# hzxie/Stereo-3D-Reconstruction

Hardware: AMD Instinct MI355X
Metric: stereo pairs/s forward (batch 32, 224x224 -> 32^3 voxel) (higher is better)
Workload: dtype f32

## Files before the change

include/s3r.h:

```cpp
#ifndef S3R_H
#define S3R_H

#include <stddef.h>
#include <stdint.h>

#ifdef __cplusplus
extern "C" {
#endif

#define S3R_ABI_VERSION 8

typedef enum s3r_status {
    S3R_OK = 0,
    S3R_ERR_INVALID = -1,
    S3R_ERR_HIP = -2,
    S3R_ERR_WORKSPACE = -3
} s3r_status;

typedef enum s3r_op {
    S3R_OP_CONV = 0,
    S3R_OP_DECONV = 1,
    S3R_OP_LINEAR = 2
} s3r_op;

typedef enum s3r_dtype {
    S3R_F32 = 0,
    S3R_BF16 = 1
} s3r_dtype;

typedef enum s3r_act { S3R_ACT_NONE = 0, S3R_ACT_RELU = 1, S3R_ACT_SIGMOID = 2,
                       S3R_ACT_LEAKY_RELU = 3, S3R_ACT_ELU = 4, S3R_ACT_TANH = 5  } s3r_act;

typedef enum s3r_layout { S3R_LAYOUT_PLAIN = 0, S3R_LAYOUT_WINO_H = 2, S3R_LAYOUT_WINO_DH = 3, S3R_LAYOUT_WINO_HW = 4 } s3r_layout;

typedef enum s3r_algo { S3R_ALGO_AUTO = 0, S3R_ALGO_DIRECT = 1, S3R_ALGO_WINOGRAD = 2 } s3r_algo;

typedef struct s3r_conv_desc {
    int32_t op;
    int32_t ndim;
    int32_t batch;
    int32_t cin, cout;
    int32_t in_size;
    int32_t k, stride, pad;
    int32_t act;
    int32_t tag;
    int32_t tile;
    int32_t in_halo;
    int32_t out_halo;
    int32_t ksplit;
    int32_t dtype;
    int32_t in_layout;
    int32_t out_layout;
    int32_t algo;
    int32_t dilation;
    int32_t out_pad;
    float act_param;
} s3r_conv_desc;

typedef struct s3r_layer {
    s3r_conv_desc desc;
    const void* packed_w;
    const float* scale;
    const float* shift;
} s3r_layer;

int s3r_abi_version(void);
const char* s3r_last_error(void);

int s3r_conv_out_size(const s3r_conv_desc* d);
int s3r_conv_packed_elems(const s3r_conv_desc* d, int64_t* elems);
int s3r_conv_pack_weights(const s3r_conv_desc* d, const float* w, void* packed, void* stream);
int64_t s3r_conv_scratch_elems(const s3r_conv_desc* d);
int s3r_conv_forward(const s3r_conv_desc* d, const void* x, const void* packed_w, const float* scale,
                     const float* shift, void* y, float* scratch, int64_t scratch_elems, void* stream);

int64_t s3r_chain_workspace_elems(const s3r_layer* layers, int n_layers);
int s3r_chain_forward(const s3r_layer* layers, int n_layers, const void* x, void* y, float* ws, int64_t ws_elems,
                      int ws_fresh, void* stream);

int s3r_encoder_forward(const s3r_layer* layers, int n_layers, const float* images_left, const float* images_right,
                        void* features, float* ws, int64_t ws_elems, int ws_fresh, void* stream);
int s3r_decoder_forward(const s3r_layer* layers, int n_layers, const void* volume, float* occupancy, float* ws,
                        int64_t ws_elems, int ws_fresh, void* stream);

int s3r_encoder_forward_u8(const s3r_layer* layers, int n_layers, const uint8_t* images_left, const uint8_t* images_right,
                           void* features, float* ws, int64_t ws_elems, int ws_fresh, void* stream);

int s3r_channels_last_to_f32(const void* x, float* y, int batch, int channels, int64_t positions, void* stream);

int s3r_cost_volume_forward(const float* feat_left, const float* feat_right, float* volume, int batch, int channels,
                            int max_disp, int height, int width, int out_halo, void* stream);

int s3r_cost_volume_forward_wino(const float* feat_left, const float* feat_right, float* planes, int batch, int channels,
                                 int max_disp, int height, int width, void* stream);
int64_t s3r_conv_wino_input_elems(const s3r_conv_desc* d);
int s3r_conv_wino_input_layout(const s3r_conv_desc* d);
int s3r_cost_volume_forward_wino2(const float* feat_left, const float* feat_right, float* planes, int batch, int channels,
                                  int max_disp, int height, int width, void* stream);

int s3r_cost_volume_forward_bf16(const void* feat_left, const void* feat_right, void* volume, int batch, int channels,
                                 int max_disp, int height, int width, int out_halo, void* stream);

int64_t s3r_linear_scratch_elems(int batch, int cin, int cout);
int s3r_linear_forward(const float* x, const float* w, const float* bias, float* y, int batch, int cin, int cout,
                       int act, float* scratch, int64_t scratch_elems, void* stream);

int s3r_chamfer_forward(const float* p, const float* q, float* dist1, float* dist2, int32_t* idx1, int32_t* idx2,
                        int batch, int n, int m, void* stream);

int s3r_chamfer_backward(const float* p, const float* q, const int32_t* idx1, const int32_t* idx2, const float* grad_dist1,
                         const float* grad_dist2, float* grad_p, float* grad_q, int batch, int n, int m, void* stream);

int s3r_voxel_iou(const float* pred, const float* gt, float threshold, float* iou, int batch, int64_t voxels,
                  void* stream);

int s3r_disparity_wta(const float* feat_l, const float* feat_r, float* disp_l, float* disp_r, int batch, int channels,
// ... 33 lines not shown
```

stereo-3d-reconstruction_amd/_lib.py:

```python
from __future__ import annotations

import ctypes as C
import os
import threading

_HERE = os.path.dirname(os.path.abspath(__file__))
LIB_PATH = os.environ.get("S3R_LIB") or os.path.join(_HERE, "csrc", "libs3r_hip.so")

OP_CONV, OP_DECONV, OP_LINEAR = 0, 1, 2
DTYPE = {"fp32": 0, "bf16": 1}
ACT = {"none": 0, "relu": 1, "sigmoid": 2, "leaky_relu": 3, "elu": 4, "tanh": 5}
FAMILY = {0: "conv_mfma", 1: "stem", 2: "head", 3: "cost_volume", 4: "linear", 5: "chamfer", 6: "iou", 7: "pack",
          8: "pad_copy", 9: "disparity", 10: "aux"}
ABI_VERSION = 8
ALGO_AUTO, ALGO_DIRECT, ALGO_WINOGRAD = 0, 1, 2
ALGO = {None: 0, "auto": 0, "direct": 1, "winograd": 2, False: 1, True: 2}
RAN = {0: "direct", 1: "winograd-serial", 2: "winograd-class-parallel", 3: "winograd-dual", 4: "winograd-2axis", 5: "winograd-3axis", 6: "winograd-3axis-class-parallel"}


class ConvDesc(C.Structure):
    _fields_ = [(n, C.c_int32) for n in
                ("op", "ndim", "batch", "cin", "cout", "in_size", "k", "stride", "pad", "act", "tag", "tile",
                 "in_halo", "out_halo", "ksplit", "dtype", "in_layout", "out_layout", "algo", "dilation", "out_pad")] + \
               [("act_param", C.c_float)]
# ... 17 lines not shown
_lock = threading.Lock()

SIGNATURES = {
    "s3r_abi_version": (C.c_int, []),
    "s3r_last_error": (C.c_char_p, []),
    "s3r_conv_out_size": (C.c_int, [C.POINTER(ConvDesc)]),
    "s3r_conv_packed_elems": (C.c_int, [C.POINTER(ConvDesc), C.POINTER(C.c_int64)]),
    "s3r_conv_pack_weights": (C.c_int, [C.POINTER(ConvDesc), C.c_void_p, C.c_void_p, C.c_void_p]),
    "s3r_conv_scratch_elems": (C.c_int64, [C.POINTER(ConvDesc)]),
    "s3r_conv_forward": (C.c_int, [C.POINTER(ConvDesc), C.c_void_p, C.c_void_p, C.c_void_p, C.c_void_p, C.c_void_p,
                                   C.c_void_p, C.c_int64, C.c_void_p]),
    "s3r_chain_workspace_elems": (C.c_int64, [C.POINTER(Layer), C.c_int]),
    "s3r_chain_forward": (C.c_int, [C.POINTER(Layer), C.c_int, C.c_void_p, C.c_void_p, C.c_void_p, C.c_int64,
                                    C.c_int, C.c_void_p]),
    "s3r_encoder_forward": (C.c_int, [C.POINTER(Layer), C.c_int, C.c_void_p, C.c_void_p, C.c_void_p, C.c_void_p,
                                      C.c_int64, C.c_int, C.c_void_p]),
    "s3r_encoder_forward_u8": (C.c_int, [C.POINTER(Layer), C.c_int, C.c_void_p, C.c_void_p, C.c_void_p, C.c_void_p,
                                         C.c_int64, C.c_int, C.c_void_p]),
    "s3r_channels_last_to_f32": (C.c_int, [C.c_void_p, C.c_void_p, C.c_int, C.c_int, C.c_int64, C.c_void_p]),
    "s3r_decoder_forward": (C.c_int, [C.POINTER(Layer), C.c_int, C.c_void_p, C.c_void_p, C.c_void_p, C.c_int64,
                                      C.c_int, C.c_void_p]),
    "s3r_cost_volume_forward": (C.c_int, [C.c_void_p, C.c_void_p, C.c_void_p, C.c_int, C.c_int, C.c_int, C.c_int,
                                          C.c_int, C.c_int, C.c_void_p]),
    "s3r_cost_volume_forward_bf16": (C.c_int, [C.c_void_p, C.c_void_p, C.c_void_p, C.c_int, C.c_int, C.c_int, C.c_int,
                                               C.c_int, C.c_int, C.c_void_p]),
    "s3r_cost_volume_forward_wino": (C.c_int, [C.c_void_p, C.c_void_p, C.c_void_p, C.c_int, C.c_int, C.c_int, C.c_int,
                                               C.c_int, C.c_void_p]),
    "s3r_conv_wino_input_elems": (C.c_int64, [C.POINTER(ConvDesc)]),
    "s3r_conv_wino_input_layout": (C.c_int, [C.POINTER(ConvDesc)]),
    "s3r_cost_volume_forward_wino2": (C.c_int, [C.c_void_p, C.c_void_p, C.c_void_p, C.c_int, C.c_int, C.c_int, C.c_int,
                                                C.c_int, C.c_void_p]),
    "s3r_linear_scratch_elems": (C.c_int64, [C.c_int, C.c_int, C.c_int]),
    "s3r_linear_forward": (C.c_int, [C.c_void_p, C.c_void_p, C.c_void_p, C.c_void_p, C.c_int, C.c_int, C.c_int,
                                     C.c_int, C.c_void_p, C.c_int64, C.c_void_p]),
    "s3r_chamfer_forward": (C.c_int, [C.c_void_p, C.c_void_p, C.c_void_p, C.c_void_p, C.c_void_p, C.c_void_p,
                                      C.c_int, C.c_int, C.c_int, C.c_void_p]),
    "s3r_chamfer_backward": (C.c_int, [C.c_void_p, C.c_void_p, C.c_void_p, C.c_void_p, C.c_void_p, C.c_void_p, C.c_void_p, C.c_void_p,
                                       C.c_int, C.c_int, C.c_int, C.c_void_p]),
    "s3r_voxel_iou": (C.c_int, [C.c_void_p, C.c_void_p, C.c_float, C.c_void_p, C.c_int, C.c_int64, C.c_void_p]),
    "s3r_disparity_wta": (C.c_int, [C.c_void_p, C.c_void_p, C.c_void_p, C.c_void_p, C.c_int, C.c_int, C.c_int, C.c_int,
                                    C.c_int, C.c_void_p]),
    "s3r_disparity_epe": (C.c_int, [C.c_void_p, C.c_void_p, C.c_void_p, C.c_void_p, C.c_int, C.c_int64, C.c_void_p]),
    "s3r_disparity_soft": (C.c_int, [C.c_void_p, C.c_void_p, C.c_int, C.c_void_p, C.c_void_p, C.c_void_p, C.c_void_p, C.c_int,
                                     C.c_int, C.c_int, C.c_int, C.c_int, C.c_float, C.c_int, C.c_int, C.c_float, C.c_void_p]),
    "s3r_disparity_metrics": (C.c_int, [C.c_void_p, C.c_void_p, C.c_void_p, C.c_void_p, C.c_int, C.c_int64, C.c_void_p]),
    "s3r_profile_enable": (C.c_int, [C.c_int]),
    "s3r_profile_reset": (C.c_int, []),
    "s3r_profile_detail": (C.c_int, [C.c_int]),
    "s3r_profile_read": (C.c_int, [C.POINTER(ProfRecord), C.c_int]),
}


def load():
    global _lib
    if _lib is not None:
        return _lib
    with _lock:
        if _lib is not None:
            return _lib
        if not os.path.exists(LIB_PATH):
            raise S3RError(
                f"HIP extension not built: {LIB_PATH} is missing. Run `python -c 'import __graft_entry__ as g; "
                f"g.build()'` (or `make -C stereo-3d-reconstruction_amd/csrc`). There is no CPU fallback.")
        try:
            lib = C.CDLL(LIB_PATH)
        except OSError as e:
            raise S3RError(f"cannot load {LIB_PATH}: {e}") from e
        for name, (res, args) in SIGNATURES.items():
            fn = getattr(lib, name)
            fn.restype, fn.argtypes = res, args
        if lib.s3r_abi_version() != ABI_VERSION:
            raise S3RError("libs3r_hip.so ABI version mismatch")
        _lib = lib
    return _lib


def check(rc, what=""):
    if rc < 0:
        msg = load().s3r_last_error().decode("utf-8", "replace")
        raise S3RError(f"{what}: {msg} (code {rc})")
    return rc


LAYOUT_PLAIN, LAYOUT_WINO_H, LAYOUT_WINO_DH, LAYOUT_WINO_HW = 0, 2, 3, 4


def make_desc(layer, batch, in_size, tag=0, tile=-1, in_halo=0, out_halo=0, ksplit=0, dtype=0, in_layout=0, out_layout=0,
              algo=0):
    from . import arch_spec as _spec
    op = {"conv2d": OP_CONV, "conv3d": OP_CONV, "deconv3d": OP_DECONV, "deconv2d": OP_DECONV, "linear": OP_LINEAR}[layer.op]
    nd = _spec.ndim(layer)
    return ConvDesc(op, nd, batch, layer.cin, layer.cout, in_size, layer.k, layer.s, layer.p, ACT[layer.act], tag,
                    tile, in_halo, out_halo, ksplit, dtype, in_layout, out_layout, algo, getattr(layer, "dil", 1),
                    getattr(layer, "opad", 0), _spec.act_param(layer))


def profile_enable(max_records):
    check(load().s3r_profile_enable(int(max_records)), "profile_enable")


def profile_detail(level):
    check(load().s3r_profile_detail(int(level)), "profile_detail")


def profile_reset():
    check(load().s3r_profile_reset(), "profile_reset")


def profile_read(max_records=4096):
    buf = (ProfRecord * max_records)()
    n = check(load().s3r_profile_read(buf, max_records), "profile_read")
    return [dict(family=FAMILY.get(r.family, str(r.family)), tag=r.tag, ms=r.ms, launches=r.launches, flops=r.flops,
                 bytes=r.bytes, exec_flops=r.exec_flops, ran=RAN.get(r.algo, str(r.algo))) for r in buf[:n]]
```

stereo-3d-reconstruction_amd/csrc/s3r_api.hip:

```cpp
#include "s3r_host.h"

#include <cmath>
#include <cstdlib>
#include <cstring>

using namespace s3rh;

namespace {

inline bool misaligned16(const void* p) { return ((uintptr_t)p & 15) != 0; }
int bf16_align_fail(const char* what, const void* p) {
    return fail(S3R_ERR_INVALID, "%s must be 16-byte aligned (got %p): bf16 tensors are accessed 16 bytes at a time", what, p);
}

int wino2_run(const s3r_conv_desc* d, const Geo& g, s3r::ConvParams p, const float* x, const float* packed_w, float* y, float* scratch,
              int64_t scratch_elems, int form, hipStream_t s, int* launches) {
    const Wino2Geo g2 = wino2_geo(d);
    const WinoNeed need = wino2_need(d, form);
    const bool pre = d->in_layout == S3R_LAYOUT_WINO_DH || d->in_layout == S3R_LAYOUT_WINO_HW;
    const bool to_v = d->out_layout == S3R_LAYOUT_WINO_HW;
    if (g2.bmax <= 0 || ((pre || to_v) && g2.bmax < d->batch))
        return fail(S3R_ERR_INVALID, "two-axis Winograd form: the transformed input of this batch exceeds 2 GiB (at most %d samples per "
                    "call with a producer-written input: s3r_conv_wino_input_elems)", g2.bmax);
    if (!scratch || scratch_elems < need.total)
        return fail(S3R_ERR_WORKSPACE, "the two-axis Winograd form of this layer needs %lld floats of scratch (s3r_conv_scratch_elems), "
                    "got %lld", (long long)need.total, (long long)(scratch ? scratch_elems : 0));
    const int64_t direct_w = ipow(d->k, g.nd) * d->cin * cout_pad(d->cout);
    p.w = packed_w + direct_w + (wino_layer(d) ? wino_w_elems(d) : 0);
    p.x = pre ? x : scratch;
    p.part = scratch + need.v;
    p.Nd = g2.sg; p.Nh = g2.sg; p.Nw = g2.out;
    p.kd = 1; p.kh = 1; p.kw = g2.kw; p.T = g2.kw;
    p.x_hs = g2.wp; p.x_ds = g2.sg * g2.wp; p.x_cs = g2.sg * g2.sg * g2.wp;
    p.x_org = 0;
    p.dS = s3r::FastDiv((unsigned)(p.Nd * p.Nh * p.Nw));
    p.dHW = s3r::FastDiv((unsigned)(p.Nh * p.Nw));
    p.dW = s3r::FastDiv((unsigned)p.Nw);
    if (g2.ax == 2) {
        p.Nd = 1; p.Nw = g2.sg;
        p.dS = s3r::FastDiv((unsigned)(g2.sg * g2.sg));
        p.dW = s3r::FastDiv((unsigned)g2.sg);
    }
    p.Hout = g2.out; p.Dout = g2.out;
    p.ncls = g2.ncls;
    p.ksplit = 1;
    const int64_t x_sample = g.x_elems / d->batch;
    *launches = 0;
    for (int b0 = 0; b0 < d->batch; b0 += g2.bmax) {
        const int nb = d->batch - b0 < g2.bmax ? d->batch - b0 : g2.bmax;
        hipError_t e = hipSuccess;
        if (!pre) {
            s3r::AuxScope aux(s, 4.0 * ((double)nb * x_sample + (double)(g2.ax == 2 ? g2.ncls * d->cin * s3r::wino2_npad(g2.pos_sample * nb) : g2.v_sample * nb)));
            if (g2.ax == 2)
                e = s3r::launch_wino2p_input(x + (int64_t)b0 * x_sample, scratch, nb, d->cin, g2.wp, g2.wp, g2.sg, g2.sg,
                                             s3r::wino2_npad(g2.pos_sample * nb), s);
            else
                e = s3r::launch_wino2_input(x + (int64_t)b0 * x_sample, scratch, g2.ax, (long long)nb * d->cin, g2.wp, g2.wp, g2.wp, g2.sg, g2.sg, s);
            if (e != hipSuccess) return hip_fail(e, "two-axis Winograd input transform launch");
            *launches += 1;
        }
        p.B = nb;
        p.x_cls = nb * d->cin * p.x_cs;
        p.x_bytes = (unsigned)(4 * (int64_t)nb * g2.v_sample);
        p.Ntotal = nb * p.Nd * p.Nh * p.Nw;
        p.y = y + (int64_t)b0 * p.y_bs;
        p.y_bytes = (unsigned)(4 * (int64_t)nb * p.y_bs);
        int nl = 0;
        e = s3r::launch_conv_wino2(p, g2.ax, wino2_form_of(d, p.Ntotal, form), to_v, s, &nl);
        if (e != hipSuccess) return hip_fail(e, "two-axis Winograd conv launch");
        *launches += nl;
    }
    return S3R_OK;
}

int dwino_run(const s3r_conv_desc* d, s3r::ConvParams p, const float* x, const float* packed_w, float* scratch, int64_t scratch_elems,
              int form, hipStream_t s, int* launches, int* ran) {
    const WinoNeed need = wino_need(d, form, p.head_w != nullptr);
    if (!scratch || scratch_elems < need.total)
        return fail(S3R_ERR_WORKSPACE, "the Winograd form of this transposed convolution needs %lld floats of scratch "
                    "(s3r_conv_scratch_elems), got %lld", (long long)need.total, (long long)(scratch ? scratch_elems : 0));
    const int n = d->in_size;
    p.xd_mode = dwino_materialise(d) ? 1 : 0;
    hipError_t e;
    {
        const double x_el = (double)d->batch * d->cin * (double)ipow(n + 2, 3);
        s3r::AuxScope aux(s, 4.0 * x_el * (p.xd_mode ? 4.0 : 2.0));
        e = s3r::launch_wino_diff(x, scratch, (long long)d->batch * d->cin, n + 2, n + 2, n + 2, p.xd_mode, s);
    }
    if (e != hipSuccess) return hip_fail(e, "Winograd difference-tensor launch");
    p.x = x;
    p.xd = scratch;
    p.part = scratch + need.v;
    p.w = packed_w + 64 * (int64_t)d->cin * cout_pad(d->cout);
    p.Nd = n / 2; p.Nh = n / 2;
    p.Ntotal = p.B * p.Nd * p.Nh * p.Nw;
    p.n_begin = 0; p.n_end = p.Ntotal;
    p.dS = s3r::FastDiv((unsigned)(p.Nd * p.Nh * p.Nw));
    p.dHW = s3r::FastDiv((unsigned)(p.Nh * p.Nw));
    p.dW = s3r::FastDiv((unsigned)p.Nw);
    p.ksplit = 1;
    const s3r::WinoLaunch L = s3r::wino_plan(2, d->cout, wino_kcls(d), p.Ntotal, p.head_w != nullptr, form);
    int nl = 0;
    e = s3r::launch_deconv_wino(p, L, s, &nl);
    if (e != hipSuccess) return hip_fail(e, "Winograd transposed-conv launch");
    *launches = 1 + nl;
    *ran = 1 + L.mode;
    return S3R_OK;
}
int dwino3_run(const s3r_conv_desc* d, s3r::ConvParams p, const float* x, const float* packed_w, float* scratch, int64_t scratch_elems,
               hipStream_t s, int form, int* launches, int* ran) {
    const int n = d->in_size;
    const Dwino3Need nd = dwino3_need(d, form);
    const int64_t need = nd.total;
    if (!scratch || scratch_elems < need)
        return fail(S3R_ERR_WORKSPACE, "the three-axis Winograd form of this transposed convolution needs %lld floats of scratch "
                    "(s3r_conv_scratch_elems), got %lld", (long long)need, (long long)(scratch ? scratch_elems : 0));
    hipError_t e;
    {
        s3r::AuxScope aux(s, 4.0 * 4.0 * (double)d->batch * d->cin * (double)ipow(n + 2, 3));
        e = s3r::launch_wino_diff(x, scratch, (long long)d->batch * d->cin, n + 2, n + 2, n + 2, 1, s);
    }
    if (e != hipSuccess) return hip_fail(e, "Winograd difference-tensor launch");
    p.x = x;
    p.xd = scratch;
    p.w = packed_w + dwino3_w_offset(d);
    p.Nd = p.Nh = p.Nw = n / 2;
    p.Ntotal = p.B * p.Nd * p.Nh * p.Nw;
    p.dS = s3r::FastDiv((unsigned)(p.Nd * p.Nh * p.Nw));
    p.dHW = s3r::FastDiv((unsigned)(p.Nh * p.Nw));
    p.dW = s3r::FastDiv((unsigned)p.Nw);
    p.ksplit = 1;
    p.part = nd.split ? scratch + nd.diff : nullptr;
    e = s3r::launch_deconv_wino3(p, nd.split, s);
    if (e != hipSuccess) return hip_fail(e, "three-axis Winograd transposed-conv launch");
    *launches = nd.split ? 3 : 2;
    *ran = nd.split ? 6 : 5;
    return S3R_OK;
}

int conv_head_fused(const s3r_conv_desc* d, const Geo& g, const s3r_conv_desc* hd, const Geo& hg, const float* x,
                    const s3r_layer& L, const s3r_layer& H, float* out, float* scratch, int64_t scratch_elems, hipStream_t s) {
    s3r::ConvParams p = make_params(d, g);
    p.x = x; p.w = static_cast<const float*>(L.packed_w); p.scale = L.scale; p.shift = L.shift; p.y = out;
    const bool is3 = hd->ndim == 3;
    p.y_hs = hg.out_p; p.y_ds = is3 ? hg.out_p * hg.out_p : 0; p.y_cs = (int)ipow(hg.out_p, hg.nd);
    p.y_bs = p.y_cs;
    p.y_org = hd->out_halo * (p.y_ds + p.y_hs + 1);
    p.y_bytes = (unsigned)(hg.y_elems * 4);
    p.head_w = static_cast<const float*>(H.packed_w); p.head_scale = H.scale; p.head_shift = H.shift; p.head_act = hd->act;
    int alg, form;
    int rc = resolve_algo(d, &alg, &form);
    if (rc) return rc;
    if (alg == ALG_WINO3) {
        if (d->cout > 64) return fail(S3R_ERR_INVALID, "the fused head rides on the transposed Winograd kernel with <= 64 couts only");
        ProfScope ps(s, F_MFMA, d->tag, g.flops + hg.flops, g.bytes - 4.0 * d->batch * d->cout * (double)g.out_sp +
                     4.0 * d->batch * (double)hg.out_sp);
        ps.exec = g.flops * (27.0 / 64.0) + hg.flops;
        ps.algo = 5;
        return dwino3_run(d, p, x, static_cast<const float*>(L.packed_w), scratch, scratch_elems, s, form, &ps.launches, &ps.algo);
    }
    if (alg != ALG_DIRECT) {
        if (alg != ALG_WINO || d->op != S3R_OP_DECONV || d->cout > 64) return fail(S3R_ERR_INVALID, "the fused head rides on the transposed Winograd kernel with <= 64 couts only");
        ProfScope ps(s, F_MFMA, d->tag, g.flops + hg.flops, g.bytes - 4.0 * d->batch * d->cout * (double)g.out_sp +
                     4.0 * d->batch * (double)hg.out_sp);
        ps.exec = wino_exec_flops(d, g) + hg.flops;
        return dwino_run(d, p, x, static_cast<const float*>(L.packed_w), scratch, scratch_elems, form, s, &ps.launches, &ps.algo);
    }
    Launch Ln;
    rc = resolve_launch(d, &p, &Ln);
    if (rc) return rc;
    if (!(Ln.cfg == 1 || Ln.cfg == 2 || Ln.cfg == 7) || (Ln.cfg == 2 && d->cout > 32)) {
        int bm, bn;
        s3r::conv_tile_dims(1, &bm, &bn);
        const long wg1 = (long)((p.Ntotal + bn - 1) / bn) * (p.transposed ? 8 : 1);
        Ln.cfg = d->cout <= 32 ? 2 : (wg1 >= 2000 ? 1 : 7);
    }
    ProfScope ps(s, F_MFMA, d->tag, g.flops + hg.flops, g.bytes - 4.0 * d->batch * d->cout * (double)g.out_sp +
                 4.0 * d->batch * (double)hg.out_sp);
    hipError_t e = s3r::launch_conv_mfma(p, Ln.cfg + 16 * Ln.vec, s);
    ps.launches = s3r::conv_last_launch_count();
    if (e != hipSuccess) return hip_fail(e, "fused conv+head launch");
    return S3R_OK;
}

int conv_head_fused_h(const s3r_conv_desc* d, const Geo& g, const s3r_conv_desc* hd, const Geo& hg, const void* x,
                      const s3r_layer& L, const s3r_layer& H, float* out, hipStream_t s) {
    s3r::ConvParamsH p = make_params_h(d, g);
    p.x = x; p.w = L.packed_w; p.scale = L.scale; p.shift = L.shift; p.y = out;
// ... 283 lines not shown
                    if (e != hipSuccess) return hip_fail(e, "conv forward launch");
                    ps.launches += s3r::conv_last_launch_count();
                }
                if (needs_act_pass(d)) {
                    s3r::AuxScope aux(s, 8.0 * (double)g.y_elems);
                    e = s3r::launch_act(y, g.y_elems, d->act, d->act_param, s);
                    if (e != hipSuccess) return hip_fail(e, "activation launch");
                    ps.launches += 1;
                }
                return S3R_OK;
            }
            s3r::ConvParams p = make_params(d, g);
            p.x = x; p.w = packed_w; p.scale = scale; p.shift = shift; p.y = y;
            const bool wino = alg == ALG_WINO;
            if (alg == ALG_WINO2) {
                ProfScope ps(s, F_MFMA, d->tag, g.flops, g.bytes);
                ps.exec = wino2_exec_flops(d);
                ps.algo = 4;
                return wino2_run(d, g, p, x, packed_w, y, scratch, scratch_elems, form, s, &ps.launches);
            }
            if (alg == ALG_WINO3) {
                ProfScope ps(s, F_MFMA, d->tag, g.flops, g.bytes);
                ps.exec = g.flops * (27.0 / 64.0);
                ps.algo = 5;
                return dwino3_run(d, p, x, packed_w, scratch, scratch_elems, s, form, &ps.launches, &ps.algo);
            }
            if (wino && d->op == S3R_OP_DECONV) {
                ProfScope ps(s, F_MFMA, d->tag, g.flops, g.bytes);
                ps.exec = wino_exec_flops(d, g);
                return dwino_run(d, p, x, packed_w, scratch, scratch_elems, form, s, &ps.launches, &ps.algo);
            }
            if (wino) {
                const bool pre = d->in_layout == S3R_LAYOUT_WINO_H;
                const int R = wino_r(d), kind = wino_kind(d);
                const int is3 = d->ndim == 3, n = d->in_size, wp = n + 2, h2 = (n + R - 1) / R, dp = is3 ? n + 2 : 1;
                const int bmax = wino_bmax(d);
                if (bmax <= 0 || (pre && bmax < d->batch))
                    return fail(S3R_ERR_INVALID, "a Winograd-transformed input takes at most %d samples per call here "
                                "(s3r_conv_wino_input_elems)", bmax);
                const WinoNeed need = wino_need(d, form, false);
                if (need.total > 0 && (!scratch || scratch_elems < need.total))
                    return fail(S3R_ERR_WORKSPACE, "the Winograd form of this layer needs %lld floats of scratch (s3r_conv_scratch_elems), "
                                "got %lld", (long long)need.total, (long long)(scratch ? scratch_elems : 0));
                const int64_t v_sample = wino_v_elems(d) / d->batch, x_sample = g.x_elems / d->batch;
                ProfScope ps(s, F_MFMA, d->tag, g.flops, g.bytes);
                ps.launches = 0;
                ps.exec = wino_exec_flops(d, g);
                p.w = packed_w + ipow(3, g.nd) * d->cin * cout_pad(d->cout);
                p.x = pre ? x : scratch;
                p.part = scratch ? scratch + need.v : nullptr;
                p.Nh = h2; p.T = p.kd * p.kw;
                p.x_hs = wp; p.x_ds = is3 ? h2 * wp : 0; p.x_cs = dp * h2 * wp;
                p.x_org = 0;
                p.dS = s3r::FastDiv((unsigned)(p.Nd * p.Nh * p.Nw));
                p.dHW = s3r::FastDiv((unsigned)(p.Nh * p.Nw));
                p.dW = s3r::FastDiv((unsigned)p.Nw);
                p.Hout = n;
                p.ksplit = 1;
                for (int b0 = 0; b0 < d->batch; b0 += bmax) {
                    const int nb = d->batch - b0 < bmax ? d->batch - b0 : bmax;
                    if (!pre) {
                        s3r::AuxScope aux(s, 4.0 * ((double)nb * x_sample + (double)nb * v_sample));
                        e = s3r::launch_wino_input(x + (int64_t)b0 * x_sample, scratch, (long long)nb * d->cin * dp, n + 2, wp, h2, R, s);
                        if (e != hipSuccess) return hip_fail(e, "Winograd input transform launch");
                        ps.launches += 1;
                    }
                    p.B = nb;
                    p.x_cls = nb * d->cin * p.x_cs;
                    p.x_bytes = (unsigned)(4 * (int64_t)nb * v_sample);
                    p.Ntotal = nb * p.Nd * p.Nh * p.Nw;
                    p.y = y + (int64_t)b0 * p.y_bs;
                    p.y_bytes = (unsigned)(4 * (int64_t)nb * p.y_bs);
                    const s3r::WinoLaunch WL = s3r::wino_plan(kind, d->cout, wino_kcls(d), p.Ntotal, false, form);
                    int nl = 0;
                    e = s3r::launch_conv_wino(p, WL, s, &nl);
                    if (e != hipSuccess) return hip_fail(e, "Winograd conv launch");
                    ps.launches += nl;
                    ps.algo = 1 + WL.mode;
                }
                return S3R_OK;
            }
            Launch L;
            if ((rc = resolve_launch(d, &p, &L))) return rc;
            if (L.ksplit > 1) {
                const int64_t need = s3r::conv_scratch_elems(p, L.cfg);
                if (scratch && scratch_elems >= need) p.part = scratch;
                else
                    return fail(S3R_ERR_WORKSPACE, "ksplit=%d needs %lld floats of scratch (s3r_conv_scratch_elems), got %lld", L.ksplit,
                                (long long)need, (long long)(scratch ? scratch_elems : 0));
            }
            ProfScope ps(s, F_MFMA, d->tag, g.flops, g.bytes);
            e = s3r::launch_conv_mfma(p, L.cfg + 16 * L.vec, s);
            ps.launches = s3r::conv_last_launch_count();
            if (e == hipSuccess && needs_act_pass(d)) {
                s3r::AuxScope aux(s, 8.0 * (double)g.y_elems);
                e = s3r::launch_act(y, g.y_elems, d->act, d->act_param, s);
                ps.launches += 1;
            }
            break;
        }
    }
    if (e != hipSuccess) return hip_fail(e, "conv forward launch");
    return S3R_OK;
}

int chain_forward_impl(const s3r_layer* layers, int n_layers, const void* x, const void* x2, int nsplit, int x_u8, void* y,
                       float* ws, int64_t ws_elems, int ws_fresh, void* stream);

}

extern "C" {

int s3r_chain_forward(const s3r_layer* layers, int n_layers, const void* x, void* y, float* ws, int64_t ws_elems,
                      int ws_fresh, void* stream) {
    return chain_forward_impl(layers, n_layers, x, nullptr, 0, 0, y, ws, ws_elems, ws_fresh, stream);
}

}

namespace {

int chain_forward_impl(const s3r_layer* layers, int n_layers, const void* x, const void* x2, int nsplit, int x_u8, void* y,
                       float* ws, int64_t ws_elems, int ws_fresh, void* stream) {
    Plan pl;
    int rc = plan_chain(layers, n_layers, &pl);
    if (rc) return rc;
    if (!x || !y) return fail(S3R_ERR_INVALID, "null tensor pointer");
    {
        const int last = n_layers - 1;
        bool any_bf16 = false;
        for (int i = 0; i < n_layers; ++i) any_bf16 = any_bf16 || pl.d[i].dtype == S3R_BF16;
        if (pl.d[0].dtype == S3R_BF16 && pl.r[0] != R_STEM && misaligned16(x)) return bf16_align_fail("the bf16 input of an S3R_BF16 chain", x);
        if (pl.d[last].dtype == S3R_BF16 && pl.r[last] != R_HEAD && misaligned16(y))
            return bf16_align_fail("the bf16 output of an S3R_BF16 chain", y);
        if (any_bf16 && pl.total > 0 && ws && misaligned16(ws)) return bf16_align_fail("the workspace of a chain with S3R_BF16 layers", ws);
    }
    if (pl.total > 0 && (!ws || ws_elems < pl.total))
        return fail(S3R_ERR_WORKSPACE, "chain needs a workspace of %lld floats, got %lld", (long long)pl.total,
                    (long long)ws_elems);
    hipStream_t s = (hipStream_t)stream;
    if (ws_fresh && pl.total > 0) {
        hipError_t e = hipMemsetAsync(ws, 0, (size_t)pl.total * sizeof(float), s);
        if (e != hipSuccess) return hip_fail(e, "workspace memset");
    }
    const void* cur = x;
    if ((x2 || x_u8) && (pl.pad_input || pl.r[0] != R_STEM))
        return fail(S3R_ERR_INVALID, "a second input tensor / 8-bit renders need a chain that starts with the stem convolution");
    if (pl.r[0] == R_STEM && (((uintptr_t)x & 15) || ((uintptr_t)x2 & 15)))
        return fail(S3R_ERR_INVALID, "render tensors must be 16-byte aligned (got %p, %p)", x, x2);
    if (pl.pad_input) {
        const s3r_conv_desc& d0 = pl.d[0];
        const int hl = d0.in_halo, is3 = d0.ndim == 3;
        ProfScope ps(s, F_PAD, d0.tag, 0.0, 8.0 * d0.batch * d0.cin * (double)pl.g[0].in_sp);
        hipError_t e;
        if (d0.dtype == S3R_BF16) {
            const int wc = d0.in_size * d0.cin / 2, hwc = hl * d0.cin / 2;
            e = s3r::launch_pad_copy(static_cast<const float*>(x), ws + pl.pad_off, d0.batch, is3 ? d0.in_size : 1,
                                     d0.in_size, wc, is3 ? hl : 0, hl, hwc, s);
        } else {
            e = s3r::launch_pad_copy(static_cast<const float*>(x), ws + pl.pad_off, (int64_t)d0.batch * d0.cin,
                                     is3 ? d0.in_size : 1, d0.in_size, d0.in_size, is3 ? hl : 0, hl, hl, s);
        }
        if (e != hipSuccess) return hip_fail(e, "pad copy launch");
        cur = ws + pl.pad_off;
    }
    for (int i = 0; i < n_layers; ++i) {
// ... 306 lines not shown
```

stereo-3d-reconstruction_amd/csrc/s3r_conv_glds.hip:

```cpp
#include "s3r_kernels.h"
#include <cstdlib>
#include <type_traits>

namespace s3r {

typedef float f32x16 __attribute__((ext_vector_type(16)));
typedef float v4f __attribute__((ext_vector_type(4)));
typedef float v2f __attribute__((ext_vector_type(2)));
typedef float v4f_u __attribute__((ext_vector_type(4), aligned(4)));
typedef float v2f_u __attribute__((ext_vector_type(2), aligned(4)));
typedef unsigned v2u __attribute__((ext_vector_type(2)));
typedef unsigned v4u __attribute__((ext_vector_type(4)));

#define S3R_LDS_PTR(p) ((__attribute__((address_space(3))) void*)(p))

template <int N> struct FVec;
template <> struct FVec<1> { typedef float type; };
template <> struct FVec<2> { typedef v2f type; };
template <> struct FVec<4> { typedef v4f type; };

template <int N>
__device__ __forceinline__ float vget(const typename FVec<N>::type& v, int i) {
    if constexpr (N == 1) return v; else return v[i];
}
// ... 544 lines not shown

void conv_tile_dims(int cfg, int* bm, int* bn) {
    *bm = kTileDims[cfg][0];
    *bn = kTileDims[cfg][1];
}
int conv_num_tiles() { return kNumTiles; }

struct Tuned { int cin, cout, T, stride, S, transposed, tile, ksplit; };
static const Tuned kTuned[] = {
    {32,  64,  9, 1, 12544, 0, 7, 1},
    {64,  64,  9, 2,  3136, 0, 1, 1},
    {64, 128,  9, 1,  3136, 0, 4, 1},
    {128, 128, 9, 2,   784, 0, 7, 1},
    {128, 256, 9, 1,   784, 0, 1, 1},
    {256, 256, 9, 1,   784, 0, 1, 1},
    {256, 32,  1, 1,   784, 0, 2, 1},
    {64,  64, 27, 1, 21952, 0, 1, 1},
    {64, 128, 27, 2,  2744, 0, 7, 1},
    {128, 128, 27, 1, 2744, 0, 7, 1},
    {128, 256, 27, 2,  343, 0, 3, 4},
    {256, 256, 27, 1,  343, 0, 3, 4},
    {256, 512, 64, 1,   64, 0, 7, 8},
    {512, 256,  8, 1,   64, 1, 7, 1},
    {256, 128,  8, 1,  512, 1, 1, 1},
    {128,  64,  8, 1, 4096, 1, 1, 1},
};

static const Tuned* find_tuned(const ConvParams& p) {
    const int S = p.Nd * p.Nh * p.Nw;
    for (const Tuned& t : kTuned)
        if (t.cin == p.Cin && t.cout == p.Cout && t.T == p.T && t.stride == p.stride && t.S == S &&
            t.transposed == p.transposed)
            return &t;
    return nullptr;
}

int conv_pick_ksplit(const ConvParams& p, int ) {
    if (const Tuned* t = find_tuned(p)) return t->ksplit;
    const int chunks = p.Cin / GBK;
    const long S = (long)p.Nd * p.Nh * p.Nw;
    const long wg_nom = ((p.Cout + 63) / 64) * ((32 * S + 63) / 64) * (p.transposed ? 8 : 1);
    int ks = 1;
    while (wg_nom * ks < 2048 && chunks % (2 * ks) == 0 && (chunks / (2 * ks)) * p.T >= 100) ks *= 2;
    return ks;
}

int conv_pick_tile(const ConvParams& p) {
    const int classes = (p.transposed ? 8 : 1) * (p.ksplit > 1 ? p.ksplit : 1);
    auto wgs = [&](int cfg) {
        const long bm = kTileDims[cfg][0], bn = kTileDims[cfg][1];
        return ((p.Cout + bm - 1) / bm) * ((p.Ntotal + bn - 1) / bn) * classes;
    };
    if (const Tuned* t = find_tuned(p))
        if (wgs(t->tile) >= 512) return t->tile;
    if (p.Cout <= 32) return wgs(2) >= 128 ? 2 : 3;
    if (p.Cout <= 64) return wgs(1) >= 2000 ? 1 : (wgs(7) >= 2000 ? 7 : 3);
    if (wgs(2) >= 1500) return 2;
    return wgs(7) >= 1500 ? 7 : 3;
}

int conv_pick_vec(const ConvParams& p) {
    if (p.stride != 1) return 1;
    return (p.Nw % 4 == 0) ? 4 : 1;
}

template <int WM, int WN, int TM, int TN, int VEC, bool HEAD, int NBUF = 2>
static hipError_t launch_cfg(ConvParams p, hipStream_t stream) {
    constexpr int BM = 32 * WM * TM, BN = 32 * WN * TN;
    if constexpr (GBK * BN % (256 * VEC) != 0 || BN > 256 * VEC) {
        return hipErrorInvalidValue;
    } else {
        p.m_tiles = (p.Cout + BM - 1) / BM;
        p.n_tiles = (p.n_end - p.n_begin + BN - 1) / BN;
        const size_t lds = (size_t)NBUF * GBK * (BM + BN) * sizeof(float);
        if (lds > 48 * 1024) {
            static LdsAttr lds_attr;
            const hipError_t attr = lds_attr.ensure(
                reinterpret_cast<const void*>(&conv_glds_kernel<WM, WN, TM, TN, VEC, HEAD, NBUF>), (int)lds);
            if (attr != hipSuccess) return attr;
        }
        dim3 grid(p.m_tiles * p.n_tiles * (p.transposed ? 8 : 1), 1, p.ksplit);
        hipLaunchKernelGGL((conv_glds_kernel<WM, WN, TM, TN, VEC, HEAD, NBUF>), grid, dim3(256), lds, stream, p);
        hipError_t e = hipGetLastError();
        if (e == hipSuccess && p.ksplit > 1) e = launch_conv_finish(p, p.n_tiles * BN, stream);
        return e;
    }
}

template <int WM, int WN, int TM, int TN, int VEC>
static hipError_t launch_dual_cfg(ConvParams p, int n_cut, hipStream_t stream) {
    constexpr int BM = 32 * WM * TM, BN = 32 * WN * TN;
    if constexpr (GBK * BN % (256 * VEC) != 0 || BN > 256 * VEC || GBK * 64 % (256 * VEC) != 0) {
        return hipErrorInvalidValue;
    } else {
        p.n_cut = n_cut;
        p.big_wgs = ((p.Cout + BM - 1) / BM) * ((n_cut - p.n_begin + BN - 1) / BN);
        const int small = ((p.Cout + 63) / 64) * ((p.n_end - n_cut + 63) / 64);
        p.m_tiles = 0; p.n_tiles = 0;
        const size_t lds = (size_t)2 * GBK * (BM + BN) * sizeof(float);
        if (lds > 48 * 1024) {
            static LdsAttr lds_attr;
            const hipError_t attr = lds_attr.ensure(reinterpret_cast<const void*>(&conv_glds_dual_kernel<WM, WN, TM, TN, VEC>), (int)lds);
            if (attr != hipSuccess) return attr;
        }
        hipLaunchKernelGGL((conv_glds_dual_kernel<WM, WN, TM, TN, VEC>), dim3(p.big_wgs + small), dim3(256), lds, stream, p);
        return hipGetLastError();
    }
}

template <int WM, int WN, int TM, int TN>
static hipError_t launch_dual_vec(const ConvParams& p, int n_cut, int vec, hipStream_t stream) {
    switch (vec) {
        case 4: return launch_dual_cfg<WM, WN, TM, TN, 4>(p, n_cut, stream);
        case 1: return launch_dual_cfg<WM, WN, TM, TN, 1>(p, n_cut, stream);
        default: return hipErrorInvalidValue;
    }
}

static hipError_t launch_dual(const ConvParams& p, int cfg, int n_cut, int vec, hipStream_t stream) {
    switch (cfg) {
        case 0: return launch_dual_vec<2, 2, 2, 2>(p, n_cut, vec, stream);
        case 1: return launch_dual_vec<1, 4, 2, 2>(p, n_cut, vec, stream);
        case 4: return launch_dual_vec<2, 2, 2, 4>(p, n_cut, vec, stream);
        case 7: return launch_dual_vec<1, 4, 2, 1>(p, n_cut, vec, stream);
        default: return hipErrorNotSupported;
    }
}

static bool sparse_launch(const ConvParams& p, int bm, int bn) {
    static const bool off = getenv("S3R_DEEP_RING") && atoi(getenv("S3R_DEEP_RING")) == 0;
    const long w = (long)((p.Cout + bm - 1) / bm) * ((p.n_end - p.n_begin + bn - 1) / bn) * (p.transposed ? 8 : 1) * p.ksplit;
    return !off && w <= 384;
}

template <int WM, int WN, int TM, int TN>
static hipError_t launch_vec(const ConvParams& p, int vec, hipStream_t stream) {
    if constexpr (WM == 1 && TM * TN <= 4) {
        if (p.head_w) {
            switch (vec) {
                case 4: return launch_cfg<WM, WN, TM, TN, 4, true>(p, stream);
                case 1: return launch_cfg<WM, WN, TM, TN, 1, true>(p, stream);
                default: return hipErrorInvalidValue;
            }
        }
    } else if (p.head_w) {
        return hipErrorInvalidValue;
    }
    if constexpr (WM == 2 && WN == 2 && TM == 1 && TN == 1) {
        if (sparse_launch(p, 64, 64)) {
            switch (vec) {
                case 4: return launch_cfg<WM, WN, TM, TN, 4, false, 6>(p, stream);
                case 1: return launch_cfg<WM, WN, TM, TN, 1, false, 6>(p, stream);
                default: return hipErrorInvalidValue;
            }
        }
    }
    switch (vec) {
        case 4: return launch_cfg<WM, WN, TM, TN, 4, false>(p, stream);
        case 1: return launch_cfg<WM, WN, TM, TN, 1, false>(p, stream);
        default: return hipErrorInvalidValue;
    }
}

static hipError_t launch_tile(const ConvParams& p, int cfg, int vec, hipStream_t stream) {
    g_launch_count += 1;
    switch (cfg) {
        case 0: return launch_vec<2, 2, 2, 2>(p, vec, stream);
        case 1: return launch_vec<1, 4, 2, 2>(p, vec, stream);
        case 2: return launch_vec<1, 4, 1, 2>(p, vec, stream);
        case 3: return launch_vec<2, 2, 1, 1>(p, vec, stream);
        case 4: return launch_vec<2, 2, 2, 4>(p, vec, stream);
        case 5: return launch_vec<1, 4, 2, 4>(p, vec, stream);
        case 6: return launch_vec<2, 2, 2, 1>(p, vec, stream);
        case 7: return launch_vec<1, 4, 2, 1>(p, vec, stream);
        default: return hipErrorInvalidValue;
    }
}

static bool plan_tail_cut(const ConvParams& p, int cfg, int* n_cut) {
    if (p.ksplit != 1 || p.Cout <= 32 || cfg == 3) return false;
    const int classes = p.transposed ? 8 : 1;
    const long bm = kTileDims[cfg][0], bn = kTileDims[cfg][1];
    const long m_tiles = (p.Cout + bm - 1) / bm, n_tiles = (p.Ntotal + bn - 1) / bn;
    const long W = m_tiles * n_tiles * classes;
    const long CUS = cu_count();
    const long rounds = W / CUS, rem = W % CUS;
    const bool dual = !p.transposed && (cfg == 0 || cfg == 1 || cfg == 4 || cfg == 7) && getenv("S3R_NO_DUAL") == nullptr;
    if (rounds < 1 || rounds >= (dual ? 64 : 16) || rem == 0) return false;
    const long n_main = (rounds * CUS) / (m_tiles * classes);
    if (n_main < 1 || n_main >= n_tiles) return false;
    const long pos_tail = p.Ntotal - n_main * bn;
    const long W_tail = ((pos_tail + 63) / 64) * ((p.Cout + 63) / 64) * classes;
    const double before = (double)((W + CUS - 1) / CUS);
    const double bulk = (double)((n_main * m_tiles * classes + CUS - 1) / CUS);
    const double small = (64.0 * 64.0) / (double)(bm * bn);
    const double after = dual ? bulk + (double)W_tail / (double)CUS * small / 0.85
                              : bulk + (double)((W_tail + CUS - 1) / CUS) * small / 0.8;
    if (after > (dual ? 0.99 : 0.97) * before) return false;
    *n_cut = (int)(n_main * bn);
    return true;
}

hipError_t launch_conv_mfma(const ConvParams& pin, int code, hipStream_t stream) {
    ConvParams p = pin;
    g_launch_count = 0;
    int cfg = code & 15;
    int vec = code >> 4;
    if (cfg == 15) cfg = conv_pick_tile(p);
    if (cfg >= kNumTiles) return hipErrorInvalidValue;
    const int vmax = conv_pick_vec(p);
    if (vec != 1 && vec != 4) vec = vmax;
    if (vec > vmax) vec = vmax;
    if (p.Cin % GBK != 0 || p.Ntotal % vec != 0) return hipErrorInvalidValue;
    if (p.ksplit < 1 || (p.Cin / GBK) % p.ksplit != 0 || (p.ksplit > 1 && !p.part)) return hipErrorInvalidValue;
    if (p.head_w) {
        int bm, bn;
        conv_tile_dims(cfg, &bm, &bn);
        const bool wm1 = cfg == 1 || cfg == 2 || cfg == 7;
        if (!wm1 || bm < p.Cout || p.ksplit != 1 || p.act == ACT_SIGMOID) return hipErrorInvalidValue;
    }
#ifdef S3R_ABLATE
    p.debug = abl_mode();
#endif
    p.n_begin = 0;
    p.n_end = p.Ntotal;
    int n_cut = 0;
    static const bool no_cut = getenv("S3R_NO_TAIL_CUT") != nullptr;
    if (!p.head_w && !no_cut && plan_tail_cut(p, cfg, &n_cut)) {
        static const bool no_dual = getenv("S3R_NO_DUAL") != nullptr;
        if (!no_dual && !p.transposed && p.Cout > 32) {
            g_launch_count += 1;
            const hipError_t ed = launch_dual(p, cfg, n_cut, vec, stream);
            if (ed != hipErrorNotSupported) return ed;
            g_launch_count -= 1;
        }
        p.n_end = n_cut;
        hipError_t e = launch_tile(p, cfg, vec, stream);
        if (e != hipSuccess) return e;
        p.n_begin = n_cut;
        p.n_end = p.Ntotal;
        return launch_tile(p, 3, vec, stream);
    }
    return launch_tile(p, cfg, vec, stream);
}

__global__ void pack_glds_kernel(const float* __restrict__ w, float* __restrict__ wp, int Cin, int Cout, int CoutPad,
                                 int T, int transposed) {
    const size_t per_cls = (size_t)T * Cin * CoutPad;
    const size_t total = (transposed ? 8 : 1) * per_cls;
    for (size_t i = blockIdx.x * (size_t)blockDim.x + threadIdx.x; i < total; i += (size_t)gridDim.x * blockDim.x) {
        const int cls = (int)(i / per_cls);
        size_t r = i % per_cls;
        const int co = (int)(r % CoutPad);
        r /= CoutPad;
        const int c = (int)(r & 15);
        r >>= 4;
        const int tap = (int)(r % T);
        const int cc = (int)(r / T);
        const int cin = cc * 16 + c;
        float v = 0.f;
        if (co < Cout) {
            if (!transposed) {
                v = w[((size_t)co * Cin + cin) * T + tap];
            } else {
                const int rd = (cls >> 2) & 1, rh = (cls >> 1) & 1, rw = cls & 1;
                const int td = (tap >> 2) & 1, th = (tap >> 1) & 1, tw = tap & 1;
                const int kd = 3 - rd - 2 * td, kh = 3 - rh - 2 * th, kw = 3 - rw - 2 * tw;
                v = w[((size_t)cin * Cout + co) * 64 + (kd * 4 + kh) * 4 + kw];
            }
        }
        wp[i] = v;
    }
}

hipError_t launch_pack_conv(const float* w, float* wp, int Cin, int Cout, int CoutPad, int T, int transposed,
                            hipStream_t s) {
    hipLaunchKernelGGL(pack_glds_kernel, dim3(1024), dim3(256), 0, s, w, wp, Cin, Cout, CoutPad, T, transposed);
    return hipGetLastError();
}

#ifdef S3R_ABLATE
}
extern "C" int s3r_debug_read_timeline(unsigned long long* out, int nblocks) {
    if (nblocks > 65536) nblocks = 65536;
    return hipMemcpyFromSymbol(out, HIP_SYMBOL(s3r::s3r_timeline), sizeof(unsigned long long) * 6 * (size_t)nblocks) == hipSuccess ? nblocks : -1;
}
namespace s3r {
#endif
}
```

stereo-3d-reconstruction_amd/csrc/s3r_conv_wino.hip:

```cpp
#include "s3r_kernels.h"
#include <cstdlib>

namespace s3r {

typedef float wf32x16 __attribute__((ext_vector_type(16)));
typedef float wv2f __attribute__((ext_vector_type(2)));
template <int N> struct WVec;
template <> struct WVec<1> { typedef float type; };
template <> struct WVec<2> { typedef wv2f type; };
typedef float wv4f __attribute__((ext_vector_type(4)));
template <> struct WVec<4> { typedef wv4f type; };
template <int N>
__device__ __forceinline__ float wvget(const typename WVec<N>::type& v, int i) {
    if constexpr (N == 1) return v; else return v[i];
}

#define S3R_LDS_PTR_W(p) ((__attribute__((address_space(3))) void*)(p))

#ifndef S3R_WNB
#define S3R_WNB 2
#endif
#ifndef S3R_WBK
#define S3R_WBK 32
#endif
// ... 686 lines not shown
            for (int k = 0; k < R; ++k)
                if (k < row1) yo[wino_out_off<KIND>(k, p.y_ds, p.y_hs)] = wino_act(y[k], sc, sf, lo);
        }
    }
}

template <int KIND>
static hipError_t launch_wino_finish(const ConvParams& p, int n_begin, int n_end, int npad, hipStream_t stream) {
    const long long total = p.head_w ? (long long)(n_end - n_begin) : (long long)p.Cout * (n_end - n_begin);
    const long long blocks = (total + 255) / 256;
    const dim3 grid((unsigned)(blocks < 8192 ? blocks : 8192), KIND == 2 ? 8 : 1);
    if constexpr (KIND == 2) {
        if (p.head_w) hipLaunchKernelGGL((wino_finish_kernel<KIND, true>), grid, dim3(256), 0, stream, p, n_begin, n_end, npad);
        else hipLaunchKernelGGL((wino_finish_kernel<KIND, false>), grid, dim3(256), 0, stream, p, n_begin, n_end, npad);
    } else {
        hipLaunchKernelGGL((wino_finish_kernel<KIND, false>), grid, dim3(256), 0, stream, p, n_begin, n_end, npad);
    }
    return hipGetLastError();
}

constexpr int WCN = 64;
#ifdef S3R_ABLATE
static int wabl_mode() { static const int m = getenv("S3R_ABL") ? atoi(getenv("S3R_ABL")) : 0; return m; }
#define S3R_WABL(p) (p).debug = wabl_mode()
#else
#define S3R_WABL(p) (void)0
#endif

int64_t wino_slab_elems(int kind, int cout, int ntotal, const WinoLaunch& L) {
    if (L.mode == WINO_SERIAL) return 0;
    const int ncls = kind == 2 ? 72 : 6;
    const int n0 = L.mode == WINO_DUAL ? L.n_cut : 0;
    const int64_t npad = (int64_t)((ntotal - n0 + WCN - 1) / WCN) * WCN;
    return (int64_t)ncls * cout * npad;
}

WinoLaunch wino_plan(int kind, int cout, int kcls, int ntotal, bool head, int forced) {
    WinoLaunch L;
    L.mode = WINO_SERIAL; L.n_cut = 0;
    const int m_tiles = (cout + WBM - 1) / WBM;
    const int pcs = kind == 2 ? 8 : 1;
    const int ncls = kind == 2 ? 9 : 6;
    const long W = (long)m_tiles * ((ntotal + WCN - 1) / WCN) * pcs;
    if (forced < 0) {
        static const int env_mode = getenv("S3R_WINO_FORM") ? atoi(getenv("S3R_WINO_FORM")) : -1;
        forced = env_mode;
    }
    const int occ = kind == 2 ? 3 : 4;
    const int CUS = cu_count();
    const double u = (double)W / (double)CUS;
    int kb = (int)u;
    if (forced >= 0) {
        L.mode = forced <= WINO_DUAL ? forced : WINO_SERIAL;
        if ((double)kb >= u) kb -= 1;
    } else {
        (void)head;
        constexpr double EFF = 0.9, EFF_ALONE = 0.7, SLAB = 100.0, LAUNCH = 220.0, TAIL = 0.6;
        const double unit = (double)ncls * kcls;
        auto serial_cost = [&](int w) {
            const int rem = w % occ;
            return (w - (rem == 1 ? 1 : 0)) * unit / EFF + (rem == 1 ? unit / EFF_ALONE : 0.0);
        };
        const double serial = serial_cost((int)__builtin_ceil(u));
        const double cp = __builtin_ceil(u * ncls) * (kcls / EFF + SLAB) + LAUNCH;
        double best = serial;
        if (cp < best) { best = cp; L.mode = WINO_CP; }
        for (int k : {(int)u, (int)u % occ == 1 ? (int)u - 1 : 0}) {
            if (k < 1 || (double)k >= u) continue;
            const double dual = serial_cost(k) + TAIL * __builtin_ceil((u - k) * ncls) * (kcls / EFF + SLAB) + LAUNCH;
            if (dual < 0.97 * best) { best = dual; L.mode = WINO_DUAL; kb = k; }
        }
    }
    if (L.mode == WINO_DUAL) {
        const long n_main = ((long)kb * CUS) / (m_tiles * pcs);
        L.n_cut = (int)(n_main * WCN);
        if (L.n_cut <= 0 || L.n_cut >= ntotal) { L.mode = L.n_cut <= 0 ? WINO_CP : WINO_SERIAL; L.n_cut = 0; }
    }
    return L;
}

template <int VEC, int KIND>
static hipError_t launch_wino_forms(ConvParams p, const WinoLaunch& L, hipStream_t stream) {
    const int ntotal = p.Ntotal;
    auto lds_of = [](int bn) { return (size_t)WNB * WBK * (WBM + (KIND == 2 ? 2 : 1) * bn) * sizeof(float); };
    const int pcs = KIND == 2 ? 8 : 1;
    constexpr int NCLS = WinoKind<KIND>::NCLS;
    p.n_begin = 0; p.n_end = ntotal;
    if (L.mode == WINO_SERIAL) {
        const dim3 grid(p.m_tiles * ((ntotal + WCN - 1) / WCN) * pcs);
        if constexpr (KIND == 2) {
            if (p.head_w) {
                if (p.xd_mode) hipLaunchKernelGGL((wino_kernel<VEC, KIND, 2, false, true, true>), grid, dim3(256), lds_of(WCN), stream, p);
                else hipLaunchKernelGGL((wino_kernel<VEC, KIND, 2, false, true, false>), grid, dim3(256), lds_of(WCN), stream, p);
            } else {
                if (p.xd_mode) hipLaunchKernelGGL((wino_kernel<VEC, KIND, 2, false, false, true>), grid, dim3(256), lds_of(WCN), stream, p);
                else hipLaunchKernelGGL((wino_kernel<VEC, KIND, 2, false, false, false>), grid, dim3(256), lds_of(WCN), stream, p);
            }
            return hipGetLastError();
        }
        hipLaunchKernelGGL((wino_kernel<VEC, KIND, 2, false, false>), grid, dim3(256), lds_of(WCN), stream, p);
        return hipGetLastError();
    }
    if (!p.part) return hipErrorInvalidValue;
    const int n0 = L.mode == WINO_DUAL ? L.n_cut : 0;
    const int cp_tiles = (ntotal - n0 + WCN - 1) / WCN;
    const int cp_wgs = p.m_tiles * cp_tiles * NCLS * pcs;
    if (L.mode == WINO_DUAL) {
        p.n_cut = n0;
        p.big_wgs = p.m_tiles * (n0 / WCN) * pcs;
        const dim3 grid(p.big_wgs + cp_wgs);
        if constexpr (KIND == 2) {
            if (p.head_w) {
                if (p.xd_mode) hipLaunchKernelGGL((wino_dual_kernel<VEC, KIND, true, true>), grid, dim3(256), lds_of(WCN), stream, p);
                else hipLaunchKernelGGL((wino_dual_kernel<VEC, KIND, true, false>), grid, dim3(256), lds_of(WCN), stream, p);
            } else {
                if (p.xd_mode) hipLaunchKernelGGL((wino_dual_kernel<VEC, KIND, false, true>), grid, dim3(256), lds_of(WCN), stream, p);
                else hipLaunchKernelGGL((wino_dual_kernel<VEC, KIND, false, false>), grid, dim3(256), lds_of(WCN), stream, p);
            }
        } else {
            hipLaunchKernelGGL((wino_dual_kernel<VEC, KIND>), grid, dim3(256), lds_of(WCN), stream, p);
        }
    } else if (KIND == 2 && p.xd_mode) {
        hipLaunchKernelGGL((wino_kernel<VEC, KIND, 2, true, false, KIND == 2>), dim3(cp_wgs), dim3(256), lds_of(WCN), stream, p);
    } else {
        hipLaunchKernelGGL((wino_kernel<VEC, KIND, 2, true, false>), dim3(cp_wgs), dim3(256), lds_of(WCN), stream, p);
    }
    hipError_t e = hipGetLastError();
    if (e != hipSuccess) return e;
    AuxScope aux(stream, 4.0 * (double)(ntotal - n0) * p.Cout * (pcs * NCLS + (p.head_w ? 0.0 : pcs * WinoKind<KIND>::R)));
    return launch_wino_finish<KIND>(p, n0, ntotal, cp_tiles * WCN, stream);
}

hipError_t launch_conv_wino(ConvParams p, const WinoLaunch& L, hipStream_t stream, int* launches) {
    if (p.Cin % WBK != 0 || p.stride != 1 || p.transposed || p.ksplit != 1 || p.head_w || p.act == ACT_SIGMOID)
        return hipErrorInvalidValue;
    p.kh = 1;
    S3R_WABL(p);
    p.m_tiles = (p.Cout + WBM - 1) / WBM;
    if (launches) *launches = L.mode == WINO_SERIAL ? 1 : 2;
    return p.Nw % 4 == 0 ? launch_wino_forms<4, 1>(p, L, stream) : launch_wino_forms<1, 1>(p, L, stream);
}

hipError_t launch_deconv_wino(ConvParams p, const WinoLaunch& L, hipStream_t stream, int* launches) {
    if (p.Cin % WBK != 0 || !p.transposed || p.ksplit != 1 || !p.xd || p.act == ACT_SIGMOID || (p.head_w && p.Cout > WBM))
        return hipErrorInvalidValue;
    S3R_WABL(p);
    p.m_tiles = (p.Cout + WBM - 1) / WBM;
    if (launches) *launches = L.mode == WINO_SERIAL ? 1 : 2;
    if (p.Nw % 4 != 0) return hipErrorInvalidValue;
    return launch_wino_forms<4, 2>(p, L, stream);
}

template <int AX> struct WAxis;
template <> struct WAxis<0> { static constexpr int N = 6, M = 4, R = 3; };
template <> struct WAxis<1> { static constexpr int N = 5, M = 2, R = 4; };
int wino2_classes(int ax) { return ax == 1 ? 25 : 36; }
int wino2_outputs(int ax) { return ax == 1 ? 2 : 4; }

template <int AX>
__device__ __forceinline__ void wax_bt(const float (&r)[WAxis<AX>::N], float (&v)[WAxis<AX>::N]) {
    if constexpr (AX == 0) wino_rows_to_classes<4>(r, v);
    else {
        v[0] = fmaf(2.f, r[0] - r[2], r[3] - r[1]);
        v[1] = fmaf(-2.f, r[1], r[3] - r[2]);
        v[2] = fmaf(2.f, r[1], fmaf(-3.f, r[2], r[3]));
        v[3] = r[3] - r[1];
        v[4] = fmaf(2.f, r[1] - r[3], r[4] - r[2]);
    }
}
template <int AX>
__device__ __forceinline__ void wax_at(const float (&m)[WAxis<AX>::N], float (&y)[WAxis<AX>::M]) {
    if constexpr (AX == 0) wino_out<1>(m, y);
    else {
        y[0] = ((m[0] + m[1]) + m[2]) + m[3];
        y[1] = fmaf(2.f, m[3], m[1] - m[2]) + m[4];
    }
}
template <int AX>
__device__ __forceinline__ float wax_g(int c, const float (&g)[WAxis<AX>::R]) {
    if constexpr (AX == 0) {
        const float s02 = g[0] + g[2], a = g[0] * (1.f / 24.f) + g[2] * (1.f / 6.f), b12 = g[1] * (1.f / 12.f);
        return c == 0 ? g[0] * 0.25f : c == 1 ? (s02 + g[1]) * (-1.f / 6.f) : c == 2 ? (s02 - g[1]) * (-1.f / 6.f)
             : c == 3 ? a + b12 : c == 4 ? a - b12 : g[2];
    } else {
        const float e = g[0] + g[2], o = g[1] + g[3];
        return c == 0 ? g[0] * 0.5f : c == 1 ? (e + o) * -0.5f : c == 2 ? (o - e) * (1.f / 6.f)
             : c == 3 ? fmaf(g[3], 4.f / 3.f, fmaf(g[2], 2.f / 3.f, fmaf(g[1], 1.f / 3.f, g[0] * (1.f / 6.f)))) : g[3];
    }
}

template <int AX>
__global__ __launch_bounds__(256) void wino2_input_kernel(const float* __restrict__ x, float* __restrict__ V, unsigned total,
                                                          int Dp, int Hp, int Wp, int SD, int SH, FastDiv dW, FastDiv dSH, FastDiv dSD) {
    constexpr int N = WAxis<AX>::N, M = WAxis<AX>::M;
    for (unsigned i = blockIdx.x * 256u + threadIdx.x; i < total; i += gridDim.x * 256u) {
        const unsigned row = (unsigned)dW.div((int)i);
        const int w = (int)(i - row * (unsigned)Wp);
        const unsigned pg = (unsigned)dSH.div((int)row);
        const int sh = (int)(row - pg * (unsigned)SH);
        const unsigned pl = (unsigned)dSD.div((int)pg);
        const int sd = (int)(pg - pl * (unsigned)SD);
        const float* __restrict__ src = x + ((size_t)pl * Dp + M * sd) * Hp * Wp + (size_t)M * sh * Wp + w;
        float t[N][N];
#pragma unroll
        for (int a = 0; a < N; ++a) {
            float r[N], v[N];
#pragma unroll
            for (int b = 0; b < N; ++b)
                r[b] = (M * sd + a < Dp && M * sh + b < Hp) ? src[((size_t)a * Hp + b) * Wp] : 0.f;
            wax_bt<AX>(r, v);
#pragma unroll
// ... 316 lines not shown
    constexpr int N = 6, M = 4;
    extern __shared__ __attribute__((aligned(16))) float fsm[];
    const int tid = threadIdx.x;
    const int G = p.Nh * p.Nw, Wp = TOV ? p.Hout + 2 : p.y_hs, plane = TOV ? Wp * Wp : p.y_cs;
    const float lo = p.act == ACT_RELU ? 0.f : -__builtin_inff();
    const size_t cstride = (size_t)p.Cout * npad;
    const int nbg = (p.B + PL - 1) / PL;
    for (int item = blockIdx.x; item < p.Cout * nbg; item += gridDim.x) {
        const int mrow = item / nbg;
        const int b0 = (item - mrow * nbg) * PL;
        const int npl = p.B - b0 < PL ? p.B - b0 : PL;
        for (int i = tid; i < npl * plane; i += 256) fsm[i] = 0.f;
        __syncthreads();
        const float sc = p.scale ? p.scale[mrow] : 1.f, sf = p.shift ? p.shift[mrow] : 0.f;
        for (int t = tid; t < npl * G; t += 256) {
            const int pl = p.dS.div(t);
            const int s = t - pl * G;
            const int sh = p.dW.div(s);
            const int sw = s - sh * p.Nw;
            const int n = b0 * G + t;
            const float* __restrict__ src = p.part + ((size_t)mrow * (npad >> 6) + (n >> 6)) * ((SEMI ? N * M : N * N) * 64) + (n & 63);
            float tt[N][M];
#pragma unroll
            for (int a = 0; a < N; ++a) {
                if constexpr (SEMI) {
#pragma unroll
                    for (int v = 0; v < M; ++v) tt[a][v] = src[(a * M + v) * 64];
                } else {
                    float m[N], y[M];
#pragma unroll
                    for (int c = 0; c < N; ++c) m[c] = src[(a * N + c) * 64];
                    wax_at<0>(m, y);
#pragma unroll
                    for (int v = 0; v < M; ++v) tt[a][v] = y[v];
                }
            }
            float* __restrict__ o = fsm + pl * plane + (halo + M * sh) * Wp + halo + M * sw;
#pragma unroll
            for (int v = 0; v < M; ++v) {
                float m[N], y[M];
#pragma unroll
                for (int a = 0; a < N; ++a) m[a] = tt[a][v];
                wax_at<0>(m, y);
#pragma unroll
                for (int u = 0; u < M; ++u)
                    if (M * sh + v < p.Hout && M * sw + u < p.Hout) o[v * Wp + u] = wino_act(y[u], sc, sf, lo);
            }
        }
        __syncthreads();
        if constexpr (TOV) {
            for (int t = tid; t < npl * G; t += 256) {
                const int pl = p.dS.div(t);
                const int s = t - pl * G;
                const int sh = p.dW.div(s);
                const int sw = s - sh * p.Nw;
                const float* __restrict__ win = fsm + pl * plane + M * sh * Wp + M * sw;
                float tt[N][N];
#pragma unroll
                for (int jc = 0; jc < N; ++jc) {
                    float r[N], v[N];
#pragma unroll
                    for (int ir = 0; ir < N; ++ir) r[ir] = win[ir * Wp + jc];
                    wax_bt<0>(r, v);
#pragma unroll
                    for (int ir = 0; ir < N; ++ir) tt[ir][jc] = v[ir];
                }
                float* __restrict__ dst = p.y + (size_t)mrow * npad + (size_t)b0 * G + t;
#pragma unroll
                for (int bb = 0; bb < N; ++bb) {
                    float v[N];
                    wax_bt<0>(tt[bb], v);
#pragma unroll
                    for (int a = 0; a < N; ++a) dst[(size_t)(a * N + bb) * cstride] = v[a];
                }
            }
        } else {
            for (int pl = 0; pl < npl; ++pl)
                wino2_copy_out(fsm + pl * plane, p.y + (size_t)(b0 + pl) * p.y_bs + (size_t)mrow * p.y_cs, plane, tid);
        }
        __syncthreads();
    }
}

int wino2_form(int ax, int cout, int ntotal, int forced) {
    if (ax == 1) return 0;
    if (forced >= 0) return forced ? 1 : 0;
    static const int env_form = getenv("S3R_WINO2_FORM") ? atoi(getenv("S3R_WINO2_FORM")) : -1;
    if (env_form >= 0) return env_form ? 1 : 0;
    const long semi_wgs = (long)((cout + WBM - 1) / WBM) * ((ntotal + WCN - 1) / WCN) * 6;
    return semi_wgs >= (ax == 2 ? 2 : 8) * (long)cu_count() ? 1 : 0;
}
int64_t wino2_npad(int64_t ntotal) { return (ntotal + WCN - 1) / WCN * WCN; }
int64_t wino2_slab_elems(int ax, int cout, int ntotal, int form) {
    const int64_t npad = (int64_t)((ntotal + WCN - 1) / WCN) * WCN;
    return (form ? 6 * 4 : wino2_classes(ax)) * (int64_t)cout * npad;
}

hipError_t launch_conv_wino2(ConvParams p, int ax, int form, bool to_v, hipStream_t stream, int* launches) {
    if (p.Cin % WBK != 0 || p.stride != 1 || p.transposed || p.ksplit != 1 || p.head_w || p.act == ACT_SIGMOID || !p.part ||
        ax < 0 || ax > 2 || p.ncls != wino2_classes(ax))
        return hipErrorInvalidValue;
    p.kh = 1;
    S3R_WABL(p);
    p.m_tiles = (p.Cout + WBM - 1) / WBM;
    p.n_begin = 0; p.n_end = p.Ntotal;
    const int n_tiles = (p.Ntotal + WCN - 1) / WCN;
    const size_t lds = (size_t)WNB * WBK * (WBM + WCN) * sizeof(float);
    const int halo = to_v ? 1 : (p.y_hs - p.Hout) / 2;
    if (to_v && (ax != 2 || p.Hout % 4 != 0)) return hipErrorInvalidValue;
    if (!to_v && (halo < 0 || p.y_hs != p.Hout + 2 * halo)) return hipErrorInvalidValue;
    if (ax == 2) {
        const int plane = to_v ? (p.Hout + 2) * (p.Hout + 2) : p.y_hs * p.y_hs, G = p.Nh * p.Nw;
        if ((!to_v && p.y_cs != plane) || (size_t)plane * 4 > 64 * 1024) return hipErrorInvalidValue;
        int PL = 256 / G < 1 ? 1 : 256 / G;
        if (PL > p.B) PL = p.B;
        while (PL > 1 && (size_t)PL * plane * 4 > 64 * 1024) --PL;
        const int npad = n_tiles * WCN;
        ConvParams q = p;
        q.B = 1; q.Nd = 1; q.Nh = 1; q.Nw = npad;
        q.dS = q.dHW = q.dW = FastDiv((unsigned)npad);
        q.kd = q.kh = q.kw = 1; q.T = 1;
        q.x_org = 0; q.x_ds = 0; q.x_hs = 0; q.x_cs = npad; q.x_cls = p.Cin * npad;
        q.x_bytes = (unsigned)(4ull * 36 * p.Cin * npad);
        q.Ntotal = npad; q.n_end = npad;
        const dim3 grid(p.m_tiles * n_tiles * (form == 1 ? 6 : 36));
        if (form == 1) hipLaunchKernelGGL((wino_kernel<4, 1, 2, false, false, false, true>), grid, dim3(256), lds, stream, q);
        else hipLaunchKernelGGL((wino_kernel<4, 1, 2, true, false>), grid, dim3(256), lds, stream, q);
        hipError_t e = hipGetLastError();
        if (e != hipSuccess) return e;
        const long long items = (long long)p.Cout * ((p.B + PL - 1) / PL);
        const dim3 fgrid((unsigned)(items < 16384 ? items : 16384));
        const size_t flds = (size_t)PL * plane * 4;
        AuxScope aux(stream, 4.0 * (double)p.Cout * ((double)(form == 1 ? 24 : 36) * npad + (to_v ? 36.0 * npad : (double)p.B * plane)));
        if (to_v) {
            if (form == 1) hipLaunchKernelGGL((wino2p_finish_kernel<true, true>), fgrid, dim3(256), flds, stream, p, npad, halo, PL);
            else hipLaunchKernelGGL((wino2p_finish_kernel<false, true>), fgrid, dim3(256), flds, stream, p, npad, halo, PL);
        } else if (form == 1) hipLaunchKernelGGL((wino2p_finish_kernel<true, false>), fgrid, dim3(256), flds, stream, p, npad, halo, PL);
        else hipLaunchKernelGGL((wino2p_finish_kernel<false, false>), fgrid, dim3(256), flds, stream, p, npad, halo, PL);
        if (launches) *launches = 2;
        return hipGetLastError();
    }
    if (p.y_ds != p.y_hs * p.y_hs || p.y_cs != (p.Dout + 2 * halo) * p.y_ds) return hipErrorInvalidValue;
    if (form == 1) {
        const int M = wino2_outputs(ax), G = p.Nh * p.Nw;
        if (ax != 0 || (size_t)M * p.y_ds * 4 > 64 * 1024) return hipErrorInvalidValue;
        int SUB = 256 / G < 1 ? 1 : 256 / G;
        if (SUB > p.B * p.Nd) SUB = p.B * p.Nd;
        while (SUB > 1 && (size_t)SUB * M * p.y_ds * 4 > 64 * 1024) --SUB;
        const size_t flds = (size_t)SUB * M * p.y_ds * 4;
        const FastDiv dNd((unsigned)p.Nd), dMS((unsigned)(M * p.y_ds));
        const long long items = (long long)p.Cout * ((p.B * p.Nd + SUB - 1) / SUB);
        const dim3 fgrid((unsigned)(items < 32768 ? items : 32768));
        const dim3 grid(p.m_tiles * n_tiles * 6);
        if (p.Nw % 4 == 0) hipLaunchKernelGGL((wino_kernel<4, 1, 2, false, false, false, true>), grid, dim3(256), lds, stream, p);
        else hipLaunchKernelGGL((wino_kernel<1, 1, 2, false, false, false, true>), grid, dim3(256), lds, stream, p);
        hipError_t e = hipGetLastError();
        if (e != hipSuccess) return e;
        AuxScope aux(stream, 4.0 * (double)p.Cout * (24.0 * n_tiles * WCN + (double)p.B * p.y_cs));
        hipLaunchKernelGGL(wino2s_finish_kernel, fgrid, dim3(256), flds, stream, p, n_tiles * WCN, halo, SUB, dNd, dMS);
        if (launches) *launches = 2;
        return hipGetLastError();
    }
    const dim3 grid(p.m_tiles * n_tiles * p.ncls);
    if (p.Nw % 4 == 0) hipLaunchKernelGGL((wino_kernel<4, 1, 2, true, false>), grid, dim3(256), lds, stream, p);
    else hipLaunchKernelGGL((wino_kernel<1, 1, 2, true, false>), grid, dim3(256), lds, stream, p);
    hipError_t e = hipGetLastError();
    if (e != hipSuccess) return e;
    const long long total = (long long)p.Cout * p.Ntotal;
    const long long blocks = (total + 255) / 256;
    const dim3 flat((unsigned)(blocks < 8192 ? blocks : 8192));
    AuxScope aux(stream, 4.0 * (double)p.Cout * ((double)p.ncls * n_tiles * WCN + (double)p.B * p.Dout * p.Hout * p.Nw));
    if (ax == 0) hipLaunchKernelGGL(wino2_finish_flat_kernel<0>, flat, dim3(256), 0, stream, p, n_tiles * WCN);
    else hipLaunchKernelGGL(wino2_finish_flat_kernel<1>, flat, dim3(256), 0, stream, p, n_tiles * WCN);
    if (launches) *launches = 2;
    return hipGetLastError();
}

#ifdef S3R_ABLATE
}
extern "C" int s3r_debug_read_timeline_wino(unsigned long long* out, int nblocks) {
    if (nblocks > 65536) nblocks = 65536;
    return hipMemcpyFromSymbol(out, HIP_SYMBOL(s3r::s3r_wino_timeline), sizeof(unsigned long long) * 6 * (size_t)nblocks) == hipSuccess ? nblocks : -1;
}
extern "C" int s3r_debug_clear_timeline_wino() {
    void* ptr = nullptr;
    if (hipGetSymbolAddress(&ptr, HIP_SYMBOL(s3r::s3r_wino_timeline)) != hipSuccess) return -1;
    return hipMemset(ptr, 0, sizeof(unsigned long long) * 6 * 65536) == hipSuccess ? 0 : -1;
}
namespace s3r {
#endif

}
```

stereo-3d-reconstruction_amd/csrc/s3r_host.h:

```cpp
#pragma once
#include "../../include/s3r.h"
#include "s3r_kernels.h"

#include <cstdint>
#include <vector>

namespace s3rh {

constexpr int64_t kMaxElems = (int64_t)1 << 31;
constexpr int64_t kMaxBytes = (int64_t)1 << 32;

const char* last_error();

enum Family { F_MFMA = 0, F_STEM = 1, F_HEAD = 2, F_COSTVOL = 3, F_LINEAR = 4, F_CHAMFER = 5, F_IOU = 6, F_PACK = 7, F_PAD = 8, F_DISP = 9,
              F_AUX = 10 };

struct ProfScope {
    bool active = false;
    int slot = -1;
    unsigned gen = 0;
    hipEvent_t e0 = nullptr, e1 = nullptr;
    int launches = 1;
    int algo = 0;
    double exec = -1.0;
    int family, prev_tag = 0;
    hipStream_t stream;
    ProfScope(hipStream_t s, int family, int tag, double flops, double bytes);
    ~ProfScope();
    ProfScope(const ProfScope&) = delete;
    ProfScope& operator=(const ProfScope&) = delete;
};

struct Geo {
    int nd;
    int in, out;
    int in_p, out_p;
    int64_t in_sp, out_sp;
    int64_t x_elems, y_elems;
    int64_t x_store, y_store;
    int64_t w_elems;
    double flops, bytes;
};

enum Route { R_STEM, R_HEAD, R_MFMA, R_LINEAR };

enum { ALG_DIRECT = 0, ALG_WINO = 1, ALG_WINO2 = 2, ALG_WINO3 = 3 };

struct Wino2Geo { int ax, m, n, ncls, out, sg, wp, kw, bmax; int64_t w_elems, v_sample, pos_sample; };

struct WinoNeed { int64_t v, slab, total; };

struct LaunchH { int tm, ksplit; };

struct Launch { int cfg, vec, ksplit; };

struct Plan {
    std::vector<s3r_conv_desc> d;
    std::vector<Route> r;
    std::vector<Geo> g;
    std::vector<int64_t> off;
    std::vector<char> fuse_head;
    bool stem_wino = false;
    bool pad_input = false;
    int64_t pad_off = 0;
    int64_t scratch_off = 0, scratch_elems = 0;
    int64_t total = 0;
};


int fail(int code, const char* fmt, ...);
int hip_fail(hipError_t e, const char* what);
int64_t ipow(int64_t b, int e);
int wino_r(const s3r_conv_desc*);
int out_size(const s3r_conv_desc* d);
int dil_of(const s3r_conv_desc* d);
bool staged_layer(const s3r_conv_desc* d);
struct StagedGeo { int cin_pad, step, pe, sp; int64_t elems; int bmax; };
StagedGeo staged_geo(const s3r_conv_desc* d);
s3r::ConvParams make_params_staged(const s3r_conv_desc* d, const Geo& g);
struct TClassAxis { int kr, ke, qmin, nq; };
bool im2col_layer(const s3r_conv_desc* d);
bool leaky_fused(const s3r_conv_desc* d);
bool needs_act_pass(const s3r_conv_desc* d);
bool tclass_layer(const s3r_conv_desc* d);
bool tclass_direct(const s3r_conv_desc* d);
bool tshuf_layer(const s3r_conv_desc* d);
s3r::ConvParams make_params_tshuf(const s3r_conv_desc* d, const Geo& g);
int want_halo(const s3r_conv_desc* d, Route r);
TClassAxis tclass_axis(const s3r_conv_desc* d, int r);
int tclass_halo(const s3r_conv_desc* d);
int64_t tclass_w_elems(const s3r_conv_desc* d);
bool make_params_tclass(const s3r_conv_desc* d, const Geo& g, int rd, int rh, int rw, s3r::ConvParams* q, int64_t* w_off, double* macs);
int geometry(const s3r_conv_desc* d, Geo* g);
int route(const s3r_conv_desc* d, Route* r);
int need_halo(const s3r_conv_desc* d, Route r);
int check_halos(const s3r_conv_desc* d, Route r);
int cout_pad(int cout);
int wino_mode();
bool wino_layer(const s3r_conv_desc* d);
bool dwino_layer(const s3r_conv_desc* d);
bool dwino3_layer(const s3r_conv_desc* d);
bool dwino3_desc_ok(const s3r_conv_desc* d);
int64_t dwino3_w_offset(const s3r_conv_desc* d);
struct Dwino3Need { int64_t diff, total; bool split; };
Dwino3Need dwino3_need(const s3r_conv_desc* d, int form);
bool wino_desc_ok(const s3r_conv_desc* d);
int wino2_ax(const s3r_conv_desc* d);
bool wino2_desc_ok(const s3r_conv_desc* d);
int wino2_max_edge();
int resolve_algo(const s3r_conv_desc* d, int* alg, int* form);
bool resolves_to_wino(const s3r_conv_desc* d);
Wino2Geo wino2_geo(const s3r_conv_desc* d);
int64_t wino_w_elems(const s3r_conv_desc* d);
int64_t wino_v_elems(const s3r_conv_desc* d);
int wino_bmax(const s3r_conv_desc* d);
int64_t dwino_w_elems(const s3r_conv_desc* d);
bool dwino_materialise(const s3r_conv_desc* d);
int64_t dwino_d_elems(const s3r_conv_desc* d);
int wino_kind(const s3r_conv_desc* d);
int wino_kcls(const s3r_conv_desc* d);
int64_t wino_positions(const s3r_conv_desc* d, int nb);
WinoNeed wino_need(const s3r_conv_desc* d, int form, bool head);
double wino_exec_flops(const s3r_conv_desc* d, const Geo& g);
int wino2_form_of(const s3r_conv_desc* d, int ntotal, int forced);
WinoNeed wino2_need(const s3r_conv_desc* d, int form);
double wino2_exec_flops(const s3r_conv_desc* d);
int cout_pad_h(int cout);
s3r::ConvParamsH make_params_h(const s3r_conv_desc* d, const Geo& g);
int resolve_launch_h(const s3r_conv_desc* d, s3r::ConvParamsH* p, LaunchH* L);
s3r::ConvParams make_params(const s3r_conv_desc* d, const Geo& g);
int resolve_launch(const s3r_conv_desc* d, s3r::ConvParams* p, Launch* L);
int64_t align_up(int64_t v, int64_t a);
int plan_chain(const s3r_layer* layers, int n, Plan* pl);

}
```

stereo-3d-reconstruction_amd/csrc/s3r_kernels.h:

```cpp
#pragma once
#include <hip/hip_runtime.h>
#include <stdint.h>
#include <atomic>

namespace s3r {

struct LdsAttr {
    std::atomic<unsigned long long> done{0};
    hipError_t ensure(const void* fn, int bytes) {
        int dev = 0;
        hipError_t e = hipGetDevice(&dev);
        if (e != hipSuccess) return e;
        if (dev >= 0 && dev < 64 && ((done.load(std::memory_order_relaxed) >> dev) & 1ull)) return hipSuccess;
        e = hipFuncSetAttribute(fn, hipFuncAttributeMaxDynamicSharedMemorySize, bytes);
        if (e == hipSuccess && dev >= 0 && dev < 64) done.fetch_or(1ull << dev, std::memory_order_relaxed);
        return e;
    }
};

inline int cu_count() {
    static std::atomic<int> cached[64];
    int dev = 0;
    if (hipGetDevice(&dev) != hipSuccess || dev < 0) { (void)hipGetLastError(); return 256; }
    int n = dev < 64 ? cached[dev].load(std::memory_order_relaxed) : 0;
    if (n > 0) return n;
    n = 0;
    if (hipDeviceGetAttribute(&n, hipDeviceAttributeMultiprocessorCount, dev) != hipSuccess || n <= 0) { (void)hipGetLastError(); n = 256; }
    if (dev < 64) cached[dev].store(n, std::memory_order_relaxed);
    return n;
}

struct AuxScope {
    void* impl;
    AuxScope(hipStream_t s, double bytes);
    ~AuxScope();
    AuxScope(const AuxScope&) = delete;
    AuxScope& operator=(const AuxScope&) = delete;
};

struct FastDiv {
    unsigned mul, shr;
    FastDiv() : mul(1), shr(0) {}
    explicit FastDiv(unsigned d) {
        shr = 0;
        while ((1ull << shr) < d) ++shr;
        mul = (unsigned)((((1ull << shr) - d) << 32) / d + 1);
    }
#if defined(__HIPCC__)
    __device__ __forceinline__ int div(int n) const { return (int)((__umulhi((unsigned)n, mul) + (unsigned)n) >> shr); }
#endif
};

#if defined(__HIPCC__)
__device__ __forceinline__ float render_f32(float v) { return v; }
__device__ __forceinline__ float render_f32(unsigned char u) {
    const float f = (float)u;
    const float rcp = 1.f / 255.f;
    const float q = __fmul_rn(f, rcp);
    return fmaf(fmaf(-q, 255.f, f), rcp, q);
}
#endif

struct ConvParams {
    const float* x;
    const float* w;
    const float* scale;
    const float* shift;
    float* y;
    int B, Cin, Cout, CoutPad;
    int Nd, Nh, Nw;
    FastDiv dS, dHW, dW;
    int kd, kh, kw, T;
    int stride;
    int dil;
    int x_cs, x_ds, x_hs;
    int x_org;
    int y_cs, y_ds, y_hs;
    int y_bs;
    int y_org;
    int y_step;
    int shuf_s, shuf_nd;
    FastDiv dSC, dS1;
    unsigned x_bytes;
    unsigned y_bytes;
    int transposed;
    int act;
    float slope;
    int Ntotal;
    int n_begin, n_end;
    int n_tiles, m_tiles;
    int n_cut, big_wgs;
    int ksplit;
    float* part;
    int debug;
    const float* head_w;
    const float* head_scale;
    const float* head_shift;
    int head_act;
    int x_cls, Hout, Dout, ncls;
    const float* xd;
    int xd_mode;
};

struct TClsEntry {
    int Nd, Nh, Nw, kd, kh, kw, T, x_org, y_org, Ntotal, wg_begin, w_off;
    FastDiv dS, dHW, dW;
};
constexpr int kTClsMax = 27;
struct TClsTable { int n; TClsEntry e[kTClsMax]; };
hipError_t launch_conv_tcls(const ConvParams& base, TClsTable tab, hipStream_t stream);

enum { WINO_SERIAL = 0, WINO_CP = 1, WINO_DUAL = 2 };
struct WinoLaunch { int mode, n_cut; };

struct ConvParamsH {
    const void* x;
    const void* w;
    const float* scale;
    const float* shift;
    void* y;
    float* part;
    int B, Cin, Cout, CoutPad;
    int Nd, Nh, Nw;
    FastDiv dS, dHW, dW, dDH, dH;
    int kd, kh, kw, T;
    int stride;
    int x_bs, x_ds, x_hs, x_ws;
    int x_org;
    int y_bs, y_ds, y_hs, y_ws;
    int y_org;
    unsigned x_bytes;
    int transposed, act, Ntotal;
    int m_tiles, n_tiles;
    int ksplit;
    int debug;
    const float* head_w;
    const float* head_scale;
    const float* head_shift;
    int head_act;
};

enum { ACT_NONE = 0, ACT_RELU = 1, ACT_SIGMOID = 2 };

hipError_t launch_conv_mfma(const ConvParams& p, int tile_code, hipStream_t stream);
int conv_pick_tile(const ConvParams& p);
int conv_pick_vec(const ConvParams& p);
int conv_pick_ksplit(const ConvParams& p, int tile_cfg);
int64_t conv_scratch_elems(const ConvParams& p, int tile_cfg);
int conv_num_tiles();
int conv_last_launch_count();
void conv_tile_dims(int tile_cfg, int* bm, int* bn);
hipError_t launch_pack_conv(const float* w, float* wp, int Cin, int Cout, int CoutPad, int T, int transposed,
                            hipStream_t s);
hipError_t launch_wino_input(const float* x, float* V, long long planes, int Hp, int Wp, int Hq, int R, hipStream_t s);
hipError_t launch_pack_wino(const float* w, float* wp, int Cin, int Cout, int CoutPad, int kd, int kw, int R, hipStream_t s);
WinoLaunch wino_plan(int kind, int cout, int kcls, int ntotal, bool head, int forced);
int64_t wino_slab_elems(int kind, int cout, int ntotal, const WinoLaunch& L);
hipError_t launch_conv_wino(ConvParams p, const WinoLaunch& L, hipStream_t stream, int* launches);
int wino2_classes(int ax);
int wino2_outputs(int ax);
hipError_t launch_wino2_input(const float* x, float* V, int ax, long long planes, int Dp, int Hp, int Wp, int SD, int SH, hipStream_t s);
hipError_t launch_wino2p_input(const float* x, float* V, int B, int Cin, int Hp, int Wp, int SH, int SW, long long npad, hipStream_t s);
hipError_t launch_pack_wino2(const float* w, float* wp, int ax, int Cin, int Cout, int CoutPad, hipStream_t s);
int wino2_form(int ax, int cout, int ntotal, int forced);
int64_t wino2_slab_elems(int ax, int cout, int ntotal, int form);
int64_t wino2_npad(int64_t ntotal);
hipError_t launch_conv_wino2(ConvParams p, int ax, int form, bool to_v, hipStream_t stream, int* launches);
hipError_t launch_cost_volume_wino2(const float* fl, const float* fr, float* V, int B, int C, int D, int H, int W, hipStream_t s);
int wino_bk();
hipError_t launch_wino_diff(const float* x, float* D, long long planes, int Dp, int Hp, int Wp, int three, hipStream_t s);
hipError_t launch_pack_wino_deconv(const float* w, float* wp, int Cin, int Cout, int CoutPad, hipStream_t s);
hipError_t launch_deconv_wino(ConvParams p, const WinoLaunch& L, hipStream_t stream, int* launches);
hipError_t launch_pack_dwino3(const float* w, float* wp, int Cin, int Cout, hipStream_t s);
int64_t dwino3_w_elems(int Cin, int Cout);
bool dwino3_edge_ok(int n);
int64_t dwino3_slab_elems(int cout, int ntotal);
bool dwino3_split(int cout, int ntotal, int forced);
hipError_t launch_deconv_wino3(ConvParams p, bool split, hipStream_t stream);
hipError_t launch_stem_wino(const void* x, const void* x2, int u8, int nsplit, const float* wt, const float* scale, const float* shift,
                            float* V, int N, int Hi, int Wi, int Ho, int Wo, hipStream_t s);
hipError_t launch_stem(const void* x, const void* x2, int u8, int nsplit, const float* w, const float* scale,
                       const float* shift, float* y, int N, int Hi, int Wi, int Ho, int Wo, int y_cs, int y_hs, int y_org,
                       hipStream_t s);
hipError_t launch_cost_volume(const float* fl, const float* fr, float* vol, int B, int C, int D, int H, int W,
                              int halo, hipStream_t s);
hipError_t launch_cost_volume_wino(const float* fl, const float* fr, float* V, int B, int C, int D, int H, int W, int R, hipStream_t s);
hipError_t launch_stage(const float* x, float* y, int B, int Cin, int CinPad, int nd, int n, int in_halo, int sp, int pe, int step,
                        hipStream_t s);
hipError_t launch_pack_general(const float* w, float* wp, int Cin, int CinPad, int Cout, int CoutPad, int T, int flip, hipStream_t s);
hipError_t launch_stage_im2col(const float* x, float* y, int B, int Cin, int KPad, int nd, int n, int in_halo, int n_out, int k, int stride,
                               int pad, int dil, hipStream_t s);
hipError_t launch_pack_tclass(const float* w, float* wp, int Cin, int CinPad, int Cout, int CoutPad, int nd, int k, int stride,
                              int rd, int rh, int rw, hipStream_t s);
hipError_t launch_act(float* y, long long total, int act, float param, hipStream_t s);
hipError_t launch_pad_copy(const float* x, float* y, int64_t planes, int D, int H, int W, int hd, int hh, int hw,
                           hipStream_t s);
hipError_t launch_pack_stem(const float* w, float* wt, hipStream_t s);
hipError_t launch_head(const float* x, const float* w, const float* scale, const float* shift, float* y, int B, int C,
                       int64_t S, int act, hipStream_t s);
hipError_t launch_chamfer(const float* p, const float* q, float* d1, float* d2, int* i1, int* i2,
                          int B, int N, int M, hipStream_t s);
hipError_t launch_chamfer_backward(const float* p, const float* q, const int* i1, const int* i2, const float* g1, const float* g2,
                                   float* gp, float* gq, int B, int N, int M, hipStream_t s);
hipError_t launch_linear(const float* x, const float* w, const float* scale, const float* bias, float* y, int B,
                         int Cin, int Cout, int act, float* scratch, hipStream_t s);
int64_t linear_scratch_elems(int B, int Cin, int Cout);
hipError_t launch_conv_bf16(const ConvParamsH& p, int tm, hipStream_t stream);
int conv_bf16_pick_tm(const ConvParamsH& p);
int conv_bf16_shape();
int conv_bf16_pick_ksplit(const ConvParamsH& p);
int64_t conv_bf16_scratch_elems(const ConvParamsH& p, int tm);
hipError_t launch_pack_bf16(const float* w, void* wp, int Cin, int Cout, int CoutPad, int T, int transposed, hipStream_t s);
hipError_t launch_stem_bf16(const void* x, const void* x2, int u8, int nsplit, const float* wt, const float* scale,
                            const float* shift, void* y, int N, int Hi, int Wi, int Ho, int Wo, int y_bs, int y_hs, int y_org,
                            hipStream_t s);
hipError_t launch_cost_volume_bf16(const void* fl, const void* fr, void* vol, int B, int C, int D, int H, int W, int halo,
                                   hipStream_t s);
hipError_t launch_head_bf16(const void* x, const float* w, const float* scale, const float* shift, float* y, int C,
                            int64_t voxels, int act, hipStream_t s);
hipError_t launch_cl_bf16_to_f32(const void* x, float* y, int N, int64_t S, int C, hipStream_t s);
hipError_t launch_iou(const float* pred, const float* gt, float th, float* iou, int B, int64_t S, hipStream_t s);
hipError_t launch_disparity_wta(const float* fl, const float* fr, float* dl, float* dr, int B, int C, int D, int H, int W,
                                hipStream_t s);
hipError_t launch_disparity_epe(const float* pred, const float* gt, float* epe, int* count, int B, int64_t S,
                                hipStream_t s);
size_t disparity_soft_lds_bytes(int C, int D, int W);
hipError_t launch_disparity_soft(const void* fl, const void* fr, int bf16, float* dl, float* dr, float* cl, float* cr, int B,
                                 int C, int D, int H, int W, float tau, int OH, int OW, float disp_scale, hipStream_t s);
hipError_t launch_disparity_metrics(const float* pred, const float* gt, float* epe, int* counts, int B, int64_t S,
                                    hipStream_t s);

#if defined(__HIPCC__)
template <int R>
__device__ __forceinline__ void wino_rows_to_classes(const float (&r)[R + 2], float (&v)[R + 2]) {
    static_assert(R == 4, "F(4,3)");
    v[0] = fmaf(4.f, r[0], fmaf(-5.f, r[2], r[4]));
    v[1] = fmaf(-4.f, r[1] + r[2], r[3] + r[4]);
    v[2] = fmaf(4.f, r[1] - r[2], r[4] - r[3]);
    v[3] = fmaf(2.f, r[3] - r[1], r[4] - r[2]);
    v[4] = fmaf(2.f, r[1] - r[3], r[4] - r[2]);
    v[5] = fmaf(4.f, r[1], fmaf(-5.f, r[3], r[5]));
}

#endif

}
```

stereo-3d-reconstruction_amd/csrc/s3r_plan.hip:

```cpp
#include "s3r_host.h"

#include <cstdarg>
#include <cstdio>
#include <cstdlib>
#include <cstring>

namespace s3rh {

thread_local char g_err[512] = "";

int fail(int code, const char* fmt, ...) {
    va_list ap;
    va_start(ap, fmt);
    vsnprintf(g_err, sizeof(g_err), fmt, ap);
    va_end(ap);
    return code;
}

int hip_fail(hipError_t e, const char* what) {
    return fail(S3R_ERR_HIP, "%s: %s", what, hipGetErrorString(e));
}

int64_t ipow(int64_t b, int e) {
    int64_t r = 1;
// ... 30 lines not shown
bool staged_layer(const s3r_conv_desc* d) {
    if (d->dtype != S3R_F32 || (d->op != S3R_OP_CONV && d->op != S3R_OP_DECONV) || (d->ndim != 2 && d->ndim != 3)) return false;
    if (stem_shape(d) || head_shape(d)) return false;
    if (d->op == S3R_OP_DECONV) return !(deconv_fast(d) && d->cin % 16 == 0);
    return d->cin % 16 != 0;
}
bool tclass_layer(const s3r_conv_desc* d) { return d->op == S3R_OP_DECONV && staged_layer(d) && dil_of(d) == 1; }
bool tclass_direct(const s3r_conv_desc* d) {
    return tclass_layer(d) && d->cin % 16 == 0 && d->in_halo >= tclass_halo(d) && d->in_layout == S3R_LAYOUT_PLAIN;
}
TClassAxis tclass_axis(const s3r_conv_desc* d, int r) {
    TClassAxis a;
    const int k = d->k, s = d->stride, p = d->pad, n_out = out_size(d);
    a.kr = r < k ? (k - r + s - 1) / s : 0;
    a.ke = a.kr > 0 ? a.kr : 1;
    a.qmin = p > r ? (p - r + s - 1) / s : 0;
    const int top = n_out - 1 + p - r;
    a.nq = top < 0 ? 0 : top / s - a.qmin + 1;
    return a;
}
int tclass_halo(const s3r_conv_desc* d) {
    int h = 0;
    for (int r = 0; r < d->stride; ++r) {
        const TClassAxis a = tclass_axis(d, r);
        if (a.nq <= 0) continue;
        const int lo = (a.ke - 1) - a.qmin, hi = a.qmin + a.nq - 1 - (d->in_size - 1);
        if (lo > h) h = lo;
        if (hi > h) h = hi;
    }
    return h;
}
bool tshuf_layer(const s3r_conv_desc* d) {
    return tclass_layer(d) && d->k == d->stride && d->stride >= 2 && d->pad == 0 && d->out_pad == 0;
}
int64_t tclass_w_elems(const s3r_conv_desc* d) {
    if (tshuf_layer(d)) return (int64_t)((d->cin + 15) / 16 * 16) * cout_pad(d->cout * (int)ipow(d->stride, d->ndim));
    int64_t per_axis = 0;
    for (int r = 0; r < d->stride; ++r) per_axis += tclass_axis(d, r).ke;
    return ipow(per_axis, d->ndim) * ((d->cin + 15) / 16 * 16) * cout_pad(d->cout);
}
bool im2col_layer(const s3r_conv_desc* d) {
    if (d->op != S3R_OP_CONV || !staged_layer(d) || d->cin > 8 || d->k > 16 || d->k < 2 || d->in_size > 4096) return false;
    const int no = out_size(d);
    if (no <= 0) return false;
    const double per_sample = ((double)d->cin * (double)ipow(d->k, d->ndim) + 15.0) * (d->ndim == 3 ? (double)no * no * no : (double)no * no);
    return per_sample * 4 <= 64.0 * (1 << 20);
}
StagedGeo staged_geo(const s3r_conv_desc* d) {
    StagedGeo s;
    s.bmax = 0;
    s.cin_pad = (d->cin + 15) / 16 * 16;
    if (im2col_layer(d)) {
        s.cin_pad = (d->cin * (int)ipow(d->k, d->ndim) + 15) / 16 * 16;
        s.step = 1; s.pe = 0;
        s.sp = out_size(d);
        const int64_t per_sample = (int64_t)s.cin_pad * ipow(s.sp, d->ndim);
        s.bmax = (int)(((int64_t)1 << 28) / per_sample);
        s.elems = (int64_t)(d->batch < s.bmax ? d->batch : s.bmax) * per_sample;
        return s;
    }
    if (tclass_layer(d)) {
        s.step = 1;
        s.pe = tclass_halo(d);
        s.sp = d->in_size + 2 * s.pe;
        s.elems = (int64_t)d->batch * s.cin_pad * ipow(s.sp, d->ndim);
        return s;
    }
    const bool tr = d->op == S3R_OP_DECONV;
    s.step = tr ? d->stride : 1;
    s.pe = tr ? dil_of(d) * (d->k - 1) - d->pad : d->pad;
    const int u = tr ? (d->in_size - 1) * d->stride + 1 + d->out_pad : d->in_size;
    s.sp = u + 2 * s.pe;
    s.elems = (int64_t)d->batch * s.cin_pad * ipow(s.sp, d->ndim);
    return s;
}

int geometry(const s3r_conv_desc* d, Geo* g) {
    if (!d) return fail(S3R_ERR_INVALID, "null descriptor");
    if (d->batch <= 0 || d->cin <= 0 || d->cout <= 0) return fail(S3R_ERR_INVALID, "batch/cin/cout must be positive");
    if (d->in_halo < 0 || d->out_halo < 0 || d->in_halo > 8 || d->out_halo > 8)
        return fail(S3R_ERR_INVALID, "halo must be in [0, 8]");
    if (d->dtype != S3R_F32 && d->dtype != S3R_BF16) return fail(S3R_ERR_INVALID, "unknown dtype %d", d->dtype);
    if ((d->in_layout != S3R_LAYOUT_PLAIN && d->in_layout != S3R_LAYOUT_WINO_H && d->in_layout != S3R_LAYOUT_WINO_DH &&
         d->in_layout != S3R_LAYOUT_WINO_HW) || (d->out_layout != S3R_LAYOUT_PLAIN && d->out_layout != S3R_LAYOUT_WINO_HW))
        return fail(S3R_ERR_INVALID, "unknown layout");
    if ((d->in_layout || d->out_layout) && d->op == S3R_OP_LINEAR)
        return fail(S3R_ERR_INVALID, "the transformed input layout exists on the convolution paths only");
    if (d->op == S3R_OP_LINEAR) {
        if (d->in_halo || d->out_halo) return fail(S3R_ERR_INVALID, "linear layers take no halo");
        if (d->act < S3R_ACT_NONE || d->act > S3R_ACT_TANH) return fail(S3R_ERR_INVALID, "unknown activation %d", d->act);
        g->nd = 0; g->in = g->out = g->in_p = g->out_p = 1; g->in_sp = 1; g->out_sp = 1;
        g->x_elems = (int64_t)d->batch * d->cin;
        g->y_elems = (int64_t)d->batch * d->cout;
        g->w_elems = (int64_t)d->cin * d->cout;
        g->x_store = g->x_elems; g->y_store = g->y_elems;
        g->flops = 2.0 * d->batch * (double)d->cin * d->cout;
        g->bytes = 4.0 * (g->x_elems + g->y_elems + g->w_elems);
        if (d->dtype != S3R_F32) return fail(S3R_ERR_INVALID, "linear layers exist on the fp32 path only");
        return S3R_OK;
    }
    if (d->op != S3R_OP_CONV && d->op != S3R_OP_DECONV) return fail(S3R_ERR_INVALID, "unknown op %d", d->op);
    if (d->ndim != 2 && d->ndim != 3) return fail(S3R_ERR_INVALID, "ndim must be 2 or 3");
    if (d->in_size <= 0 || d->k <= 0 || d->stride <= 0 || d->pad < 0) return fail(S3R_ERR_INVALID, "bad size/k/stride/pad");
    if (d->dilation < 0 || d->out_pad < 0) return fail(S3R_ERR_INVALID, "dilation / out_pad must not be negative");
    if (d->act < S3R_ACT_NONE || d->act > S3R_ACT_TANH) return fail(S3R_ERR_INVALID, "unknown activation %d", d->act);
    if (d->dtype == S3R_BF16 && (dil_of(d) != 1 || d->out_pad != 0 || d->act > S3R_ACT_SIGMOID || (d->op == S3R_OP_DECONV && !deconv_fast(d))))
        return fail(S3R_ERR_INVALID, "bf16 path: Conv with dilation 1 / ConvTranspose3d k4 s2 p1 and none / relu / sigmoid only (the "
                    "parameter-general layers are fp32)");
    if (d->op == S3R_OP_CONV && d->out_pad != 0) return fail(S3R_ERR_INVALID, "out_pad belongs to transposed convolutions");
    if (d->op == S3R_OP_DECONV && !deconv_fast(d)) {
        if (dil_of(d) * (d->k - 1) - d->pad < 0)
            return fail(S3R_ERR_INVALID, "ConvTranspose with pad %d > dilation * (k - 1) = %d crops more than the kernel reaches: not supported",
                        d->pad, dil_of(d) * (d->k - 1));
        if (d->out_pad >= (d->stride > dil_of(d) ? d->stride : dil_of(d)))
            return fail(S3R_ERR_INVALID, "out_pad %d must be smaller than max(stride, dilation)", d->out_pad);
    }
    if (staged_layer(d) && !im2col_layer(d)) {
        const bool tr = d->op == S3R_OP_DECONV && !tclass_layer(d);
        if (d->stride > 64 || d->k > 1024) return fail(S3R_ERR_INVALID, "stride / kernel size out of range");
        const double pe = tclass_layer(d) ? (double)tclass_halo(d) : tr ? (double)dil_of(d) * (d->k - 1) - d->pad : d->pad;
        const double sp = (tr ? ((double)d->in_size - 1) * d->stride + 1 + d->out_pad : d->in_size) + 2 * pe;
        const double est = (double)d->batch * ((d->cin + 15) / 16 * 16) * (d->ndim == 3 ? sp * sp * sp : sp * sp);
        if (est >= (double)kMaxElems || est * 4 >= (double)kMaxBytes)
            return fail(S3R_ERR_INVALID, "staged input too large for one call (>= 2^31 elements / 4 GiB): split the batch");
    }
    g->nd = d->ndim;
    g->in = d->in_size;
    g->out = out_size(d);
    if (g->out <= 0) return fail(S3R_ERR_INVALID, "empty output");
    g->in_p = g->in + 2 * d->in_halo;
    g->out_p = g->out + 2 * d->out_halo;
    g->in_sp = ipow(g->in, g->nd);
    g->out_sp = ipow(g->out, g->nd);
    g->x_elems = (int64_t)d->batch * d->cin * ipow(g->in_p, g->nd);
    g->y_elems = (int64_t)d->batch * d->cout * ipow(g->out_p, g->nd);
    if (d->in_layout == S3R_LAYOUT_WINO_H) {
        if (d->dtype != S3R_F32 || d->op != S3R_OP_CONV || d->stride != 1 || d->k != 3 || d->pad != 1 || (g->in & 1) || d->in_halo != 1 ||
            d->cin % 16 != 0 || d->cout <= 1)
            return fail(S3R_ERR_INVALID, "a Winograd-transformed input serves an fp32 Conv k=3 s=1 p=1 over an even edge, in_halo = 1");
        if (g->in % wino_r(d) != 0) return fail(S3R_ERR_INVALID, "a Winograd-transformed input needs an edge that is a multiple of %d", wino_r(d));
        g->x_elems = (wino_r(d) + 2) * (int64_t)d->batch * d->cin * (g->nd == 3 ? g->in_p : 1) * (g->in / wino_r(d)) * g->in_p;
    }
    if (d->in_layout == S3R_LAYOUT_WINO_DH) {
        if (d->dtype != S3R_F32 || d->op != S3R_OP_CONV || d->ndim != 3 || d->stride != 1 || d->k != 3 || d->pad != 1 || (g->in & 3) ||
            d->in_halo != 1 || d->cin % 32 != 0 || d->cout <= 1)
            return fail(S3R_ERR_INVALID, "a two-axis Winograd-transformed input serves an fp32 Conv3d k=3 s=1 p=1 over an edge %% 4 == 0, in_halo = 1");
        g->x_elems = 36 * (int64_t)d->batch * d->cin * (g->in / 4) * (g->in / 4) * g->in_p;
    }
    if (d->in_layout == S3R_LAYOUT_WINO_HW) {
        if (d->dtype != S3R_F32 || d->op != S3R_OP_CONV || d->ndim != 2 || d->stride != 1 || d->k != 3 || d->pad != 1 || (g->in & 3) ||
            d->in_halo != 1 || d->cin % 32 != 0 || d->cout <= 1)
            return fail(S3R_ERR_INVALID, "a two-axis Winograd-transformed input (2D) serves an fp32 Conv2d k=3 s=1 p=1 over an edge %% 4 == 0, in_halo = 1");
        g->x_elems = 36 * (int64_t)d->cin * s3r::wino2_npad((int64_t)d->batch * (g->in / 4) * (g->in / 4));
    }
    if (d->out_layout == S3R_LAYOUT_WINO_HW) {
        if (d->dtype != S3R_F32 || d->op != S3R_OP_CONV || d->ndim != 2 || (g->out & 3) || d->cout % 32 != 0 || d->act == S3R_ACT_SIGMOID)
            return fail(S3R_ERR_INVALID, "the two-axis Winograd output layout is written by an fp32 Conv2d with an output edge %% 4 == 0 and cout %% 32 == 0");
        g->y_elems = 36 * (int64_t)d->cout * s3r::wino2_npad((int64_t)d->batch * (g->out / 4) * (g->out / 4));
    }
    g->w_elems = (int64_t)d->cin * d->cout * ipow(d->k, g->nd);
    if (d->op == S3R_OP_DECONV)
        g->flops = 2.0 * d->batch * (double)d->cin * g->in_sp * d->cout * ipow(d->k, g->nd);
    else
        g->flops = 2.0 * d->batch * (double)d->cout * g->out_sp * d->cin * ipow(d->k, g->nd);
    const bool bf = d->dtype == S3R_BF16;
    const bool stem = d->ndim == 2 && d->cin == 3;
    const bool head = d->cout == 1 && d->k == 1;
    const int xs = (bf && !stem) ? 2 : 4, ys = (bf && !head) ? 2 : 4, wsz = bf && !stem && !head ? 2 : 4;
    g->x_store = (g->x_elems * xs + 3) / 4;
    g->y_store = (g->y_elems * ys + 3) / 4;
    g->bytes = (double)d->batch * (xs * d->cin * (double)g->in_sp + ys * d->cout * (double)g->out_sp) + wsz * (double)g->w_elems;
    if (g->x_elems >= kMaxElems || g->y_elems >= kMaxElems || g->x_elems * 4 >= kMaxBytes || g->y_elems * 4 >= kMaxBytes)
        return fail(S3R_ERR_INVALID, "tensor too large for one call (>= 2^31 elements / 4 GiB): split the batch");
    return S3R_OK;
}


int route(const s3r_conv_desc* d, Route* r) {
    if (d->op == S3R_OP_LINEAR) { *r = R_LINEAR; return S3R_OK; }
    if (stem_shape(d)) { *r = R_STEM; return S3R_OK; }
    if (head_shape(d)) { *r = R_HEAD; return S3R_OK; }
    if (d->dtype == S3R_BF16 ? d->cin % 32 == 0 : (d->cin % 16 == 0 || staged_layer(d))) { *r = R_MFMA; return S3R_OK; }
    return fail(S3R_ERR_INVALID, "no kernel for this layer shape (cin=%d cout=%d k=%d s=%d p=%d ndim=%d): the MFMA path "
                "needs cin %% 16 == 0", d->cin, d->cout, d->k, d->stride, d->pad, d->ndim);
}

int need_halo(const s3r_conv_desc* d, Route r) {
    if (r != R_MFMA || staged_layer(d)) return 0;
    return d->op == S3R_OP_DECONV ? 1 : d->pad;
}

int want_halo(const s3r_conv_desc* d, Route r) {
    if (r == R_MFMA && tclass_layer(d) && d->cin % 16 == 0 && tclass_halo(d) <= 8) return tclass_halo(d);
    return need_halo(d, r);
}

int check_halos(const s3r_conv_desc* d, Route r) {
    if ((d->in_layout || d->out_layout) && r != R_MFMA)
        return fail(S3R_ERR_INVALID, "the transformed input layout is read by the MFMA convolution kernels only");
    if (d->in_halo < need_halo(d, r))
        return fail(S3R_ERR_INVALID, "this layer's kernel reads its zero padding from memory: the input must carry a "
                    "zero halo of >= %d (got in_halo=%d); s3r_chain_forward pads unpadded inputs itself",
                    need_halo(d, r), d->in_halo);
    if ((r == R_STEM || r == R_HEAD) && d->in_halo != 0) return fail(S3R_ERR_INVALID, "stem / head kernels take an unpadded input");
    if (r == R_HEAD && d->out_halo != 0) return fail(S3R_ERR_INVALID, "head kernel writes an unpadded output");
    return S3R_OK;
}

int cout_pad(int cout) { return (cout + 127) / 128 * 128; }

int wino_mode() {
    static const int mode = getenv("S3R_WINO") ? atoi(getenv("S3R_WINO")) : 1;
    return mode;
}
bool wino_layer(const s3r_conv_desc* d) {
    return d->dtype != S3R_BF16 && d->op == S3R_OP_CONV && (d->ndim == 2 || d->ndim == 3) && d->k == 3 && d->stride == 1 &&
           d->pad == 1 && d->cin % s3r::wino_bk() == 0 && d->cout > 1 && d->in_size >= 4;
}
bool dwino_layer(const s3r_conv_desc* d) {
    return d->dtype != S3R_BF16 && deconv_fast(d) && d->cin % s3r::wino_bk() == 0 && d->in_size >= 4 && (d->in_size & 3) == 0;
}
bool dwino3_layer(const s3r_conv_desc* d) {
    return d->dtype != S3R_BF16 && deconv_fast(d) && d->cin % 16 == 0 && d->cout > 1 && s3r::dwino3_edge_ok(d->in_size);
}
bool dwino3_desc_ok(const s3r_conv_desc* d) {
    return dwino3_layer(d) && d->act < S3R_ACT_SIGMOID && d->in_halo == 1 && d->ksplit <= 1 && d->in_layout == S3R_LAYOUT_PLAIN &&
           d->out_layout == S3R_LAYOUT_PLAIN;
}
Dwino3Need dwino3_need(const s3r_conv_desc* d, int form) {
    Dwino3Need n;
    n.diff = (3 * (int64_t)d->batch * d->cin * ipow(d->in_size + 2, 3) + 255) / 256 * 256;
    const int ntotal = d->batch * (int)ipow(d->in_size / 2, 3);
    n.split = s3r::dwino3_split(d->cout, ntotal, form);
    n.total = n.diff + ((n.split || form < 0) ? (s3r::dwino3_slab_elems(d->cout, ntotal) + 255) / 256 * 256 : 0);
    return n;
}
int64_t dwino3_w_offset(const s3r_conv_desc* d) {
    return 64 * (int64_t)d->cin * cout_pad(d->cout) + (dwino_layer(d) ? dwino_w_elems(d) : 0);
}
bool wino_desc_ok(const s3r_conv_desc* d) {
    if (!(wino_layer(d) || dwino_layer(d)) || d->act >= S3R_ACT_SIGMOID || d->in_halo != 1 || d->ksplit > 1 || dil_of(d) != 1) return false;
    if (d->out_layout != S3R_LAYOUT_PLAIN) return false;
    return d->in_layout == S3R_LAYOUT_PLAIN || (d->in_layout == S3R_LAYOUT_WINO_H && wino_layer(d));
}
int wino2_ax(const s3r_conv_desc* d) {
    if (d->dtype == S3R_BF16 || d->op != S3R_OP_CONV || d->stride != 1 || d->cin % s3r::wino_bk() != 0 || d->cout <= 1) return -1;
    if (d->ndim == 2) return d->k == 3 && d->pad == 1 && d->in_size >= 4 && d->in_size <= 124 ? 2 : -1;
    if (d->ndim != 3) return -1;
    if (d->k == 3 && d->pad == 1 && d->in_size >= 4) return 0;
    if (d->k == 4 && d->pad == 0 && d->in_size >= 5) return 1;
    return -1;
}
bool wino2_desc_ok(const s3r_conv_desc* d) {
    return wino2_ax(d) >= 0 && d->act < S3R_ACT_SIGMOID && dil_of(d) == 1 && d->in_halo == d->pad && d->ksplit <= 1 &&
           (d->in_layout == S3R_LAYOUT_PLAIN || (d->in_layout == S3R_LAYOUT_WINO_DH && wino2_ax(d) == 0 && d->in_size % 4 == 0) ||
            (d->in_layout == S3R_LAYOUT_WINO_HW && wino2_ax(d) == 2 && d->in_size % 4 == 0)) &&
           (d->out_layout == S3R_LAYOUT_PLAIN || (d->out_layout == S3R_LAYOUT_WINO_HW && wino2_ax(d) == 2 && d->in_size % 4 == 0));
}
int wino2_max_edge() {
    static const int e = getenv("S3R_WINO2_MAX_EDGE") ? atoi(getenv("S3R_WINO2_MAX_EDGE")) : 28;
    return e;
}
bool leaky_fused(const s3r_conv_desc* d) {
    return d->dtype == S3R_F32 && d->op != S3R_OP_LINEAR && d->act == S3R_ACT_LEAKY_RELU && d->act_param >= 0.f && d->act_param <= 1.f;
}
bool needs_act_pass(const s3r_conv_desc* d) { return d->act > S3R_ACT_SIGMOID && !leaky_fused(d); }

int resolve_algo(const s3r_conv_desc* d, int* alg, int* form) {
    *alg = ALG_DIRECT;
    *form = -1;
    if (d->algo != S3R_ALGO_AUTO && d->algo != S3R_ALGO_DIRECT && d->algo != S3R_ALGO_WINOGRAD)
        return fail(S3R_ERR_INVALID, "unknown algo %d", d->algo);
    if (staged_layer(d) || d->act > S3R_ACT_SIGMOID || dil_of(d) != 1) {
        if (d->algo == S3R_ALGO_WINOGRAD) return fail(S3R_ERR_INVALID, "algo = WINOGRAD: a parameter-general layer (staged input, dilation, "
                                                      "LeakyReLU / ELU / Tanh) has no Winograd form");
        if (d->in_layout != S3R_LAYOUT_PLAIN || d->out_layout != S3R_LAYOUT_PLAIN)
            return fail(S3R_ERR_INVALID, "a parameter-general layer reads and writes plain layouts");
        return S3R_OK;
    }
    if (d->algo == S3R_ALGO_WINOGRAD && d->tile >= 6 && d->tile <= 8) {
        if (!dwino3_desc_ok(d))
            return fail(S3R_ERR_INVALID, "algo = WINOGRAD, tile = 6: the three-axis form serves an fp32 ConvTranspose3d k4 s2 p1 over an edge of "
                        "8, 16 or 32 with cin %% 16 == 0 (in_halo = 1, plain layouts, no split-K, no sigmoid)");
        *alg = ALG_WINO3;
        *form = d->tile == 6 ? -1 : d->tile == 7 ? 1 : 0;
        return S3R_OK;
    }
    if (d->algo == S3R_ALGO_WINOGRAD) {
        const bool one = wino_desc_ok(d), two = wino2_desc_ok(d);
        if ((d->tile >= 3 && !two) || (d->tile >= 0 && d->tile <= 2 && !one) || (!one && !two) || d->tile > 5 ||
            (d->tile == 5 && (wino2_ax(d) == 1 || (wino2_ax(d) == 0 && d->in_size > 60))))
            return fail(S3R_ERR_INVALID, "algo = WINOGRAD: this layer / descriptor has no such Winograd form (one-axis: fp32 Conv k3 s1 p1 "
                        "with cin %% %d == 0 and edge >= 4, or ConvTranspose3d k4 s2 p1 over an edge %% 4 == 0, in_halo = 1; two-axis "
                        "(tile = 3): Conv3d k3 s1 p1 / k4 s1 p0, in_halo = pad; plain layouts, no split-K, no sigmoid)", s3r::wino_bk());
        const bool two_io = d->in_layout == S3R_LAYOUT_WINO_DH || d->in_layout == S3R_LAYOUT_WINO_HW || d->out_layout == S3R_LAYOUT_WINO_HW;
        if (two_io && !(two && (d->tile < 0 || d->tile >= 3)))
            return fail(S3R_ERR_INVALID, "a two-axis transformed input / output runs the two-axis kernel only");
        if (d->tile >= 3 || !one || two_io ||
            (d->tile < 0 && two && d->in_layout == S3R_LAYOUT_PLAIN && d->in_size <= wino2_max_edge())) {
            *alg = ALG_WINO2;
            *form = d->tile >= 4 ? d->tile - 4 : -1;
        } else { *alg = ALG_WINO; *form = d->tile; }
        return S3R_OK;
    }
    if (d->in_layout == S3R_LAYOUT_WINO_DH || d->in_layout == S3R_LAYOUT_WINO_HW || d->out_layout == S3R_LAYOUT_WINO_HW) {
        if (d->algo == S3R_ALGO_DIRECT || !wino2_desc_ok(d) || d->tile >= 0)
            return fail(S3R_ERR_INVALID, "a two-axis transformed input / output runs the two-axis kernel only: algo AUTO / WINOGRAD, no direct "
                        "tile / split-K override");
        *alg = ALG_WINO2;
        return S3R_OK;
    }
    if (d->in_layout == S3R_LAYOUT_WINO_H) {
        if (d->algo == S3R_ALGO_DIRECT || !wino_desc_ok(d) || d->tile >= 0)
            return fail(S3R_ERR_INVALID, "a Winograd-transformed input runs the Winograd kernel only: algo AUTO / WINOGRAD, no direct tile / "
                        "split-K override, a plain output");
        *alg = ALG_WINO;
        return S3R_OK;
    }
    if (d->algo == S3R_ALGO_DIRECT || d->tile >= 0 || d->ksplit >= 1 || wino_mode() <= 0) return S3R_OK;
    if (wino2_desc_ok(d) && d->in_size <= wino2_max_edge()) *alg = ALG_WINO2;
    else if (d->op == S3R_OP_DECONV && dwino3_desc_ok(d) && d->in_size >= 16) *alg = ALG_WINO3;
    else if (wino_desc_ok(d)) *alg = ALG_WINO;
    return S3R_OK;
}
bool resolves_to_wino(const s3r_conv_desc* d) {
    int a, f;
    return resolve_algo(d, &a, &f) == S3R_OK && a != ALG_DIRECT;
}
Wino2Geo wino2_geo(const s3r_conv_desc* d) {
    Wino2Geo w;
    w.ax = wino2_ax(d);
    w.m = s3r::wino2_outputs(w.ax);
    w.ncls = s3r::wino2_classes(w.ax);
    w.out = out_size(d);
    w.sg = (w.out + w.m - 1) / w.m;
    w.wp = d->in_size + 2 * d->in_halo;
    w.kw = w.ax == 2 ? 1 : d->k;
    w.w_elems = (int64_t)w.ncls * w.kw * d->cin * cout_pad(d->cout);
    w.v_sample = w.ax == 2 ? (int64_t)w.ncls * d->cin * (w.sg * w.sg + 64) : (int64_t)w.ncls * d->cin * w.sg * w.sg * w.wp;
    w.pos_sample = w.ax == 2 ? (int64_t)w.sg * w.sg : (int64_t)w.sg * w.sg * w.out;
    const int64_t mx = w.v_sample > 0 ? (((int64_t)1 << 31) - 1) / (4 * w.v_sample) : 0;
    w.bmax = (int)(mx < d->batch ? mx : d->batch);
    w.n = 0;
    return w;
}
int64_t wino_w_elems(const s3r_conv_desc* d) {
    return (wino_r(d) + 2) * ipow(3, d->ndim - 1) * d->cin * (int64_t)cout_pad(d->cout);
}
int64_t wino_v_elems(const s3r_conv_desc* d) {
    const int R = wino_r(d);
    const int64_t dp = d->ndim == 3 ? d->in_size + 2 : 1, hq = (d->in_size + R - 1) / R, wp = d->in_size + 2;
    return (R + 2) * (int64_t)d->batch * d->cin * dp * hq * wp;
}
int wino_bmax(const s3r_conv_desc* d) {
    const int64_t v_sample = wino_v_elems(d) / (d->batch > 0 ? d->batch : 1);
    const int64_t m = v_sample > 0 ? (((int64_t)1 << 31) - 1) / (4 * v_sample) : 0;
    return (int)(m < d->batch ? m : d->batch);
}
int64_t dwino_w_elems(const s3r_conv_desc* d) { return 72 * 2 * (int64_t)d->cin * cout_pad(d->cout); }
bool dwino_materialise(const s3r_conv_desc* d) {
    static const int forced = getenv("S3R_DWINO_MAT") ? atoi(getenv("S3R_DWINO_MAT")) : -1;
    if (forced >= 0) return forced != 0;
    return 4 * 4 * (int64_t)d->batch * d->cin * ipow(d->in_size + 2, 3) <= (int64_t)192 << 20;
}
int64_t dwino_d_elems(const s3r_conv_desc* d) {
    return (dwino_materialise(d) ? 3 : 1) * (int64_t)d->batch * d->cin * ipow(d->in_size + 2, 3);
}

int wino_kind(const s3r_conv_desc* d) { return d->op == S3R_OP_DECONV ? 2 : 1; }
int wino_kcls(const s3r_conv_desc* d) {
    return d->cin * (d->op == S3R_OP_DECONV ? 2 : (d->ndim == 3 ? 9 : 3));
}
int64_t wino_positions(const s3r_conv_desc* d, int nb) {
    const int n = d->in_size;
    if (d->op == S3R_OP_DECONV) return (int64_t)nb * (n / 2) * (n / 2) * n;
    const int R = wino_r(d);
    return (int64_t)nb * (d->ndim == 3 ? n : 1) * ((n + R - 1) / R) * n;
}
WinoNeed wino_need(const s3r_conv_desc* d, int form, bool head) {
    WinoNeed w = {0, 0, 0};
    if (d->batch <= 0) return w;
    const int kind = wino_kind(d);
    if (d->op == S3R_OP_DECONV) {
        w.v = dwino_d_elems(d);
        const int nt = (int)wino_positions(d, d->batch);
        w.slab = s3r::wino_slab_elems(kind, d->cout, nt, s3r::wino_plan(kind, d->cout, wino_kcls(d), nt, head, form < 0 ? 1 : form));
    } else {
        const int bmax = wino_bmax(d);
        if (bmax <= 0) return w;
        if (d->in_layout != S3R_LAYOUT_WINO_H) w.v = wino_v_elems(d) / d->batch * bmax;
        for (int b0 = 0; b0 < d->batch; b0 += bmax) {
            const int nb = d->batch - b0 < bmax ? d->batch - b0 : bmax;
            if (b0 > 0 && nb == bmax) continue;
            const int nt = (int)wino_positions(d, nb);
            const int64_t sl = s3r::wino_slab_elems(kind, d->cout, nt, s3r::wino_plan(kind, d->cout, wino_kcls(d), nt, false, form < 0 ? 1 : form));
            if (sl > w.slab) w.slab = sl;
        }
    }
    w.v = (w.v + 255) / 256 * 256;
    w.total = w.v + w.slab;
    return w;
}
double wino_exec_flops(const s3r_conv_desc* d, const Geo& g) {
    if (d->op == S3R_OP_DECONV) return g.flops * 0.5625;
    const int R = wino_r(d);
    const double taps = (d->ndim == 3 ? 3.0 : 1.0) * 3.0 * (R + 2);
    return 2.0 * (double)wino_positions(d, d->batch) * d->cout * d->cin * taps;
}

int wino2_form_of(const s3r_conv_desc* d, int ntotal, int forced) {
    if (forced < 0 && wino2_ax(d) == 0 && d->in_size > 60) forced = 0;
    return s3r::wino2_form(wino2_ax(d), d->cout, ntotal, forced);
}
WinoNeed wino2_need(const s3r_conv_desc* d, int form) {
    WinoNeed w = {0, 0, 0};
    const Wino2Geo g2 = wino2_geo(d);
    if (d->batch <= 0 || g2.bmax <= 0) return w;
    if (d->in_layout != S3R_LAYOUT_WINO_DH && d->in_layout != S3R_LAYOUT_WINO_HW)
        w.v = ((g2.ax == 2 ? g2.ncls * d->cin * s3r::wino2_npad(g2.pos_sample * g2.bmax) : g2.v_sample * g2.bmax) + 255) / 256 * 256;
    for (int b0 = 0; b0 < d->batch; b0 += g2.bmax) {
        const int nb = d->batch - b0 < g2.bmax ? d->batch - b0 : g2.bmax;
        if (b0 > 0 && nb == g2.bmax) continue;
        const int nt = (int)(g2.pos_sample * nb);
        const int64_t sl = s3r::wino2_slab_elems(g2.ax, d->cout, nt, form < 0 ? 0 : wino2_form_of(d, nt, form));
        if (sl > w.slab) w.slab = sl;
    }
    w.total = w.v + w.slab;
    return w;
}
double wino2_exec_flops(const s3r_conv_desc* d) {
    const Wino2Geo g2 = wino2_geo(d);
    return 2.0 * (double)g2.pos_sample * d->batch * g2.ncls * d->cout * d->cin * g2.kw;
}
int cout_pad_h(int cout) { return (cout + 63) / 64 * 64; }

s3r::ConvParamsH make_params_h(const s3r_conv_desc* d, const Geo& g) {
    s3r::ConvParamsH p;
    memset(&p, 0, sizeof(p));
    const bool is3 = d->ndim == 3;
    p.B = d->batch; p.Cin = d->cin; p.Cout = d->cout; p.CoutPad = cout_pad_h(d->cout);
    p.act = d->act;
    p.x_ws = d->cin; p.x_hs = g.in_p * d->cin; p.x_ds = is3 ? g.in_p * g.in_p * d->cin : 0;
    p.x_bs = (int)ipow(g.in_p, g.nd) * d->cin;
    p.y_ws = d->cout; p.y_hs = g.out_p * d->cout; p.y_ds = is3 ? g.out_p * g.out_p * d->cout : 0;
    p.y_bs = (int)ipow(g.out_p, g.nd) * d->cout;
    p.y_org = d->out_halo * (p.y_ds + p.y_hs + p.y_ws);
    p.x_bytes = (unsigned)(g.x_elems * 2);
    if (d->op == S3R_OP_DECONV) {
        p.transposed = 1;
        p.Nd = g.in; p.Nh = g.in; p.Nw = g.in;
        p.kd = p.kh = p.kw = 2; p.T = 8;
        p.stride = 1;
        p.x_org = d->in_halo * (p.x_ds + p.x_hs + p.x_ws);
    } else {
        p.transposed = 0;
        p.Nd = is3 ? g.out : 1; p.Nh = g.out; p.Nw = g.out;
        p.kd = is3 ? d->k : 1; p.kh = d->k; p.kw = d->k; p.T = p.kd * p.kh * p.kw;
        p.stride = d->stride;
        p.x_org = (d->in_halo - d->pad) * (p.x_ds + p.x_hs + p.x_ws);
    }
    p.Ntotal = p.B * p.Nd * p.Nh * p.Nw;
    p.dS = s3r::FastDiv((unsigned)(p.Nd * p.Nh * p.Nw));
    p.dHW = s3r::FastDiv((unsigned)(p.Nh * p.Nw));
    p.dW = s3r::FastDiv((unsigned)p.Nw);
    p.dDH = s3r::FastDiv((unsigned)(p.Nd * p.Nh));
    p.dH = s3r::FastDiv((unsigned)p.Nh);
    p.ksplit = 1;
    return p;
}


int resolve_launch_h(const s3r_conv_desc* d, s3r::ConvParamsH* p, LaunchH* L) {
    const int chunks = d->cin / 32;
    if (d->ksplit < 0 || (d->ksplit > 0 && chunks % d->ksplit != 0))
        return fail(S3R_ERR_INVALID, "ksplit=%d must divide cin/32=%d", d->ksplit, chunks);
    L->ksplit = d->ksplit > 0 ? d->ksplit : s3r::conv_bf16_pick_ksplit(*p);
    p->ksplit = L->ksplit;
    if (d->tile >= 0 && d->tile != 1 && d->tile != 2 && d->tile != 3 && d->tile != 19 && d->tile != 4 && d->tile != 5 && d->tile != 6 && d->tile != 9 &&
        d->tile != 10 && d->tile != 17 && d->tile != 18 && d->tile != 20 && d->tile != 21 && d->tile != 22 && d->tile != 23 &&
        d->tile != 40)
        return fail(S3R_ERR_INVALID, "bf16 path: tile must be -1 (auto), 1, 2, 4 (x128 positions, per-tap gather), 3 (128 x 128 couts), 5, 6 "
                    "(x128 positions = 1, 2, plane-reuse gather) or 9, 10 (row-reuse gather); per-tap / plane + 16 = "
                    "32-channel K tiles; 40 (row-persistent e2)");
    L->tm = d->tile >= 0 ? d->tile : s3r::conv_bf16_pick_tm(*p);
    return S3R_OK;
}

s3r::ConvParams make_params(const s3r_conv_desc* d, const Geo& g) {
    s3r::ConvParams p;
    memset(&p, 0, sizeof(p));
    const bool is3 = d->ndim == 3;
    p.B = d->batch; p.Cin = d->cin; p.Cout = d->cout; p.CoutPad = cout_pad(d->cout);
    p.act = d->act;
    p.x_hs = g.in_p; p.x_ds = is3 ? g.in_p * g.in_p : 0; p.x_cs = (int)ipow(g.in_p, g.nd);
    p.y_hs = g.out_p; p.y_ds = is3 ? g.out_p * g.out_p : 0; p.y_cs = (int)ipow(g.out_p, g.nd);
    p.y_org = d->out_halo * (p.y_ds + p.y_hs + 1);
    p.y_bs = d->cout * p.y_cs;
    p.x_bytes = (unsigned)(g.x_elems * 4);
    p.y_bytes = (unsigned)(g.y_elems * 4);
    if (d->op == S3R_OP_DECONV) {
        p.transposed = 1;
// ... 63 lines not shown
    p.Nd = is3 ? d->in_size : 1; p.Nh = d->in_size; p.Nw = d->in_size;
    p.kd = p.kh = p.kw = 1; p.T = 1;
    p.stride = 1; p.dil = 1;
    p.y_step = s;
    p.shuf_s = s; p.shuf_nd = d->ndim;
    p.dSC = s3r::FastDiv((unsigned)sc);
    p.dS1 = s3r::FastDiv((unsigned)s);
    p.Ntotal = p.B * p.Nd * p.Nh * p.Nw;
    p.dS = s3r::FastDiv((unsigned)(p.Nd * p.Nh * p.Nw));
    p.dHW = s3r::FastDiv((unsigned)(p.Nh * p.Nw));
    p.dW = s3r::FastDiv((unsigned)p.Nw);
    p.ksplit = 1;
    return p;
}

bool make_params_tclass(const s3r_conv_desc* d, const Geo& g, int rd, int rh, int rw, s3r::ConvParams* q, int64_t* w_off, double* macs) {
    const bool is3 = d->ndim == 3;
    StagedGeo sg = staged_geo(d);
    if (tclass_direct(d)) {
        sg.pe = d->in_halo;
        sg.sp = d->in_size + 2 * d->in_halo;
        sg.elems = (int64_t)d->batch * sg.cin_pad * ipow(sg.sp, d->ndim);
    }
    const int s = d->stride, h = sg.pe;
    const TClassAxis ad = is3 ? tclass_axis(d, rd) : TClassAxis{1, 1, 0, 1}, ah = tclass_axis(d, rh), aw = tclass_axis(d, rw);
    int64_t taps_before = 0;
    {
        int64_t sum_ke = 0;
        for (int r = 0; r < s; ++r) sum_ke += tclass_axis(d, r).ke;
        int64_t kd_before = 0, kh_before = 0, kw_before = 0;
        for (int r = 0; r < rd; ++r) kd_before += tclass_axis(d, r).ke;
        for (int r = 0; r < rh; ++r) kh_before += tclass_axis(d, r).ke;
        for (int r = 0; r < rw; ++r) kw_before += tclass_axis(d, r).ke;
        taps_before = (is3 ? kd_before * sum_ke * sum_ke : 0) + (int64_t)ad.ke * kh_before * sum_ke + (int64_t)ad.ke * ah.ke * kw_before;
    }
    *w_off = taps_before * sg.cin_pad * cout_pad(d->cout);
    if (ad.nq <= 0 || ah.nq <= 0 || aw.nq <= 0) return false;
    s3r::ConvParams p = make_params(d, g);
    p.Cin = sg.cin_pad;
    p.transposed = 0;
    p.x_hs = sg.sp; p.x_ds = is3 ? sg.sp * sg.sp : 0; p.x_cs = (int)ipow(sg.sp, g.nd);
    p.x_bytes = (unsigned)(sg.elems * 4);
    p.Nd = is3 ? ad.nq : 1; p.Nh = ah.nq; p.Nw = aw.nq;
    p.kd = is3 ? ad.ke : 1; p.kh = ah.ke; p.kw = aw.ke; p.T = p.kd * p.kh * p.kw;
    p.stride = 1; p.dil = 1;
    p.x_org = (is3 ? (h + ad.qmin - (ad.ke - 1)) * p.x_ds : 0) + (h + ah.qmin - (ah.ke - 1)) * p.x_hs + (h + aw.qmin - (aw.ke - 1));
    p.y_step = s;
    p.y_org += (is3 ? (s * ad.qmin + rd - d->pad) * p.y_ds : 0) + (s * ah.qmin + rh - d->pad) * p.y_hs + (s * aw.qmin + rw - d->pad);
    p.Ntotal = p.B * p.Nd * p.Nh * p.Nw;
    p.dS = s3r::FastDiv((unsigned)(p.Nd * p.Nh * p.Nw));
    p.dHW = s3r::FastDiv((unsigned)(p.Nh * p.Nw));
    p.dW = s3r::FastDiv((unsigned)p.Nw);
    p.ksplit = 1;
    *macs = (double)p.Ntotal * p.T * (double)sg.cin_pad * d->cout;
    *q = p;
    return true;
}


int resolve_launch(const s3r_conv_desc* d, s3r::ConvParams* p, Launch* L) {
    const int chunks = d->cin / 16;
    if (d->ksplit < 0 || (d->ksplit > 0 && chunks % d->ksplit != 0))
        return fail(S3R_ERR_INVALID, "ksplit=%d must divide cin/16=%d", d->ksplit, chunks);
    L->ksplit = d->ksplit > 0 ? d->ksplit : s3r::conv_pick_ksplit(*p, 0);
    p->ksplit = L->ksplit;
    const int code = d->tile >= 0 ? d->tile : 15;
    L->cfg = code & 15;
    L->vec = code >> 4;
    if (L->cfg != 15 && L->cfg >= s3r::conv_num_tiles()) return fail(S3R_ERR_INVALID, "unknown tile configuration %d", L->cfg);
    if (L->cfg == 15) L->cfg = s3r::conv_pick_tile(*p);
    const int vmax = s3r::conv_pick_vec(*p);
    const int vec = (L->vec == 1 || L->vec == 4) && L->vec <= vmax ? L->vec : vmax;
    int bm, bn;
    s3r::conv_tile_dims(L->cfg, &bm, &bn);
    if (bn > 256 * vec)
        return fail(S3R_ERR_INVALID, "tile configuration %d (%d positions) needs the 16-byte gather: rows of a multiple of 4 positions, "
                    "stride 1", L->cfg, bn);
    return S3R_OK;
}


int64_t align_up(int64_t v, int64_t a) { return (v + a - 1) / a * a; }

int plan_chain(const s3r_layer* layers, int n, Plan* pl) {
    if (!layers || n <= 0) return fail(S3R_ERR_INVALID, "empty chain");
    pl->d.resize(n); pl->r.resize(n); pl->g.resize(n); pl->off.assign(n, -1); pl->fuse_head.assign(n, 0);
    for (int i = 0; i < n; ++i) {
        pl->d[i] = layers[i].desc;
        if (i > 0) pl->d[i].in_layout = S3R_LAYOUT_PLAIN;
        if (i + 1 < n) pl->d[i].out_layout = S3R_LAYOUT_PLAIN;
        int rc = route(&pl->d[i], &pl->r[i]);
        if (rc) return rc;
    }
    const int need0 = need_halo(&pl->d[0], pl->r[0]);
    pl->pad_input = pl->d[0].in_halo < need0;
    const int user_in_halo = pl->d[0].in_halo;
    if (pl->pad_input) pl->d[0].in_halo = need0;
    for (int i = 0; i < n; ++i) {
        if (i > 0) pl->d[i].in_halo = pl->d[i - 1].out_halo;
        if (i + 1 < n) {
            const s3r_conv_desc& a = pl->d[i];
            const s3r_conv_desc& b = pl->d[i + 1];
            const bool carries = pl->r[i] != R_LINEAR && pl->r[i] != R_HEAD && out_size(&a) == b.in_size && a.cout == b.cin;
            pl->d[i].out_halo = carries ? want_halo(&b, pl->r[i + 1]) : need_halo(&b, pl->r[i + 1]);
        }
        if (i == 1 && pl->r[0] == R_STEM && pl->r[1] == R_MFMA && pl->d[1].dtype == S3R_F32 && pl->d[1].op == S3R_OP_CONV) {
            static const int fuse = getenv("S3R_STEM_WINO") ? atoi(getenv("S3R_STEM_WINO")) : 1;
            int alg, form;
            const bool fits = pl->d[0].in_size % 16 == 0 && pl->d[0].in_size <= 236;
            if (fuse && fits && resolve_algo(&pl->d[1], &alg, &form) == S3R_OK && alg == ALG_WINO &&
                pl->d[1].in_size % wino_r(&pl->d[1]) == 0 && wino_bmax(&pl->d[1]) >= pl->d[1].batch) {
                pl->stem_wino = true;
                pl->d[1].in_layout = S3R_LAYOUT_WINO_H;
            }
        }
        if (i > 0 && pl->r[i - 1] == R_MFMA && pl->r[i] == R_MFMA && pl->d[i].dtype == S3R_F32) {
            static const int fuse = getenv("S3R_WINO_HANDOFF") ? atoi(getenv("S3R_WINO_HANDOFF")) : 1;
            s3r_conv_desc& a = pl->d[i - 1];
            s3r_conv_desc& b = pl->d[i];
            int alg_a, alg_b, form;
            if (fuse && wino2_ax(&a) == 2 && wino2_ax(&b) == 2 && a.cout == b.cin && out_size(&a) == b.in_size && b.in_size % 4 == 0 &&
                resolve_algo(&a, &alg_a, &form) == S3R_OK && alg_a == ALG_WINO2 && resolve_algo(&b, &alg_b, &form) == S3R_OK &&
                alg_b == ALG_WINO2 && wino2_geo(&a).bmax >= a.batch && wino2_geo(&b).bmax >= b.batch) {
                a.out_layout = S3R_LAYOUT_WINO_HW;
                b.in_layout = S3R_LAYOUT_WINO_HW;
                const int rg = geometry(&a, &pl->g[i - 1]);
                if (rg) return rg;
            }
        }
        int rc = geometry(&pl->d[i], &pl->g[i]);
        if (rc) return rc;
        if ((rc = check_halos(&pl->d[i], pl->r[i]))) return rc;
        if (pl->d[i].dtype != pl->d[0].dtype) return fail(S3R_ERR_INVALID, "all layers of a chain must share one dtype");
        if (i > 0) {
            const s3r_conv_desc& a = pl->d[i - 1];
            const int64_t prev_out = (int64_t)a.cout * pl->g[i - 1].out_sp, cur_in = (int64_t)pl->d[i].cin * pl->g[i].in_sp;
            if (prev_out != cur_in || a.batch != pl->d[i].batch)
                return fail(S3R_ERR_INVALID, "layer %d input (%lld/sample) does not match layer %d output (%lld/sample)", i,
                            (long long)cur_in, i - 1, (long long)prev_out);
            if (pl->d[i].in_halo && (pl->g[i - 1].out != pl->g[i].in || a.cout != pl->d[i].cin))
                return fail(S3R_ERR_INVALID, "layer %d needs a halo but reshapes layer %d's output", i, i - 1);
        }
    }
    for (int i = 0; i + 1 < n; ++i) {
        if (pl->r[i] != R_MFMA || pl->r[i + 1] != R_HEAD || pl->d[i].cout > 64) continue;
        if (pl->d[i + 1].cin != pl->d[i].cout || pl->d[i].out_halo != 0 || pl->d[i].act >= S3R_ACT_SIGMOID || staged_layer(&pl->d[i])) continue;
        if (pl->d[i].op == S3R_OP_CONV && resolves_to_wino(&pl->d[i])) continue;
        if (pl->d[i].dtype == S3R_BF16) {
            s3r::ConvParamsH ph = make_params_h(&pl->d[i], pl->g[i]);
            LaunchH Lh;
            if (resolve_launch_h(&pl->d[i], &ph, &Lh) != S3R_OK || Lh.ksplit != 1) continue;
        } else {
            int alg, form;
            if (resolve_algo(&pl->d[i], &alg, &form) != S3R_OK) continue;
            if (alg == ALG_DIRECT) {
                s3r::ConvParams p = make_params(&pl->d[i], pl->g[i]);
                Launch L;
                if (resolve_launch(&pl->d[i], &p, &L) != S3R_OK || L.ksplit != 1) continue;
            }
        }
        pl->fuse_head[i] = 1;
    }
    int64_t off = 0;
    if (pl->pad_input && pl->d[0].in_layout != S3R_LAYOUT_PLAIN)
        return fail(S3R_ERR_INVALID, "a transformed chain input must come with its halo (in_halo = 1)");
    if (pl->pad_input) {
        if (user_in_halo != 0) return fail(S3R_ERR_INVALID, "chain input halo %d is smaller than the %d its first layer needs",
                                           user_in_halo, need0);
        pl->pad_off = 0;
        off = align_up(pl->g[0].x_store, 256);
    }
    for (int i = 0; i + 1 < n; ++i) {
        pl->off[i] = off;
        if (i == 0 && pl->stem_wino) off = align_up(off + pl->g[1].x_store, 256);
        else if (!pl->fuse_head[i]) off = align_up(off + pl->g[i].y_store, 256);
    }
    for (int i = 0; i < n; ++i) {
        const int64_t sc = s3r_conv_scratch_elems(&pl->d[i]);
        if (sc < 0) return (int)sc;
        if (sc > pl->scratch_elems) pl->scratch_elems = sc;
    }
    pl->scratch_off = off;
    off = align_up(off + pl->scratch_elems, 256);
    pl->total = off;
    return S3R_OK;
}

}

using namespace s3rh;

extern "C" {

int s3r_conv_out_size(const s3r_conv_desc* d) {
    if (!d) return fail(S3R_ERR_INVALID, "null descriptor");
    if (d->op == S3R_OP_LINEAR) return 1;
    if (d->op != S3R_OP_CONV && d->op != S3R_OP_DECONV) return fail(S3R_ERR_INVALID, "unknown op %d", d->op);
    if (d->in_size <= 0 || d->k <= 0 || d->stride <= 0 || d->pad < 0)
        return fail(S3R_ERR_INVALID, "bad size/k/stride/pad (in_size=%d k=%d stride=%d pad=%d)", d->in_size, d->k, d->stride, d->pad);
    const int n = out_size(d);
    if (n <= 0) return fail(S3R_ERR_INVALID, "empty output");
    return n;
}

int s3r_conv_packed_elems(const s3r_conv_desc* d, int64_t* elems) {
    Geo g; Route r;
    int rc = geometry(d, &g);
    if (rc) return rc;
    if ((rc = route(d, &r))) return rc;
    if (!elems) return fail(S3R_ERR_INVALID, "null output");
    switch (r) {
        case R_STEM: *elems = 27 * 32; break;
        case R_HEAD: *elems = d->cin; break;
        case R_LINEAR: *elems = g.w_elems; break;
        case R_MFMA: {
            if (tclass_layer(d)) { *elems = tclass_w_elems(d); break; }
            if (im2col_layer(d)) { *elems = (int64_t)staged_geo(d).cin_pad * cout_pad(d->cout); break; }
            if (staged_layer(d)) { *elems = ipow(d->k, g.nd) * staged_geo(d).cin_pad * cout_pad(d->cout); break; }
            const int64_t taps = d->op == S3R_OP_DECONV ? 64 : ipow(d->k, g.nd);
            if (d->dtype == S3R_BF16) *elems = (taps * d->cin * cout_pad_h(d->cout) + 1) / 2;
            else *elems = taps * d->cin * cout_pad(d->cout) + (wino_layer(d) ? wino_w_elems(d) : 0) + (dwino_layer(d) ? dwino_w_elems(d) : 0) +
                          (wino2_ax(d) >= 0 ? wino2_geo(d).w_elems : 0) + (dwino3_layer(d) ? s3r::dwino3_w_elems(d->cin, d->cout) : 0);
            break;
        }
    }
    return S3R_OK;
}

int64_t s3r_conv_scratch_elems(const s3r_conv_desc* d) {
    Geo g; Route r;
    int rc = geometry(d, &g);
    if (rc) return rc;
    if ((rc = route(d, &r))) return rc;
    if (r == R_LINEAR) return s3r::linear_scratch_elems(d->batch, d->cin, d->cout);
    if (r != R_MFMA) return 0;
    if (d->dtype == S3R_BF16) {
        s3r::ConvParamsH ph = make_params_h(d, g);
        LaunchH Lh;
        if ((rc = resolve_launch_h(d, &ph, &Lh))) return rc;
        return s3r::conv_bf16_scratch_elems(ph, Lh.tm);
    }
    int alg, form;
    if ((rc = resolve_algo(d, &alg, &form))) return rc;
    if (tclass_direct(d)) return 0;
    if (staged_layer(d)) return (staged_geo(d).elems + 255) / 256 * 256;
    if (alg == ALG_WINO3) return dwino3_need(d, form).total;
    if (alg == ALG_WINO) return wino_need(d, form, false).total;
    if (alg == ALG_WINO2) return wino2_need(d, form).total;
    s3r::ConvParams p = make_params(d, g);
    Launch L;
    if ((rc = resolve_launch(d, &p, &L))) return rc;
    return s3r::conv_scratch_elems(p, L.cfg);
}

}

extern "C" {

int64_t s3r_chain_workspace_elems(const s3r_layer* layers, int n_layers) {
    Plan pl;
    int rc = plan_chain(layers, n_layers, &pl);
// ... 47 lines not shown
```

Measured before the change: 8772.

## Hand off 3D Winograd transformed operands directly between consecutive decoder layers

Adds new layouts (WINO_3D, DIFF) and a handoff kernel. A producer layer's split-K or class-parallel finish pass now writes the consumer's Winograd input transform or difference tensors directly, instead of writing a plain output that the next layer re-reads and transforms. This is meant to remove a separate transform launch and a round trip through global memory for the 3D decoder chain. In exchange the planner logic grows and can need extra workspace, and the transform is staged in shared memory per batch and channel block, which may limit parallelism.

```diff
diff --git a/include/s3r.h b/include/s3r.h
--- a/include/s3r.h
+++ b/include/s3r.h
@@ -31,7 +31,8 @@
 typedef enum s3r_act { S3R_ACT_NONE = 0, S3R_ACT_RELU = 1, S3R_ACT_SIGMOID = 2,
                        S3R_ACT_LEAKY_RELU = 3, S3R_ACT_ELU = 4, S3R_ACT_TANH = 5  } s3r_act;
 
-typedef enum s3r_layout { S3R_LAYOUT_PLAIN = 0, S3R_LAYOUT_WINO_H = 2, S3R_LAYOUT_WINO_DH = 3, S3R_LAYOUT_WINO_HW = 4 } s3r_layout;
+typedef enum s3r_layout { S3R_LAYOUT_PLAIN = 0, S3R_LAYOUT_WINO_H = 2, S3R_LAYOUT_WINO_DH = 3, S3R_LAYOUT_WINO_HW = 4,
+                          S3R_LAYOUT_WINO_3D = 5, S3R_LAYOUT_DIFF = 6 } s3r_layout;
 
 typedef enum s3r_algo { S3R_ALGO_AUTO = 0, S3R_ALGO_DIRECT = 1, S3R_ALGO_WINOGRAD = 2 } s3r_algo;
 
diff --git a/stereo-3d-reconstruction_amd/_lib.py b/stereo-3d-reconstruction_amd/_lib.py
--- a/stereo-3d-reconstruction_amd/_lib.py
+++ b/stereo-3d-reconstruction_amd/_lib.py
@@ -123,7 +123,7 @@
     return rc
 
 
-LAYOUT_PLAIN, LAYOUT_WINO_H, LAYOUT_WINO_DH, LAYOUT_WINO_HW = 0, 2, 3, 4
+LAYOUT_PLAIN, LAYOUT_WINO_H, LAYOUT_WINO_DH, LAYOUT_WINO_HW, LAYOUT_WINO_3D, LAYOUT_DIFF = 0, 2, 3, 4, 5, 6
 
 
 def make_desc(layer, batch, in_size, tag=0, tile=-1, in_halo=0, out_halo=0, ksplit=0, dtype=0, in_layout=0, out_layout=0,
diff --git a/stereo-3d-reconstruction_amd/csrc/s3r_api.hip b/stereo-3d-reconstruction_amd/csrc/s3r_api.hip
--- a/stereo-3d-reconstruction_amd/csrc/s3r_api.hip
+++ b/stereo-3d-reconstruction_amd/csrc/s3r_api.hip
@@ -17,9 +17,14 @@
               int64_t scratch_elems, int form, hipStream_t s, int* launches) {
     const Wino2Geo g2 = wino2_geo(d);
     const WinoNeed need = wino2_need(d, form);
-    const bool pre = d->in_layout == S3R_LAYOUT_WINO_DH || d->in_layout == S3R_LAYOUT_WINO_HW;
+    const bool pre = d->in_layout == S3R_LAYOUT_WINO_DH || d->in_layout == S3R_LAYOUT_WINO_HW ||
+                     d->in_layout == S3R_LAYOUT_WINO_3D;
     const bool to_v = d->out_layout == S3R_LAYOUT_WINO_HW;
-    if (g2.bmax <= 0 || ((pre || to_v) && g2.bmax < d->batch))
+    p.out_mode = d->out_layout == S3R_LAYOUT_WINO_3D ? (d->out_halo ? 1 : 2) : d->out_layout == S3R_LAYOUT_DIFF ? 3 : 0;
+    if (p.out_mode && (g2.ax > 1 || wino2_form_of(d, (int)(g2.pos_sample * d->batch), form) != 0))
+        return fail(S3R_ERR_INVALID, "a consumer's operand is written from the class-parallel launch form of a 3D two-axis layer only (the semi-fused "
+                    "form of this batch keeps the plain output: s3r_chain_forward plans that itself)");
+    if (g2.bmax <= 0 || ((pre || to_v || p.out_mode) && g2.bmax < d->batch))
         return fail(S3R_ERR_INVALID, "two-axis Winograd form: the transformed input of this batch exceeds 2 GiB (at most %d samples per "
                     "call with a producer-written input: s3r_conv_wino_input_elems)", g2.bmax);
     if (!scratch || scratch_elems < need.total)
@@ -80,16 +85,19 @@
         return fail(S3R_ERR_WORKSPACE, "the Winograd form of this transposed convolution needs %lld floats of scratch "
                     "(s3r_conv_scratch_elems), got %lld", (long long)need.total, (long long)(scratch ? scratch_elems : 0));
     const int n = d->in_size;
-    p.xd_mode = dwino_materialise(d) ? 1 : 0;
-    hipError_t e;
-    {
-        const double x_el = (double)d->batch * d->cin * (double)ipow(n + 2, 3);
-        s3r::AuxScope aux(s, 4.0 * x_el * (p.xd_mode ? 4.0 : 2.0));
+    const bool pre = d->in_layout == S3R_LAYOUT_DIFF;
+    const int64_t x_plain = (int64_t)d->batch * d->cin * ipow(n + 2, 3);
+    p.xd_mode = pre || dwino_materialise(d) ? 1 : 0;
+    hipError_t e = hipSuccess;
+    if (!pre) {
+        s3r::AuxScope aux(s, 4.0 * (double)x_plain * (p.xd_mode ? 4.0 : 2.0));
         e = s3r::launch_wino_diff(x, scratch, (long long)d->batch * d->cin, n + 2, n + 2, n + 2, p.xd_mode, s);
     }
     if (e != hipSuccess) return hip_fail(e, "Winograd difference-tensor launch");
     p.x = x;
-    p.xd = scratch;
+    p.xd = pre ? x + x_plain : scratch;
+    p.x_bytes = (unsigned)(4 * x_plain);
+    p.out_mode = d->out_layout == S3R_LAYOUT_DIFF ? 3 : 0;
     p.part = scratch + need.v;
     p.w = packed_w + 64 * (int64_t)d->cin * cout_pad(d->cout);
     p.Nd = n / 2; p.Nh = n / 2;
@@ -100,10 +108,13 @@
     p.dW = s3r::FastDiv((unsigned)p.Nw);
     p.ksplit = 1;
     const s3r::WinoLaunch L = s3r::wino_plan(2, d->cout, wino_kcls(d), p.Ntotal, p.head_w != nullptr, form);
+    if (p.out_mode && (L.mode != s3r::WINO_CP || p.head_w))
+        return fail(S3R_ERR_INVALID, "a consumer's difference tensors are written from the class-parallel launch form of the transposed Winograd "
+                    "layer only (the form of this batch keeps the plain output: s3r_chain_forward plans that itself)");
     int nl = 0;
     e = s3r::launch_deconv_wino(p, L, s, &nl);
     if (e != hipSuccess) return hip_fail(e, "Winograd transposed-conv launch");
-    *launches = 1 + nl;
+    *launches = (pre ? 0 : 1) + nl;
     *ran = 1 + L.mode;
     return S3R_OK;
 }
@@ -553,6 +564,14 @@
             }
             Launch L;
             if ((rc = resolve_launch(d, &p, &L))) return rc;
+            if (d->in_layout != S3R_LAYOUT_PLAIN || d->out_layout == S3R_LAYOUT_DIFF || d->out_layout == S3R_LAYOUT_WINO_HW)
+                return fail(S3R_ERR_INVALID, "the direct kernel reads a plain input and writes a plain output or (split-K) its consumer's two-axis plane sets");
+            if (d->out_layout == S3R_LAYOUT_WINO_3D) {
+                if (L.ksplit <= 1 || d->op != S3R_OP_CONV || needs_act_pass(d) || p.act == S3R_ACT_SIGMOID)
+                    return fail(S3R_ERR_INVALID, "a direct layer writes its consumer's plane sets from its split-K finish pass only (convolution, "
+                                "ksplit > 1, no activation pass behind it)");
+                p.out_mode = d->out_halo ? 1 : 2;
+            }
             if (L.ksplit > 1) {
                 const int64_t need = s3r::conv_scratch_elems(p, L.cfg);
                 if (scratch && scratch_elems >= need) p.part = scratch;
diff --git a/stereo-3d-reconstruction_amd/csrc/s3r_conv_glds.hip b/stereo-3d-reconstruction_amd/csrc/s3r_conv_glds.hip
--- a/stereo-3d-reconstruction_amd/csrc/s3r_conv_glds.hip
+++ b/stereo-3d-reconstruction_amd/csrc/s3r_conv_glds.hip
@@ -650,7 +650,12 @@
         dim3 grid(p.m_tiles * p.n_tiles * (p.transposed ? 8 : 1), 1, p.ksplit);
         hipLaunchKernelGGL((conv_glds_kernel<WM, WN, TM, TN, VEC, HEAD, NBUF>), grid, dim3(256), lds, stream, p);
         hipError_t e = hipGetLastError();
-        if (e == hipSuccess && p.ksplit > 1) e = launch_conv_finish(p, p.n_tiles * BN, stream);
+        if (e == hipSuccess && p.ksplit > 1) {
+            if (p.out_mode) {
+                g_launch_count += 1;
+                e = launch_wino_handoff(p, 3, p.out_mode - 1, p.n_tiles * BN, stream);
+            } else e = launch_conv_finish(p, p.n_tiles * BN, stream);
+        }
         return e;
     }
 }
@@ -781,6 +786,7 @@
     if (vec > vmax) vec = vmax;
     if (p.Cin % GBK != 0 || p.Ntotal % vec != 0) return hipErrorInvalidValue;
     if (p.ksplit < 1 || (p.Cin / GBK) % p.ksplit != 0 || (p.ksplit > 1 && !p.part)) return hipErrorInvalidValue;
+    if (p.out_mode && (p.ksplit <= 1 || p.head_w || p.transposed)) return hipErrorInvalidValue;
     if (p.head_w) {
         int bm, bn;
         conv_tile_dims(cfg, &bm, &bn);
diff --git a/stereo-3d-reconstruction_amd/csrc/s3r_conv_wino.hip b/stereo-3d-reconstruction_amd/csrc/s3r_conv_wino.hip
--- a/stereo-3d-reconstruction_amd/csrc/s3r_conv_wino.hip
+++ b/stereo-3d-reconstruction_amd/csrc/s3r_conv_wino.hip
@@ -792,6 +792,7 @@
 template <int VEC, int KIND>
 static hipError_t launch_wino_forms(ConvParams p, const WinoLaunch& L, hipStream_t stream) {
     const int ntotal = p.Ntotal;
+    if (p.out_mode && (KIND != 2 || L.mode != WINO_CP)) return hipErrorInvalidValue;
     auto lds_of = [](int bn) { return (size_t)WNB * WBK * (WBM + (KIND == 2 ? 2 : 1) * bn) * sizeof(float); };
     const int pcs = KIND == 2 ? 8 : 1;
     constexpr int NCLS = WinoKind<KIND>::NCLS;
@@ -837,6 +838,7 @@
     }
     hipError_t e = hipGetLastError();
     if (e != hipSuccess) return e;
+    if (p.out_mode) return launch_wino_handoff(p, 2, p.out_mode - 1, cp_tiles * WCN, stream);
     AuxScope aux(stream, 4.0 * (double)(ntotal - n0) * p.Cout * (pcs * NCLS + (p.head_w ? 0.0 : pcs * WinoKind<KIND>::R)));
     return launch_wino_finish<KIND>(p, n0, ntotal, cp_tiles * WCN, stream);
 }
@@ -1319,6 +1321,220 @@
     }
 }
 
+template <int PROD, int CONS>
+__global__ __launch_bounds__(256) void wino_handoff_kernel(const ConvParams p, const int npad, const int CB, const int On, const int halo,
+                                                           const int SG, const FastDiv dG1, const FastDiv dG2, const FastDiv dOp,
+                                                           const FastDiv dOp2, const FastDiv dSG) {
+    extern __shared__ __attribute__((aligned(16))) float hsm[];
+    const int tid = threadIdx.x;
+    const int Op = On + 2 * halo, hs = Op, ds = Op * Op, vol = ds * Op, org = halo * (ds + hs + 1);
+    const int S = p.Nd * p.Nh * p.Nw;
+    const int G1 = PROD == 2 ? 8 * S : S;
+    const int G2 = CONS == 2 ? vol : SG * SG * Op;
+    const int ncb = (p.Cout + CB - 1) / CB;
+    const float lo = p.act == ACT_RELU ? 0.f : -__builtin_inff();
+    const bool vec2 = CONS == 2 && (Op & 1) == 0 && (reinterpret_cast<size_t>(p.y) & 7) == 0;
+    for (int item = blockIdx.x; item < p.B * ncb; item += gridDim.x) {
+        const int b = item / ncb;
+        const int c0 = (item - b * ncb) * CB;
+        const int nc = p.Cout - c0 < CB ? p.Cout - c0 : CB;
+        for (int i = tid; i < nc * vol; i += 256) hsm[i] = 0.f;
+        __syncthreads();
+        for (int t = tid; t < nc * G1; t += 256) {
+            const int cl = dG1.div(t);
+            int g = t - cl * G1;
+            const int mrow = c0 + cl;
+            const float sc = p.scale ? p.scale[mrow] : 1.f, sf = p.shift ? p.shift[mrow] : 0.f;
+            float* __restrict__ o = hsm + cl * vol + org;
+            if constexpr (PROD <= 1) {
+                constexpr int N = WAxis<PROD>::N, M = WAxis<PROD>::M;
+                const int n = b * S + g;
+                const int sd = p.dHW.div(g);
+                g -= sd * p.Nh * p.Nw;
+                const int sh = p.dW.div(g);
+                const int pw = g - sh * p.Nw;
+                const float* __restrict__ src = p.part + ((size_t)mrow * (npad >> 6) + (n >> 6)) * (N * N * 64) + (n & 63);
+                float tt[N][M];
+#pragma unroll
+                for (int a = 0; a < N; ++a) {
+                    float m[N], y[M];
+#pragma unroll
+                    for (int c = 0; c < N; ++c) m[c] = src[(a * N + c) * 64];
+                    wax_at<PROD>(m, y);
+#pragma unroll
+                    for (int v = 0; v < M; ++v) tt[a][v] = y[v];
+                }
+                o += M * sd * ds + M * sh * hs + pw;
+#pragma unroll
+                for (int v = 0; v < M; ++v) {
+                    float m[N], y[M];
+#pragma unroll
+                    for (int a = 0; a < N; ++a) m[a] = tt[a][v];
+                    wax_at<PROD>(m, y);
+#pragma unroll
+                    for (int u = 0; u < M; ++u)
+                        if (M * sd + u < p.Dout && M * sh + v < p.Hout) o[u * ds + v * hs] = wino_act(y[u], sc, sf, lo);
+                }
+            } else if constexpr (PROD == 2) {
+                constexpr int NCLS = WinoKind<2>::NCLS, R = WinoKind<2>::R;
+                const int pc = p.dS.div(g);
+                g -= pc * S;
+                const int rd = (pc >> 2) & 1, rh = (pc >> 1) & 1, rw = pc & 1;
+                const int n = b * S + g;
+                const int pd = p.dHW.div(g);
+                g -= pd * p.Nh * p.Nw;
+                const int q = p.dW.div(g);
+                const int pw = g - q * p.Nw;
+                const float* __restrict__ src = p.part + (size_t)pc * NCLS * 64 + ((size_t)mrow * (npad >> 6) + (n >> 6)) * (8 * NCLS * 64) + (n & 63);
+                float m[NCLS], y[R];
+#pragma unroll
+                for (int c = 0; c < NCLS; ++c) m[c] = src[c * 64];
+                wino_out<2>(m, y);
+                o += (2 * pd * ds + 2 * q * hs + pw) * 2 + rd * ds + rh * hs + rw;
+#pragma unroll
+                for (int k = 0; k < R; ++k) o[wino_out_off<2>(k, ds, hs)] = wino_act(y[k], sc, sf, lo);
+            } else {
+                const int n = b * S + g;
+                const float* __restrict__ src = p.part + (size_t)mrow * npad + n;
+                const size_t zs = (size_t)p.Cout * npad;
+                float sum = src[0];
+                for (int z = 1; z < p.ksplit; ++z) sum += src[(size_t)z * zs];
+                const int pd = p.dHW.div(g);
+                g -= pd * p.Nh * p.Nw;
+                const int ph = p.dW.div(g);
+                const int pw = g - ph * p.Nw;
+                float t1 = fmaf(sum, sc, sf);
+                if (p.act == ACT_RELU) t1 = fmaxf(t1, fmaf(t1, p.slope, 0.f));
+                o[pd * ds + ph * hs + pw] = t1;
+            }
+        }
+        __syncthreads();
+        const size_t base = ((size_t)b * p.Cout + c0) * G2;
+        const size_t total = (size_t)p.B * p.Cout * G2;
+        for (int t = tid; t < (CONS == 2 && vec2 ? 0 : nc * G2); t += 256) {
+            const int cl = dG2.div(t);
+            const int e = t - cl * G2;
+            if constexpr (CONS <= 1) {
+                constexpr int N = WAxis<CONS>::N, M = WAxis<CONS>::M;
+                const int row = dOp.div(e);
+                const int w = e - row * Op;
+                const int sd = dSG.div(row);
+                const int sh = row - sd * SG;
+                const float* __restrict__ src = hsm + cl * vol + M * sd * ds + M * sh * hs + w;
+                float tt[N][N];
+#pragma unroll
+                for (int a = 0; a < N; ++a) {
+                    float r[N], v[N];
+#pragma unroll
+                    for (int c = 0; c < N; ++c) r[c] = (M * sd + a < Op && M * sh + c < Op) ? src[a * ds + c * hs] : 0.f;
+                    wax_bt<CONS>(r, v);
+#pragma unroll
+                    for (int c = 0; c < N; ++c) tt[a][c] = v[c];
+                }
+#pragma unroll
+                for (int c = 0; c < N; ++c) {
+                    float r[N], v[N];
+#pragma unroll
+                    for (int a = 0; a < N; ++a) r[a] = tt[a][c];
+                    wax_bt<CONS>(r, v);
+#pragma unroll
+                    for (int a = 0; a < N; ++a) p.y[(size_t)(a * N + c) * total + base + t] = v[a];
+                }
+            } else if (!vec2) {
+                const int z = dOp2.div(e);
+                const int r = dOp.div(e - z * ds);
+                const bool rn = r + 1 < Op, zn = z + 1 < Op;
+                const float* __restrict__ src = hsm + t;
+                const float x00 = src[0];
+                const float x01 = rn ? src[hs] : 0.f;
+                const float dh0 = rn ? x00 - x01 : 0.f;
+                const float x10 = zn ? src[ds] : 0.f;
+                const float x11 = (rn && zn) ? src[ds + hs] : 0.f;
+                const float dh1 = rn ? x10 - x11 : 0.f;
+                float* __restrict__ dst = p.y + base + t;
+                dst[0] = x00;
+                dst[total] = dh0;
+                dst[2 * total] = zn ? x00 - x10 : 0.f;
+                dst[3 * total] = zn ? dh0 - dh1 : 0.f;
+            }
+        }
+        if constexpr (CONS == 2) {
+            if (vec2)
+                for (int t = tid * 2; t < nc * G2; t += 512) {
+                    const int cl = dG2.div(t);
+                    const int e = t - cl * G2;
+                    const int z = dOp2.div(e);
+                    const int r = dOp.div(e - z * ds);
+                    const bool rn = r + 1 < Op, zn = z + 1 < Op;
+                    const wv2f zero = {0.f, 0.f};
+                    const float* __restrict__ src = hsm + t;
+                    const wv2f x00 = *reinterpret_cast<const wv2f*>(src);
+                    const wv2f x01 = rn ? *reinterpret_cast<const wv2f*>(src + hs) : zero;
+                    const wv2f dh0 = rn ? x00 - x01 : zero;
+                    const wv2f x10 = zn ? *reinterpret_cast<const wv2f*>(src + ds) : zero;
+                    const wv2f x11 = (rn && zn) ? *reinterpret_cast<const wv2f*>(src + ds + hs) : zero;
+                    const wv2f dh1 = rn ? x10 - x11 : zero;
+                    float* __restrict__ dst = p.y + base + t;
+                    *reinterpret_cast<wv2f*>(dst) = x00;
+                    *reinterpret_cast<wv2f*>(dst + total) = dh0;
+                    *reinterpret_cast<wv2f*>(dst + 2 * total) = zn ? x00 - x10 : zero;
+                    *reinterpret_cast<wv2f*>(dst + 3 * total) = zn ? dh0 - dh1 : zero;
+                }
+        }
+        __syncthreads();
+    }
+}
+
+hipError_t launch_wino_handoff(const ConvParams& p, int prod, int cons, int npad, hipStream_t stream) {
+    if (prod < 0 || prod > 3 || cons < 0 || cons > 2 || !p.part || !p.y || npad <= 0 || (npad & 63) || p.head_w) return hipErrorInvalidValue;
+    const int Op = p.y_hs;
+    if (Op <= 0 || p.y_ds != Op * Op || p.y_cs != Op * Op * Op || p.y_bs != p.Cout * p.y_cs) return hipErrorInvalidValue;
+    const int halo = p.y_org / (p.y_ds + p.y_hs + 1), On = Op - 2 * halo;
+    if (p.y_org != halo * (p.y_ds + p.y_hs + 1) || On <= 0) return hipErrorInvalidValue;
+    if ((cons == 0 && (halo != 1 || On < 4)) || (cons == 1 && (halo != 0 || On < 5)) || (cons == 2 && (halo != 1 || (On & 3)))) return hipErrorInvalidValue;
+    const int SG = cons == 0 ? (On + 3) / 4 : cons == 1 ? (On - 2) / 2 : 1;
+    const int vol = Op * Op * Op;
+    if (vol > 8192) return hipErrorInvalidValue;
+    const int CB = 8192 / vol < 8 ? 8192 / vol : 8;
+    const int S = p.Nd * p.Nh * p.Nw;
+    if (p.Ntotal != p.B * S || npad < p.Ntotal) return hipErrorInvalidValue;
+    double slabs;
+    if (prod <= 1) {
+        if (p.ncls != wino2_classes(prod) || p.Dout != On || p.Hout != On || p.Nw != On || p.act == ACT_SIGMOID) return hipErrorInvalidValue;
+        slabs = (double)p.ncls * npad;
+    } else if (prod == 2) {
+        if (!p.transposed || cons != 2 || 2 * p.Nw != On || 4 * p.Nd != On || 4 * p.Nh != On || p.act == ACT_SIGMOID) return hipErrorInvalidValue;
+        slabs = 72.0 * npad;
+    } else {
+        if (p.transposed || cons == 2 || p.ksplit <= 1 || p.y_step > 1 || p.shuf_s || p.Nd != On || p.Nh != On || p.Nw != On || p.act == ACT_SIGMOID)
+            return hipErrorInvalidValue;
+        slabs = (double)p.ksplit * npad;
+    }
+    const int G1 = prod == 2 ? 8 * S : S, G2 = cons == 2 ? vol : SG * SG * Op;
+    const double written = cons == 2 ? 4.0 * p.B * vol : (double)wino2_classes(cons) * p.B * G2;
+    if ((double)p.Cout * written >= 2147483648.0) return hipErrorInvalidValue;
+    const long long items = (long long)p.B * ((p.Cout + CB - 1) / CB);
+    const dim3 grid((unsigned)(items < 16384 ? items : 16384));
+    const size_t lds = (size_t)CB * vol * sizeof(float);
+    const FastDiv dG1((unsigned)G1), dG2((unsigned)G2), dOp((unsigned)Op), dOp2((unsigned)(Op * Op)), dSG((unsigned)SG);
+    AuxScope aux(stream, 4.0 * (double)p.Cout * (slabs + written));
+#define S3R_HANDOFF(PR, CO) hipLaunchKernelGGL((wino_handoff_kernel<PR, CO>), grid, dim3(256), lds, stream, p, npad, CB, On, halo, SG, dG1, dG2, dOp, dOp2, dSG)
+    switch (prod * 3 + cons) {
+        case 0: S3R_HANDOFF(0, 0); break;
+        case 1: S3R_HANDOFF(0, 1); break;
+        case 2: S3R_HANDOFF(0, 2); break;
+        case 3: S3R_HANDOFF(1, 0); break;
+        case 4: S3R_HANDOFF(1, 1); break;
+        case 5: S3R_HANDOFF(1, 2); break;
+        case 8: S3R_HANDOFF(2, 2); break;
+        case 9: S3R_HANDOFF(3, 0); break;
+        case 10: S3R_HANDOFF(3, 1); break;
+        default: return hipErrorInvalidValue;
+    }
+#undef S3R_HANDOFF
+    return hipGetLastError();
+}
+
 int wino2_form(int ax, int cout, int ntotal, int forced) {
     if (ax == 1) return 0;
     if (forced >= 0) return forced ? 1 : 0;
@@ -1345,6 +1561,7 @@
     const size_t lds = (size_t)WNB * WBK * (WBM + WCN) * sizeof(float);
     const int halo = to_v ? 1 : (p.y_hs - p.Hout) / 2;
     if (to_v && (ax != 2 || p.Hout % 4 != 0)) return hipErrorInvalidValue;
+    if (p.out_mode && (to_v || ax == 2 || form != 0)) return hipErrorInvalidValue;
     if (!to_v && (halo < 0 || p.y_hs != p.Hout + 2 * halo)) return hipErrorInvalidValue;
     if (ax == 2) {
         const int plane = to_v ? (p.Hout + 2) * (p.Hout + 2) : p.y_hs * p.y_hs, G = p.Nh * p.Nw;
@@ -1403,6 +1620,8 @@
     else hipLaunchKernelGGL((wino_kernel<1, 1, 2, true, false>), grid, dim3(256), lds, stream, p);
     hipError_t e = hipGetLastError();
     if (e != hipSuccess) return e;
+    if (launches) *launches = 2;
+    if (p.out_mode) return launch_wino_handoff(p, ax, p.out_mode - 1, n_tiles * WCN, stream);
     const long long total = (long long)p.Cout * p.Ntotal;
     const long long blocks = (total + 255) / 256;
     const dim3 flat((unsigned)(blocks < 8192 ? blocks : 8192));
diff --git a/stereo-3d-reconstruction_amd/csrc/s3r_host.h b/stereo-3d-reconstruction_amd/csrc/s3r_host.h
--- a/stereo-3d-reconstruction_amd/csrc/s3r_host.h
+++ b/stereo-3d-reconstruction_amd/csrc/s3r_host.h
@@ -60,6 +60,7 @@
     std::vector<Geo> g;
     std::vector<int64_t> off;
     std::vector<char> fuse_head;
+    std::vector<int64_t> region;
     bool stem_wino = false;
     bool pad_input = false;
     int64_t pad_off = 0;
diff --git a/stereo-3d-reconstruction_amd/csrc/s3r_kernels.h b/stereo-3d-reconstruction_amd/csrc/s3r_kernels.h
--- a/stereo-3d-reconstruction_amd/csrc/s3r_kernels.h
+++ b/stereo-3d-reconstruction_amd/csrc/s3r_kernels.h
@@ -100,6 +100,7 @@
     int x_cls, Hout, Dout, ncls;
     const float* xd;
     int xd_mode;
+    int out_mode;
 };
 
 struct TClsEntry {
@@ -166,6 +167,7 @@
 int64_t wino2_slab_elems(int ax, int cout, int ntotal, int form);
 int64_t wino2_npad(int64_t ntotal);
 hipError_t launch_conv_wino2(ConvParams p, int ax, int form, bool to_v, hipStream_t stream, int* launches);
+hipError_t launch_wino_handoff(const ConvParams& p, int prod, int cons, int npad, hipStream_t stream);
 hipError_t launch_cost_volume_wino2(const float* fl, const float* fr, float* V, int B, int C, int D, int H, int W, hipStream_t s);
 int wino_bk();
 hipError_t launch_wino_diff(const float* x, float* D, long long planes, int Dp, int Hp, int Wp, int three, hipStream_t s);
diff --git a/stereo-3d-reconstruction_amd/csrc/s3r_plan.hip b/stereo-3d-reconstruction_amd/csrc/s3r_plan.hip
--- a/stereo-3d-reconstruction_amd/csrc/s3r_plan.hip
+++ b/stereo-3d-reconstruction_amd/csrc/s3r_plan.hip
@@ -136,7 +136,9 @@
         return fail(S3R_ERR_INVALID, "halo must be in [0, 8]");
     if (d->dtype != S3R_F32 && d->dtype != S3R_BF16) return fail(S3R_ERR_INVALID, "unknown dtype %d", d->dtype);
     if ((d->in_layout != S3R_LAYOUT_PLAIN && d->in_layout != S3R_LAYOUT_WINO_H && d->in_layout != S3R_LAYOUT_WINO_DH &&
-         d->in_layout != S3R_LAYOUT_WINO_HW) || (d->out_layout != S3R_LAYOUT_PLAIN && d->out_layout != S3R_LAYOUT_WINO_HW))
+         d->in_layout != S3R_LAYOUT_WINO_HW && d->in_layout != S3R_LAYOUT_WINO_3D && d->in_layout != S3R_LAYOUT_DIFF) ||
+        (d->out_layout != S3R_LAYOUT_PLAIN && d->out_layout != S3R_LAYOUT_WINO_HW && d->out_layout != S3R_LAYOUT_WINO_3D &&
+         d->out_layout != S3R_LAYOUT_DIFF))
         return fail(S3R_ERR_INVALID, "unknown layout");
     if ((d->in_layout || d->out_layout) && d->op == S3R_OP_LINEAR)
         return fail(S3R_ERR_INVALID, "the transformed input layout exists on the convolution paths only");
@@ -212,6 +214,32 @@
             return fail(S3R_ERR_INVALID, "the two-axis Winograd output layout is written by an fp32 Conv2d with an output edge %% 4 == 0 and cout %% 32 == 0");
         g->y_elems = 36 * (int64_t)d->cout * s3r::wino2_npad((int64_t)d->batch * (g->out / 4) * (g->out / 4));
     }
+    if (d->in_layout == S3R_LAYOUT_WINO_3D) {
+        const int ax = wino2_ax(d);
+        if ((ax != 0 && ax != 1) || d->in_halo != d->pad)
+            return fail(S3R_ERR_INVALID, "the general two-axis Winograd input layout serves an fp32 Conv3d k=3 s=1 p=1 / k=4 s=1 p=0 with cin %% %d == 0, "
+                        "in_halo = pad", s3r::wino_bk());
+        g->x_elems = wino2_geo(d).v_sample * d->batch;
+    }
+    if (d->in_layout == S3R_LAYOUT_DIFF) {
+        if (!dwino_layer(d) || d->in_halo != 1)
+            return fail(S3R_ERR_INVALID, "the difference-tensor input layout serves the Winograd form of an fp32 ConvTranspose3d k=4 s=2 p=1 over an "
+                        "edge %% 4 == 0, in_halo = 1");
+        g->x_elems *= 4;
+    }
+    if (d->out_layout == S3R_LAYOUT_WINO_3D || d->out_layout == S3R_LAYOUT_DIFF) {
+        const bool diff = d->out_layout == S3R_LAYOUT_DIFF;
+        if (d->dtype != S3R_F32 || d->ndim != 3 || d->cout % s3r::wino_bk() != 0 || d->act > S3R_ACT_RELU ||
+            (diff ? d->out_halo != 1 || (g->out & 3) : d->out_halo > 1 || g->out < (d->out_halo ? 4 : 5)))
+            return fail(S3R_ERR_INVALID, "a consumer's operand is written by an fp32 3D layer with cout %% %d == 0, no activation or ReLU, and the halo the "
+                        "consumer reads (two-axis planes: out_halo 1 for k3 p1, 0 for k4 p0; difference tensors: out_halo 1, output edge %% 4 == 0)",
+                        s3r::wino_bk());
+        if (diff) g->y_elems *= 4;
+        else {
+            const int sg = d->out_halo ? (g->out + 3) / 4 : (g->out - 2) / 2;
+            g->y_elems = (int64_t)(d->out_halo ? 36 : 25) * d->batch * d->cout * sg * sg * g->out_p;
+        }
+    }
     g->w_elems = (int64_t)d->cin * d->cout * ipow(d->k, g->nd);
     if (d->op == S3R_OP_DECONV)
         g->flops = 2.0 * d->batch * (double)d->cin * g->in_sp * d->cout * ipow(d->k, g->nd);
@@ -294,8 +322,9 @@
 }
 bool wino_desc_ok(const s3r_conv_desc* d) {
     if (!(wino_layer(d) || dwino_layer(d)) || d->act >= S3R_ACT_SIGMOID || d->in_halo != 1 || d->ksplit > 1 || dil_of(d) != 1) return false;
-    if (d->out_layout != S3R_LAYOUT_PLAIN) return false;
-    return d->in_layout == S3R_LAYOUT_PLAIN || (d->in_layout == S3R_LAYOUT_WINO_H && wino_layer(d));
+    if (d->out_layout != S3R_LAYOUT_PLAIN && !(d->out_layout == S3R_LAYOUT_DIFF && dwino_layer(d))) return false;
+    return d->in_layout == S3R_LAYOUT_PLAIN || (d->in_layout == S3R_LAYOUT_WINO_H && wino_layer(d)) ||
+           (d->in_layout == S3R_LAYOUT_DIFF && dwino_layer(d));
 }
 int wino2_ax(const s3r_conv_desc* d) {
     if (d->dtype == S3R_BF16 || d->op != S3R_OP_CONV || d->stride != 1 || d->cin % s3r::wino_bk() != 0 || d->cout <= 1) return -1;
@@ -308,8 +337,20 @@
 bool wino2_desc_ok(const s3r_conv_desc* d) {
     return wino2_ax(d) >= 0 && d->act < S3R_ACT_SIGMOID && dil_of(d) == 1 && d->in_halo == d->pad && d->ksplit <= 1 &&
            (d->in_layout == S3R_LAYOUT_PLAIN || (d->in_layout == S3R_LAYOUT_WINO_DH && wino2_ax(d) == 0 && d->in_size % 4 == 0) ||
-            (d->in_layout == S3R_LAYOUT_WINO_HW && wino2_ax(d) == 2 && d->in_size % 4 == 0)) &&
-           (d->out_layout == S3R_LAYOUT_PLAIN || (d->out_layout == S3R_LAYOUT_WINO_HW && wino2_ax(d) == 2 && d->in_size % 4 == 0));
+            (d->in_layout == S3R_LAYOUT_WINO_HW && wino2_ax(d) == 2 && d->in_size % 4 == 0) ||
+            (d->in_layout == S3R_LAYOUT_WINO_3D && wino2_ax(d) <= 1)) &&
+           (d->out_layout == S3R_LAYOUT_PLAIN || (d->out_layout == S3R_LAYOUT_WINO_HW && wino2_ax(d) == 2 && d->in_size % 4 == 0) ||
+            ((d->out_layout == S3R_LAYOUT_WINO_3D || d->out_layout == S3R_LAYOUT_DIFF) && wino2_ax(d) <= 1));
+}
+static bool forced_direct(const s3r_conv_desc* d) {
+    return d->algo == S3R_ALGO_DIRECT || (d->algo == S3R_ALGO_AUTO && (d->tile >= 0 || d->ksplit >= 1));
+}
+static bool two_axis_io(const s3r_conv_desc* d) {
+    if (d->in_layout == S3R_LAYOUT_WINO_DH || d->in_layout == S3R_LAYOUT_WINO_HW || d->in_layout == S3R_LAYOUT_WINO_3D ||
+        d->out_layout == S3R_LAYOUT_WINO_HW)
+        return true;
+    return d->op == S3R_OP_CONV && (d->out_layout == S3R_LAYOUT_WINO_3D || d->out_layout == S3R_LAYOUT_DIFF) && wino2_ax(d) >= 0 &&
+           !forced_direct(d);
 }
 int wino2_max_edge() {
     static const int e = getenv("S3R_WINO2_MAX_EDGE") ? atoi(getenv("S3R_WINO2_MAX_EDGE")) : 28;
@@ -347,7 +388,7 @@
             return fail(S3R_ERR_INVALID, "algo = WINOGRAD: this layer / descriptor has no such Winograd form (one-axis: fp32 Conv k3 s1 p1 "
                         "with cin %% %d == 0 and edge >= 4, or ConvTranspose3d k4 s2 p1 over an edge %% 4 == 0, in_halo = 1; two-axis "
                         "(tile = 3): Conv3d k3 s1 p1 / k4 s1 p0, in_halo = pad; plain layouts, no split-K, no sigmoid)", s3r::wino_bk());
-        const bool two_io = d->in_layout == S3R_LAYOUT_WINO_DH || d->in_layout == S3R_LAYOUT_WINO_HW || d->out_layout == S3R_LAYOUT_WINO_HW;
+        const bool two_io = two_axis_io(d);
         if (two_io && !(two && (d->tile < 0 || d->tile >= 3)))
             return fail(S3R_ERR_INVALID, "a two-axis transformed input / output runs the two-axis kernel only");
         if (d->tile >= 3 || !one || two_io ||
@@ -357,7 +398,7 @@
         } else { *alg = ALG_WINO; *form = d->tile; }
         return S3R_OK;
     }
-    if (d->in_layout == S3R_LAYOUT_WINO_DH || d->in_layout == S3R_LAYOUT_WINO_HW || d->out_layout == S3R_LAYOUT_WINO_HW) {
+    if (two_axis_io(d)) {
         if (d->algo == S3R_ALGO_DIRECT || !wino2_desc_ok(d) || d->tile >= 0)
             return fail(S3R_ERR_INVALID, "a two-axis transformed input / output runs the two-axis kernel only: algo AUTO / WINOGRAD, no direct "
                         "tile / split-K override");
@@ -371,7 +412,17 @@
         *alg = ALG_WINO;
         return S3R_OK;
     }
+    if (d->in_layout == S3R_LAYOUT_DIFF || d->out_layout == S3R_LAYOUT_DIFF) {
+        if (d->op != S3R_OP_DECONV || forced_direct(d) || !wino_desc_ok(d))
+            return fail(S3R_ERR_INVALID, "the difference-tensor layout is read / written by the Winograd form of a ConvTranspose3d k4 s2 p1 (algo AUTO / "
+                        "WINOGRAD, no direct tile / split-K override), or written by a two-axis Conv3d");
+        *alg = ALG_WINO;
+        return S3R_OK;
+    }
+    if (d->in_layout == S3R_LAYOUT_WINO_3D || (d->out_layout == S3R_LAYOUT_WINO_3D && d->op != S3R_OP_CONV))
+        return fail(S3R_ERR_INVALID, "the general two-axis layout is read by the two-axis kernel and written by a convolution only");
     if (d->algo == S3R_ALGO_DIRECT || d->tile >= 0 || d->ksplit >= 1 || wino_mode() <= 0) return S3R_OK;
+    if (d->out_layout == S3R_LAYOUT_WINO_3D) return S3R_OK;
     if (wino2_desc_ok(d) && d->in_size <= wino2_max_edge()) *alg = ALG_WINO2;
     else if (d->op == S3R_OP_DECONV && dwino3_desc_ok(d) && d->in_size >= 16) *alg = ALG_WINO3;
     else if (wino_desc_ok(d)) *alg = ALG_WINO;
@@ -436,7 +487,7 @@
     if (d->batch <= 0) return w;
     const int kind = wino_kind(d);
     if (d->op == S3R_OP_DECONV) {
-        w.v = dwino_d_elems(d);
+        if (d->in_layout != S3R_LAYOUT_DIFF) w.v = dwino_d_elems(d);
         const int nt = (int)wino_positions(d, d->batch);
         w.slab = s3r::wino_slab_elems(kind, d->cout, nt, s3r::wino_plan(kind, d->cout, wino_kcls(d), nt, head, form < 0 ? 1 : form));
     } else {
@@ -470,7 +521,7 @@
     WinoNeed w = {0, 0, 0};
     const Wino2Geo g2 = wino2_geo(d);
     if (d->batch <= 0 || g2.bmax <= 0) return w;
-    if (d->in_layout != S3R_LAYOUT_WINO_DH && d->in_layout != S3R_LAYOUT_WINO_HW)
+    if (d->in_layout != S3R_LAYOUT_WINO_DH && d->in_layout != S3R_LAYOUT_WINO_HW && d->in_layout != S3R_LAYOUT_WINO_3D)
         w.v = ((g2.ax == 2 ? g2.ncls * d->cin * s3r::wino2_npad(g2.pos_sample * g2.bmax) : g2.v_sample * g2.bmax) + 255) / 256 * 256;
     for (int b0 = 0; b0 < d->batch; b0 += g2.bmax) {
         const int nb = d->batch - b0 < g2.bmax ? d->batch - b0 : g2.bmax;
@@ -700,9 +751,59 @@
 
 int64_t align_up(int64_t v, int64_t a) { return (v + a - 1) / a * a; }
 
+static int handoff_mask() {
+    static const int m = getenv("S3R_WINO_HANDOFF") ? atoi(getenv("S3R_WINO_HANDOFF")) : 1;
+    return m == 1 ? ~0 : m;
+}
+
+static int handoff3d(const s3r_conv_desc& a, const s3r_conv_desc& b, bool* take) {
+    *take = false;
+    if (a.dtype != S3R_F32 || b.dtype != S3R_F32 || a.ndim != 3 || b.ndim != 3 || a.cout != b.cin || out_size(&a) != b.in_size ||
+        a.batch != b.batch || a.out_halo != b.in_halo || a.act > S3R_ACT_RELU || a.cout % s3r::wino_bk() != 0 || staged_layer(&a) ||
+        staged_layer(&b))
+        return S3R_LAYOUT_PLAIN;
+    const int op = b.in_size + 2 * b.in_halo;
+    if (op * op * op > 8192) return S3R_LAYOUT_PLAIN;
+    int alg_a, form_a, alg_b, form_b;
+    if (resolve_algo(&a, &alg_a, &form_a) != S3R_OK || resolve_algo(&b, &alg_b, &form_b) != S3R_OK) return S3R_LAYOUT_PLAIN;
+    int lay = S3R_LAYOUT_PLAIN, bit = 0;
+    bool forms = true;
+    if (alg_b == ALG_WINO2 && wino2_ax(&b) <= 1 && b.in_halo == b.pad && b.in_size >= (b.pad ? 4 : 5) && wino2_geo(&b).bmax >= b.batch)
+        lay = S3R_LAYOUT_WINO_3D;
+    else if (alg_b == ALG_WINO && b.op == S3R_OP_DECONV && b.in_halo == 1 && dwino_materialise(&b))
+        lay = S3R_LAYOUT_DIFF;
+    else return S3R_LAYOUT_PLAIN;
+    if (alg_a == ALG_WINO2 && wino2_ax(&a) <= 1) {
+        bit = lay == S3R_LAYOUT_DIFF ? 16 : 8;
+        const Wino2Geo g2 = wino2_geo(&a);
+        if (g2.bmax < a.batch) return S3R_LAYOUT_PLAIN;
+        forms = wino2_form_of(&a, (int)(g2.pos_sample * a.batch), form_a) == 0;
+    } else if (alg_a == ALG_WINO && a.op == S3R_OP_DECONV && lay == S3R_LAYOUT_DIFF) {
+        bit = 32;
+        forms = s3r::wino_plan(2, a.cout, wino_kcls(&a), (int)wino_positions(&a, a.batch), false, form_a).mode == s3r::WINO_CP;
+    } else if (alg_a == ALG_DIRECT && a.op == S3R_OP_CONV && lay == S3R_LAYOUT_WINO_3D && a.out_layout == S3R_LAYOUT_PLAIN) {
+        bit = 4;
+        Geo ga;
+        Launch L;
+        if (geometry(&a, &ga) != S3R_OK) return S3R_LAYOUT_PLAIN;
+        s3r::ConvParams pa = make_params(&a, ga);
+        if (resolve_launch(&a, &pa, &L) != S3R_OK || L.ksplit <= 1) return S3R_LAYOUT_PLAIN;
+    } else return S3R_LAYOUT_PLAIN;
+    if (!(handoff_mask() & bit)) return S3R_LAYOUT_PLAIN;
+    s3r_conv_desc a2 = a, b2 = b;
+    a2.out_layout = lay; b2.in_layout = lay;
+    int alg2, form2;
+    Geo g2;
+    if (geometry(&a2, &g2) != S3R_OK || geometry(&b2, &g2) != S3R_OK) return S3R_LAYOUT_PLAIN;
+    if (resolve_algo(&a2, &alg2, &form2) != S3R_OK || alg2 != alg_a || form2 != form_a) return S3R_LAYOUT_PLAIN;
+    if (resolve_algo(&b2, &alg2, &form2) != S3R_OK || alg2 != alg_b || form2 != form_b) return S3R_LAYOUT_PLAIN;
+    *take = forms;
+    return lay;
+}
+
 int plan_chain(const s3r_layer* layers, int n, Plan* pl) {
     if (!layers || n <= 0) return fail(S3R_ERR_INVALID, "empty chain");
-    pl->d.resize(n); pl->r.resize(n); pl->g.resize(n); pl->off.assign(n, -1); pl->fuse_head.assign(n, 0);
+    pl->d.resize(n); pl->r.resize(n); pl->g.resize(n); pl->off.assign(n, -1); pl->fuse_head.assign(n, 0); pl->region.assign(n, 0);
     for (int i = 0; i < n; ++i) {
         pl->d[i] = layers[i].desc;
         if (i > 0) pl->d[i].in_layout = S3R_LAYOUT_PLAIN;
@@ -733,7 +834,7 @@
             }
         }
         if (i > 0 && pl->r[i - 1] == R_MFMA && pl->r[i] == R_MFMA && pl->d[i].dtype == S3R_F32) {
-            static const int fuse = getenv("S3R_WINO_HANDOFF") ? atoi(getenv("S3R_WINO_HANDOFF")) : 1;
+            const int fuse = handoff_mask() & 2;
             s3r_conv_desc& a = pl->d[i - 1];
             s3r_conv_desc& b = pl->d[i];
             int alg_a, alg_b, form;
@@ -744,6 +845,21 @@
                 b.in_layout = S3R_LAYOUT_WINO_HW;
                 const int rg = geometry(&a, &pl->g[i - 1]);
                 if (rg) return rg;
+            }
+            bool take = false;
+            const int lay = b.ndim == 3 ? handoff3d(a, b, &take) : S3R_LAYOUT_PLAIN;
+            if (lay != S3R_LAYOUT_PLAIN) {
+                s3r_conv_desc a2 = a;
+                a2.out_layout = lay;
+                Geo ga;
+                const int rg = geometry(&a2, &ga);
+                if (rg) return rg;
+                pl->region[i - 1] = ga.y_store > pl->g[i - 1].y_store ? ga.y_store : pl->g[i - 1].y_store;
+                if (take) {
+                    a = a2;
+                    b.in_layout = lay;
+                    pl->g[i - 1] = ga;
+                }
             }
         }
         int rc = geometry(&pl->d[i], &pl->g[i]);
@@ -791,10 +907,13 @@
     for (int i = 0; i + 1 < n; ++i) {
         pl->off[i] = off;
         if (i == 0 && pl->stem_wino) off = align_up(off + pl->g[1].x_store, 256);
-        else if (!pl->fuse_head[i]) off = align_up(off + pl->g[i].y_store, 256);
+        else if (!pl->fuse_head[i]) off = align_up(off + (pl->region[i] > pl->g[i].y_store ? pl->region[i] : pl->g[i].y_store), 256);
     }
     for (int i = 0; i < n; ++i) {
-        const int64_t sc = s3r_conv_scratch_elems(&pl->d[i]);
+        s3r_conv_desc t = pl->d[i];
+        if (i > 0 && pl->region[i - 1]) t.in_layout = S3R_LAYOUT_PLAIN;
+        if (pl->region[i]) t.out_layout = S3R_LAYOUT_PLAIN;
+        const int64_t sc = s3r_conv_scratch_elems(&t);
         if (sc < 0) return (int)sc;
         if (sc > pl->scratch_elems) pl->scratch_elems = sc;
     }
```

New measurement: 8876 (median of 6 runs). 1.2% higher.
